# VictoriaMetrics/VictoriaLogs

Measured on NVIDIA H100. Metric: log rows scanned/sec (LogsQL phrase+regex), higher is better.
Workload: dtype u8

## Files before the change

### include/vlscan.h

```cpp
#ifndef VLSCAN_H
#define VLSCAN_H

#include <stddef.h>
#include <stdint.h>

#ifdef __cplusplus
extern "C" {
#endif

typedef struct vlscan_ctx vlscan_ctx;
typedef struct vlscan_program vlscan_program;
typedef struct vlscan_batch vlscan_batch;

enum {
    VLSCAN_VT_STRING = 1, VLSCAN_VT_DICT = 2, VLSCAN_VT_UINT8 = 3, VLSCAN_VT_UINT16 = 4, VLSCAN_VT_UINT32 = 5,
    VLSCAN_VT_UINT64 = 6, VLSCAN_VT_FLOAT64 = 7, VLSCAN_VT_IPV4 = 8, VLSCAN_VT_ISO8601 = 9, VLSCAN_VT_INT64 = 10
};

enum { VLSCAN_COL_CONST = 1, VLSCAN_COL_VALUES = 2 };

enum {
    VLSCAN_STAGE_ONDISK = 0,
    VLSCAN_STAGE_DECODED = 1
};

typedef struct vlscan_column {
    uint32_t field;
    uint8_t kind;
    uint8_t value_type;
    uint8_t stage;
    uint8_t dict_len;
    uint64_t min_value;
    uint64_t max_value;
    const uint8_t* const_value; uint64_t const_len;
    const uint8_t* dict_blob;   const uint32_t* dict_offsets;
    const uint8_t* values;      uint64_t values_len;
    const uint8_t* lens_items;  uint64_t lens_items_len;
    const uint8_t* data;        uint64_t data_len;
    const uint8_t* bloom;       uint64_t bloom_len;
} vlscan_column;

typedef struct vlscan_block {
    uint64_t rows;
    uint32_t ncols;
    uint32_t ts_marshal_type;
    const vlscan_column* cols;
    const uint8_t* timestamps; uint64_t timestamps_len;
    int64_t min_timestamp, max_timestamp;
} vlscan_block;

typedef struct vlscan_stats {
    uint64_t blocks;
    uint64_t rows;
    uint64_t rows_matched;
    uint64_t blocks_matched;
    uint64_t values_bytes;
    uint64_t bloom_probe_bytes;
    uint64_t bitmap_bytes;
    uint64_t columns_read;
    uint64_t gpu_launches;
    uint64_t h2d_bytes;
    uint64_t d2h_bytes;
    double gpu_ms;
    double scan_kernel_ms;
    uint64_t scan_kernel_bytes;
    uint64_t staged_columns;
    uint64_t pruned_columns;
} vlscan_stats;

typedef struct vlscan_gen_config {
    uint64_t seed;
    uint64_t total_rows;
    uint32_t rows_per_block;
    uint32_t hot_block_permille;
    uint32_t hit_row_permille;
    uint32_t columns_mask;
} vlscan_gen_config;
#define VLSCAN_GEN_T0 1700000000000000000ll
#define VLSCAN_GEN_STEP 1000000ll

int vlscan_device_count(void);
vlscan_ctx* vlscan_ctx_create(int device);
void vlscan_ctx_free(vlscan_ctx* ctx);
const char* vlscan_last_error(const vlscan_ctx* ctx);
void* vlscan_ctx_stream(const vlscan_ctx* ctx);
int vlscan_ctx_sync(vlscan_ctx* ctx);

enum { VLSCAN_F_NOOP = 0, VLSCAN_F_PHRASE, VLSCAN_F_PREFIX, VLSCAN_F_EXACT, VLSCAN_F_IN, VLSCAN_F_REGEXP, VLSCAN_F_AND, VLSCAN_F_OR, VLSCAN_F_NOT,
       VLSCAN_F_EXACT_PREFIX = 9, VLSCAN_F_LEN_RANGE = 10, VLSCAN_F_STRING_RANGE = 11, VLSCAN_F_IPV4_RANGE = 12, VLSCAN_F_VALUE_TYPE = 13,
       VLSCAN_F_ANY_CASE_PHRASE = 14, VLSCAN_F_ANY_CASE_PREFIX = 15, VLSCAN_F_SEQUENCE = 16, VLSCAN_F_CONTAINS_ALL = 17, VLSCAN_F_CONTAINS_ANY = 18, VLSCAN_F_EQ_FIELD = 19, VLSCAN_F_LE_FIELD = 20, VLSCAN_F_RANGE = 21, VLSCAN_F_TIME = 22 };
int vlscan_program_create(const void* tree, size_t tree_len, vlscan_program** out);
void vlscan_program_free(vlscan_program* prog);
uint32_t vlscan_program_nfields(const vlscan_program* prog);
const char* vlscan_program_field(const vlscan_program* prog, uint32_t i, size_t* len);
int64_t vlscan_program_leaf_tokens(const vlscan_program* prog, uint32_t leaf, char* buf, size_t cap);
int64_t vlscan_program_prepass_tokens(const vlscan_program* prog, char* buf, size_t cap);
int64_t vlscan_program_in_hashes(const vlscan_program* prog, uint32_t leaf, uint64_t* out, size_t cap);
int64_t vlscan_program_in_typed(const vlscan_program* prog, uint32_t leaf, int value_type, uint64_t* out, size_t cap);
int vlscan_format_float64(uint64_t ieee_bits, char* buf, size_t cap);
double vlscan_parse_math_number(const void* s, size_t len);
int vlscan_parse_typed(int value_type, const void* s, size_t len, uint64_t* out);
int vlscan_eval_predicate(int kind, const void* value, size_t value_len, const void* arg1, size_t arg1_len, const void* arg2,
                          size_t arg2_len, uint64_t aux0, uint64_t aux1);

int vlscan_batch_upload(vlscan_ctx* ctx, const char* const* field_names, const size_t* field_name_lens, uint32_t nfields,
                        const vlscan_block* blocks, uint64_t nblocks, vlscan_batch** out, vlscan_stats* stats );
void vlscan_batch_free(vlscan_batch* batch);
uint64_t vlscan_batch_nblocks(const vlscan_batch* batch);
uint64_t vlscan_batch_rows(const vlscan_batch* batch);
uint64_t vlscan_batch_words(const vlscan_batch* batch);
uint64_t vlscan_batch_device_bytes(const vlscan_batch* batch);

int vlscan_batch_generate(vlscan_ctx* ctx, const vlscan_gen_config* cfg, uint64_t block_lo, uint64_t block_hi, vlscan_batch** out);

typedef struct vlscan_host_blocks vlscan_host_blocks;
int vlscan_batch_download(vlscan_ctx* ctx, const vlscan_batch* batch, vlscan_host_blocks** out);
const vlscan_block* vlscan_host_blocks_get(const vlscan_host_blocks* hb, uint64_t* nblocks, uint32_t* nfields);
const char* vlscan_host_blocks_field(const vlscan_host_blocks* hb, uint32_t i, size_t* len);
uint64_t vlscan_host_blocks_bytes(const vlscan_host_blocks* hb);
void vlscan_host_blocks_free(vlscan_host_blocks* hb);
int vlscan_host_blocks_compress(const vlscan_host_blocks* in, int threads, vlscan_host_blocks** out);

int vlscan_zstd_decompress(vlscan_ctx* ctx, uint32_t nframes, const void* const* frames, const size_t* frame_lens, void* dst,
                           const uint64_t* dst_offsets);
int vlscan_zstd_inspect(const void* bytes_block, size_t len, uint64_t out[5]);
int vlscan_zstd_walk_digest(const vlscan_block* blocks, uint64_t nblocks, int threads, uint64_t out[12]);

typedef struct vlscan_part vlscan_part;
typedef int (*vlscan_inflate_fn)(void* user, const void* frame, size_t frame_len, void* dst, size_t dst_len);
int vlscan_part_open(vlscan_ctx* ctx , const char* path, vlscan_inflate_fn inflate , void* user, vlscan_part** out);
void vlscan_part_free(vlscan_part* part);
void vlscan_part_header(const vlscan_part* part, uint64_t out[8]);
uint64_t vlscan_part_nblocks(const vlscan_part* part);
int vlscan_part_block_header(const vlscan_part* part, uint64_t i, uint64_t out[15]);
int vlscan_part_timestamps(const vlscan_part* part, uint64_t i, const uint8_t** data, uint64_t* len);
uint32_t vlscan_part_ncolumn_names(const vlscan_part* part);
const char* vlscan_part_column_name(const vlscan_part* part, uint32_t i, size_t* len);
int vlscan_part_blocks(const vlscan_part* part, const char* const* field_names, const size_t* field_name_lens, uint32_t nfields, uint64_t block_lo,
                       uint64_t block_hi, int64_t min_timestamp, int64_t max_timestamp, vlscan_host_blocks** out);
const uint64_t* vlscan_host_blocks_source(const vlscan_host_blocks* hb, uint64_t* n);

int vlscan_scan_resident(vlscan_ctx* ctx, const vlscan_program* prog, const vlscan_batch* batch, vlscan_stats* stats);

int vlscan_last_scan_stats(vlscan_ctx* ctx, vlscan_stats* stats);

int vlscan_fetch_results(vlscan_ctx* ctx, uint64_t* out_bitmap_words, uint32_t* out_match_counts, vlscan_stats* stats );
int vlscan_fetch_hits(vlscan_ctx* ctx, uint32_t* out_hit_rows, uint64_t cap, uint64_t* out_hit_offsets);
int vlscan_gather_timestamps(vlscan_ctx* ctx, int64_t* out_timestamps, uint64_t cap, uint64_t* out_hit_offsets);
int vlscan_gather_values(vlscan_ctx* ctx, const char* field, size_t field_len, uint8_t* out_bytes, uint64_t cap_bytes, uint64_t* out_value_offsets, uint64_t cap_values,
                         uint64_t* out_total_bytes, uint64_t* out_hit_offsets);
enum { VLSCAN_BUCKET_PLAIN = 0, VLSCAN_BUCKET_WEEK = 1, VLSCAN_BUCKET_MONTH = 2, VLSCAN_BUCKET_YEAR = 3 };
#define VLSCAN_HITS_MAX_BY 4
typedef struct vlscan_hits_query {
    int64_t step, offset;
    uint32_t calendar;
    uint32_t nby;
    const char* const* by_names;
    const size_t* by_name_lens;
} vlscan_hits_query;
int vlscan_hits_stats(vlscan_ctx* ctx, const vlscan_hits_query* q, int64_t* out_buckets, uint64_t* out_counts, uint64_t cap_groups, uint8_t* out_key_bytes,
                      uint64_t cap_key_bytes, uint64_t* out_key_offsets, uint64_t out_info[4]);
#define VLSCAN_STATS_MAX_VALUES 4
int vlscan_hits_sums(vlscan_ctx* ctx, const vlscan_hits_query* q, const char* const* value_names, const size_t* value_name_lens, uint32_t nvalues, int64_t* out_buckets,
                     uint64_t* out_counts, double* out_sums, uint64_t* out_value_counts, uint64_t cap_groups, uint8_t* out_key_bytes, uint64_t cap_key_bytes,
                     uint64_t* out_key_offsets, uint64_t out_info[4]);
int64_t vlscan_truncate_timestamp(int64_t ts, int64_t step, int64_t offset, uint32_t calendar);
typedef struct vlscan_last_query {
    uint64_t limit;
    int64_t min_timestamp;
    uint32_t nfields;
    const char* const* field_names;
    const size_t* field_name_lens;
} vlscan_last_query;
int vlscan_last_rows(vlscan_ctx* ctx, const vlscan_last_query* q, int64_t* out_timestamps, uint32_t* out_blocks, uint32_t* out_rows, uint64_t cap_rows,
                     uint8_t* out_bytes, uint64_t cap_bytes, uint64_t* out_offsets, uint64_t out_info[4]);
enum { VLSCAN_FACET_UINT64 = 0, VLSCAN_FACET_NEGATIVE = 1, VLSCAN_FACET_STRING = 2 };
#define VLSCAN_FACETS_DEFAULT_MAX_VALUES 1000
#define VLSCAN_FACETS_DEFAULT_MAX_VALUE_LEN 128
typedef struct vlscan_facets_query {
    uint64_t max_values_per_field;
    uint64_t max_value_len;
    uint32_t nfields;
    const char* const* field_names;
    const size_t* field_name_lens;
} vlscan_facets_query;
int vlscan_facets(vlscan_ctx* ctx, const vlscan_facets_query* q, uint8_t* out_dropped, uint64_t* out_field_offsets, uint64_t* out_hits, uint8_t* out_classes,
                  uint64_t cap_entries, uint8_t* out_bytes, uint64_t cap_bytes, uint64_t* out_value_offsets, uint64_t out_info[4]);
int vlscan_result_digest(vlscan_ctx* ctx, uint64_t block_lo, uint64_t block_hi, uint64_t key_base, uint64_t* out_digest);
int vlscan_totals_sum(vlscan_ctx* const* ctxs, int nctx, uint64_t out4[4]);
int vlscan_result_device_ptrs(vlscan_ctx* ctx, void** bitmap_words, void** match_counts, void** totals4);

int vlscan_scan_batch(vlscan_ctx* ctx, const vlscan_program* prog, const char* const* field_names, const size_t* field_name_lens,
                      uint32_t nfields, const vlscan_block* blocks, uint64_t nblocks, uint64_t* out_bitmap_words,
                      uint32_t* out_match_counts, vlscan_stats* stats);
int vlscan_scan_batch_keep(vlscan_ctx* ctx, const vlscan_program* prog, const char* const* field_names, const size_t* field_name_lens,
                           uint32_t nfields, const vlscan_block* blocks, uint64_t nblocks, uint64_t* out_bitmap_words,
                           uint32_t* out_match_counts, vlscan_stats* stats);
int vlscan_stage_selected(vlscan_ctx* ctx, const vlscan_block* blocks, uint64_t nblocks, const char* const* field_names, const size_t* field_name_lens,
                          uint32_t nfields, const uint32_t* block_list , uint64_t nlist, uint64_t out_info[4]);

#ifdef __cplusplus
}
#endif
#endif
```

### victorialogs_b200/csrc/vl_engine.cu

```cuda
#include <dlfcn.h>
#include <algorithm>
#include <atomic>
#include <chrono>
#include <cmath>
#include <limits>
#include <thread>
#include <cstdio>
#include <cstdlib>
#include <cstring>
#include <functional>
#include <map>
#include <memory>
#include <mutex>
#include "vl_copier.h"
#include "vl_engine.h"
#include "vl_kernels.cuh"
#include "vl_program.h"
#include "vl_part.h"
#include "vl_mathnum.cuh"

using namespace vl;

namespace vl {
static thread_local std::string g_thread_err;
void set_thread_error(const std::string& s) { g_thread_err = s; }
}

struct vlscan_program {
    Program p;
    struct Image { DevBuf leaves, prepass, regexes, blob, u64s, u32s; DevProgram view; };
    std::map<int, std::unique_ptr<Image>> images;
    std::mutex mu;
    const DevProgram& image(int device, cudaStream_t st) {
        std::lock_guard<std::mutex> g(mu);
        auto it = images.find(device);
        if (it != images.end()) return it->second->view;
        auto im = std::make_unique<Image>();
        auto up = [&](DevBuf& b, const void* src, size_t n) { b.ensure(std::max<size_t>(n, 16)); if (n) VL_CUDA(cudaMemcpyAsync(b.p, src, n, cudaMemcpyHostToDevice, st)); };
        up(im->leaves, p.leaves.data(), p.leaves.size() * sizeof(DevLeaf));
        up(im->prepass, p.prepass.data(), p.prepass.size() * sizeof(DevPrepass));
        up(im->regexes, p.regexes.data(), p.regexes.size() * sizeof(DevRegex));
        up(im->blob, p.blob.data(), p.blob.size());
        up(im->u64s, p.u64s.data(), p.u64s.size() * 8);
        up(im->u32s, p.u32s.data(), p.u32s.size() * 4);
        VL_CUDA(cudaStreamSynchronize(st));
        im->view = DevProgram{im->leaves.as<DevLeaf>(), im->prepass.as<DevPrepass>(), im->regexes.as<DevRegex>(), im->blob.as<uint8_t>(), im->u64s.as<uint64_t>(), im->u32s.as<uint32_t>()};
        auto& ref = *im;
        images[device] = std::move(im);
        return ref.view;
    }
    ~vlscan_program() { for (auto& kv : images) { cudaSetDevice(kv.first); kv.second->leaves.release(); kv.second->prepass.release(); kv.second->regexes.release(); kv.second->blob.release(); kv.second->u64s.release(); kv.second->u32s.release(); } }
};

struct vlscan_host_blocks {
    void* pinned = nullptr; size_t bytes = 0;
    std::vector<vlscan_block> blocks;
    std::vector<vlscan_column> cols;
    std::vector<std::string> fields;
    std::vector<std::vector<uint32_t>> dict_offsets;
    std::vector<std::unique_ptr<std::vector<uint8_t>>> owned;
    std::vector<uint64_t> source;
};
struct vlscan_part { vl::part::PartReader r; };

void* vlscan_ctx::ensure_pinned(size_t n) {
    if (n <= pinned_cap) return pinned;
    if (pinned) cudaFreeHost(pinned);
    pinned = nullptr; pinned_cap = 0;
    VL_CUDA(cudaMallocHost(&pinned, n));
    pinned_cap = n;
    return pinned;
}

namespace {

struct ZstdWriter {
    size_t (*compress)(void*, size_t, const void*, size_t, int) = nullptr;
    size_t (*bound)(size_t) = nullptr;
    unsigned (*is_error)(size_t) = nullptr;
    bool ok = false;
    ZstdWriter() {
        void* h = dlopen("libzstd.so.1", RTLD_NOW | RTLD_GLOBAL);
        if (!h) return;
        compress = (decltype(compress))dlsym(h, "ZSTD_compress");
        bound = (decltype(bound))dlsym(h, "ZSTD_compressBound");
        is_error = (decltype(is_error))dlsym(h, "ZSTD_isError");
        ok = compress && bound && is_error;
    }
};
ZstdWriter& zstd_writer() { static ZstdWriter z; return z; }

}

namespace vl {
void finish_batch_layout(vlscan_ctx* ctx, vlscan_batch* b, const std::vector<uint32_t>& rows) {
    b->nblocks = rows.size();
    b->h_rows = rows;
    b->h_word_off.assign(rows.size() + 1, 0);
    b->rows = 0;
    for (size_t i = 0; i < rows.size(); i++) { b->h_word_off[i + 1] = b->h_word_off[i] + (rows[i] + 63) / 64; b->rows += rows[i]; }
    b->nwords = b->h_word_off.back();
    std::vector<uint32_t> wb(b->nwords);
    std::vector<uint64_t> init(b->nwords);
    for (size_t i = 0; i < rows.size(); i++) {
        for (uint64_t w = b->h_word_off[i]; w < b->h_word_off[i + 1]; w++) { wb[w] = (uint32_t)i; init[w] = ~0ull; }
        uint32_t tail = rows[i] & 63;
        if (tail) init[b->h_word_off[i + 1] - 1] = (~0ull) >> (64 - tail);
    }
    b->blk_rows.ensure(std::max<size_t>(rows.size() * 4, 16));
    b->blk_word_off.ensure((rows.size() + 1) * 8);
    b->word_block.ensure(std::max<size_t>(b->nwords * 4, 16));
    b->init_bitmap.ensure(std::max<size_t>(b->nwords * 8, 16));
    if (!rows.empty()) VL_CUDA(cudaMemcpyAsync(b->blk_rows.p, rows.data(), rows.size() * 4, cudaMemcpyHostToDevice, ctx->stream));
    VL_CUDA(cudaMemcpyAsync(b->blk_word_off.p, b->h_word_off.data(), (rows.size() + 1) * 8, cudaMemcpyHostToDevice, ctx->stream));
    if (b->nwords) {
        VL_CUDA(cudaMemcpyAsync(b->word_block.p, wb.data(), b->nwords * 4, cudaMemcpyHostToDevice, ctx->stream));
        VL_CUDA(cudaMemcpyAsync(b->init_bitmap.p, init.data(), b->nwords * 8, cudaMemcpyHostToDevice, ctx->stream));
    }
    VL_CUDA(cudaStreamSynchronize(ctx->stream));
}
}

static uint64_t collect_values_blocks(const vlscan_block* blocks, uint64_t nblocks, std::vector<ZValuesBlock>& zv, const uint8_t* need = nullptr, uint32_t nfields = 0, std::vector<size_t>* at = nullptr) {
    uint64_t zc = 512;
    if (at) at->assign((size_t)nblocks * nfields, SIZE_MAX);
    for (uint64_t b = 0; b < nblocks; b++)
        for (uint32_t k = 0; k < blocks[b].ncols; k++) {
            const vlscan_column& c = blocks[b].cols[k];
            if (c.kind != VLSCAN_COL_VALUES || c.stage != VLSCAN_STAGE_ONDISK) continue;
            if (need && (c.field >= nfields || !need[b * nfields + c.field])) continue;
            if (at && c.field < nfields && (*at)[b * nfields + c.field] == SIZE_MAX) (*at)[b * nfields + c.field] = zv.size();
            zv.push_back({c.values, (size_t)c.values_len, zc});
            zc += c.values_len;
        }
    return zc;
}
static double now_s() { return std::chrono::duration<double>(std::chrono::steady_clock::now().time_since_epoch()).count(); }

namespace {
struct Upload {
    vlscan_ctx* ctx; vlscan_batch* out; const vlscan_block* blocks; uint64_t nblocks; uint32_t nfields; vlscan_stats* stats;
    const std::vector<char>* need_bloom;
    std::vector<DevColumn>& cols = out->h_cols;
    const bool dbg = getenv("VLSCAN_DEBUG_TIMING") != nullptr; const double t_start = now_s();
    Copier io{ctx};
    std::vector<uint32_t> rows = std::vector<uint32_t>(nblocks);
    std::vector<Piece> pieces;
    std::vector<std::unique_ptr<std::vector<uint8_t>>> owned;
    uint64_t cursor = 16;
    ZstdJob zjob;
    uint64_t regen_cursor = 0;
    struct Ondisk { uint64_t col; uint32_t lens_frame, data_frame; uint64_t lens_rel, data_rel; };
    std::vector<Ondisk> ondisk;
    std::vector<OndiskCol> ocols;
    struct TsFrame { uint64_t block; uint32_t frame; uint64_t rel; };
    std::vector<TsFrame> ts_frames;
    std::vector<DevTimestamps> tsv;
    std::vector<ZValuesBlock> zv; std::vector<ZValuesInfo> zinfo; std::vector<size_t> zv_of; std::vector<uint64_t> ts_zoff; size_t zbad = SIZE_MAX; std::string zmsg;
    uint64_t add_piece(const uint8_t* src, uint64_t len) { uint64_t off = arena_reserve(cursor, len); if (len) pieces.push_back({src, len, off}); return off; }
    template <class F> void walk(bool ts, F&& f) {
        for (uint64_t b = 0; b < nblocks; b++) {
            const vlscan_block& blk = blocks[b];
            if (blk.rows > (8u << 20)) throw BadInput("block rows exceed maxRowsPerBlock (8Mi)");
            rows[b] = (uint32_t)blk.rows;
            if (ts) timestamps(blk, b);
            for (uint32_t k = 0; k < blk.ncols; k++) {
                if (blk.cols[k].field >= nfields) throw BadInput("column refers to a field outside the batch field table");
                f(blk, blk.cols[k], (size_t)b * nfields + blk.cols[k].field);
            }
        }
    }
    void sources(const uint8_t* need, bool ts) {
        uint64_t zc = collect_values_blocks(blocks, nblocks, zv, need, nfields, &zv_of);
        for (const ZValuesBlock& v : zv) if (v.n) io.src.push_back({v.p, v.n, v.zoff});
        ts_zoff.resize(ts ? nblocks : 0);
        for (uint64_t b = 0; b < nblocks && ts; b++) {
            const vlscan_block& blk = blocks[b];
            if (blk.ts_marshal_type != MT_ZSTD_NEAREST_DELTA2 && blk.ts_marshal_type != MT_ZSTD_NEAREST_DELTA) continue;
            if (blk.timestamps_len > vl::part::kMaxTimestampsBlockSize) throw BadInput("timestamps block size cannot exceed 8 MiB");
            ts_zoff[b] = zc;
            if (blk.timestamps_len) io.src.push_back({blk.timestamps, blk.timestamps_len, zc});
            zc += blk.timestamps_len;
        }
        if (!io.src.empty()) { ctx->zsrc.ensure(zc + 512); io.send_sources(ctx->zsrc.as<uint8_t>()); }
        zinfo.resize(zv.size());
        const double t_w = now_s();
        if (!zv.empty()) zjob.add_values_blocks(zv.data(), zv.size(), host_threads(), zinfo.data(), &zbad, &zmsg);
        if (dbg) fprintf(stderr, "[vlscan upload] header walk of %zu values blocks on %d host threads: %.1f ms (after %.1f ms of collecting and enqueueing the copies)\n",
                         zv.size(), host_threads(), 1e3 * (now_s() - t_w), 1e3 * (t_w - t_start));
    }
    template <class F> void header(const vlscan_column& c, size_t i, F&& payload) {
        DevColumn& d = cols[i];
        if (d.kind != COL_MISSING) throw BadInput("duplicate column for one field in a block");
        if (c.kind == VLSCAN_COL_CONST) {
            d.kind = COL_CONST; d.meta_len = (uint32_t)c.const_len; d.meta_off = add_piece(c.const_value, c.const_len);
            return;
        }
        if (c.kind != VLSCAN_COL_VALUES) throw BadInput("unknown column kind");
        if (c.value_type < VT_STRING || c.value_type >= VT_MAX) throw BadInput("unknown valueType");
        d.kind = COL_VALUES; d.vt = c.value_type; d.min_value = c.min_value; d.max_value = c.max_value;
        payload();
        if (c.bloom_len % 8) throw BadInput("cannot unmarshal bloomFilter from src with size not multiple by 8");
        if (need_bloom && !(*need_bloom)[c.field]) { d.bloom_words = 0; d.bloom_off = add_piece(c.bloom, 0); }
        else { d.bloom_words = (uint32_t)(c.bloom_len / 8); d.bloom_off = add_piece(c.bloom, c.bloom_len); }
        if (c.value_type == VT_DICT) {
            if (c.dict_len > 8) throw BadInput("valuesDict may contain max 8 items");
            d.dict_len = c.dict_len;
            uint32_t total = c.dict_len ? c.dict_offsets[c.dict_len] : 0;
            d.meta_len = total;
            if (c.dict_len && c.dict_blob == (const uint8_t*)c.dict_offsets + 4 * (c.dict_len + 1)) {
                d.meta_off = add_piece((const uint8_t*)c.dict_offsets, 4 * (c.dict_len + 1) + total);
            } else {
                auto meta = std::make_unique<std::vector<uint8_t>>();
                meta->resize(4 * (c.dict_len + 1) + total);
                if (c.dict_len) memcpy(meta->data(), c.dict_offsets, 4 * (c.dict_len + 1)); else memset(meta->data(), 0, 4);
                if (total) memcpy(meta->data() + 4 * (c.dict_len + 1), c.dict_blob, total);
                d.meta_off = add_piece(meta->data(), meta->size());
                owned.push_back(std::move(meta));
            }
        }
    }
    void values(const vlscan_block& blk, const vlscan_column& c, size_t ci) {
        DevColumn& d = cols[ci];
        if (c.stage == VLSCAN_STAGE_ONDISK) {
            const size_t z = zv_of[ci];
            if (z >= zbad) throw BadInput(zmsg);
            const uint64_t lens_len = zinfo[z].lens_len, data_len = zinfo[z].data_len;
            if (data_len > 0xFFFFFFFFull) throw BadInput("values block too large");
            const uint64_t lr = arena_reserve(regen_cursor, lens_len + 15), dr = arena_reserve(regen_cursor, data_len);
            d.lens_off = lr + 16; d.data_off = dr; d.data_len = data_len;
            ondisk.push_back({ci, (uint32_t)(2 * z), (uint32_t)(2 * z + 1), lr + 15, dr});
            ocols.push_back({ci, lens_len, blk.rows});
        } else if (c.stage == VLSCAN_STAGE_DECODED) {
            const uint8_t* lens_items = c.lens_items; const uint64_t lens_len = c.lens_items_len, data_len = c.data_len;
            if (lens_len < 1) throw BadInput("cannot unmarshal uint64 block type from empty src");
            uint8_t lt = lens_items[0];
            if (lt > 7) throw BadInput("unexpected uint64 block type");
            uint64_t want = lt < 4 ? (blk.rows << lt) : (1ull << (lt - 4));
            if (lens_len - 1 != want) throw BadInput("unexpected block length for uint items");
            d.lens_type = lt;
            if (lt >= 4) { uint64_t v = 0; for (uint64_t i = 0; i < want; i++) v = (v << 8) | lens_items[1 + i]; if (v > 0xFFFFFFFFull) throw BadInput("row length does not fit 32 bits"); d.lens_const = (uint32_t)v; }
            if (data_len > 0xFFFFFFFFull) throw BadInput("values block too large");
            d.lens_off = add_piece(lens_items + 1, lens_len - 1);
            d.data_off = add_piece(c.data, data_len); d.data_len = data_len;
            d.data_const = (blk.rows >= 2 && lt >= 4 && data_len == d.lens_const) ? 1 : 0;
        } else throw BadInput("unknown values stage");
    }
    void timestamps(const vlscan_block& blk, uint64_t b) {
        if (!blk.ts_marshal_type) return;
        if (blk.ts_marshal_type > MT_NEAREST_DELTA) throw BadInput("unknown MarshalType of a timestamps block");
        if (blk.timestamps_len > vl::part::kMaxTimestampsBlockSize) throw BadInput("timestamps block size cannot exceed 8 MiB");
        if (tsv.empty()) { tsv.resize(nblocks); memset(tsv.data(), 0, nblocks * sizeof(DevTimestamps)); }
        DevTimestamps& t = tsv[b];
        t.first = blk.min_timestamp; t.max = blk.max_timestamp;
        if (blk.ts_marshal_type == MT_ZSTD_NEAREST_DELTA2 || blk.ts_marshal_type == MT_ZSTD_NEAREST_DELTA) {
            uint64_t regen = 0; uint32_t id = 0;
            zjob.add_frame(blk.timestamps, blk.timestamps_len, ts_zoff[b], &regen, &id);
            if (regen > 10ull * blk.rows + 16) throw BadInput("cannot unmarshal timestamps: the decompressed block is larger than its varints can be");
            t.mt = blk.ts_marshal_type == MT_ZSTD_NEAREST_DELTA2 ? MT_NEAREST_DELTA2 : MT_NEAREST_DELTA;
            t.len = (uint32_t)regen;
            ts_frames.push_back({b, id, arena_reserve(regen_cursor, regen)});
        } else {
            t.mt = (uint8_t)blk.ts_marshal_type; t.len = (uint32_t)blk.timestamps_len;
            t.off = add_piece(blk.timestamps, blk.timestamps_len);
        }
    }

    uint64_t commit(DevBuf& region, const std::vector<uint64_t>* patch, bool layout) {
        const uint64_t regen_base = (cursor + kArenaAlign - 1) / kArenaAlign * kArenaAlign;
        for (const Ondisk& o : ondisk) {
            DevColumn& d = cols[o.col];
            d.lens_off += regen_base; d.data_off += regen_base;
            zjob.set_dst(o.lens_frame, regen_base + o.lens_rel); zjob.set_dst(o.data_frame, regen_base + o.data_rel);
        }
        for (const TsFrame& tf : ts_frames) { tsv[tf.block].off = regen_base + tf.rel; zjob.set_dst(tf.frame, regen_base + tf.rel); }
        const bool have_z = !ondisk.empty() || !ts_frames.empty();
        if (have_z) cursor = regen_base + regen_cursor;
        const uint64_t bytes = cursor + kArenaPad;
        const double t_desc = now_s();
        region.ensure(bytes);
        const double t_alloc = now_s();
        uint8_t* cols_base = region.as<uint8_t>();
        std::vector<ColPatch> patches;
        if (patch) {
            const uint64_t delta = (uint64_t)(uintptr_t)region.p - (uint64_t)(uintptr_t)out->arena.p;
            cols_base = out->arena.as<uint8_t>();
            patches.resize(patch->size());
            for (size_t i = 0; i < patch->size(); i++) {
                DevColumn& d = cols[(*patch)[i]];
                d.lens_off += delta; d.data_off += delta;
                patches[i].col = (*patch)[i]; patches[i].c = d;
            }
        }
        cudaStream_t cs = ctx->copy_stream;
        cudaEvent_t ev_cleared = io.events.make(), ev_copied = io.events.make();
        VL_CUDA(cudaMemsetAsync(region.p, 0, bytes, ctx->stream));
        VL_CUDA(cudaEventRecord(ev_cleared, ctx->stream));
        VL_CUDA(cudaStreamWaitEvent(cs, ev_cleared, 0));
        const double t_h2d = dbg ? now_s() : 0;
        double t_zrun = 0;
        if (have_z) {
            zjob.set_group_hook([&](uint64_t src_end) { io.wait_sources(ctx->stream, src_end); });
            zjob.run(ctx, ctx->zsrc.as<uint8_t>(), region.as<uint8_t>());
            io.ship_sources(UINT64_MAX);
            if (dbg) t_zrun = now_s();
        }
        io.copy(pieces, region.as<uint8_t>());
        DevBuf& table = patch ? ctx->patch : out->cols;
        const void* entries = patch ? (const void*)patches.data() : (const void*)cols.data();
        const size_t table_bytes = patch ? patches.size() * sizeof(ColPatch) : cols.size() * sizeof(DevColumn);
        table.ensure(std::max<size_t>(table_bytes, 16));
        if (table_bytes) VL_CUDA(cudaMemcpyAsync(table.p, entries, table_bytes, cudaMemcpyHostToDevice, cs));
        io.h2d += table_bytes;
        if (!patch) out->has_ts = !tsv.empty();
        if (!tsv.empty()) {
            out->ts.ensure(nblocks * sizeof(DevTimestamps));
            VL_CUDA(cudaMemcpyAsync(out->ts.p, tsv.data(), nblocks * sizeof(DevTimestamps), cudaMemcpyHostToDevice, cs));
            io.h2d += nblocks * sizeof(DevTimestamps);
        }
        VL_CUDA(cudaEventRecord(ev_copied, cs));
        if (!patches.empty()) {
            VL_CUDA(cudaStreamWaitEvent(ctx->stream, ev_copied, 0));
            k_patch_cols<<<cdiv(patches.size(), 128), 128, 0, ctx->stream>>>(out->cols.as<DevColumn>(), ctx->patch.as<ColPatch>(), (uint32_t)patches.size());
            launch_check(ctx);
        }
        const double t_enq = dbg ? now_s() : 0;
        if (have_z) {
            VL_CUDA(cudaStreamWaitEvent(ctx->stream, ev_copied, 0));
            ctx->zcols.ensure(16 + ocols.size() * sizeof(OndiskCol));
            VL_CUDA(cudaMemsetAsync(ctx->zcols.p, 0, 16, ctx->stream));
            VL_CUDA(cudaMemcpyAsync(ctx->zcols.as<uint8_t>() + 16, ocols.data(), ocols.size() * sizeof(OndiskCol), cudaMemcpyHostToDevice, ctx->stream));
            if (!ocols.empty()) {
                k_finish_ondisk_cols<<<cdiv(ocols.size(), 128), 128, 0, ctx->stream>>>(cols_base, out->cols.as<DevColumn>(), (const OndiskCol*)(ctx->zcols.as<uint8_t>() + 16),
                                                                                         (uint32_t)ocols.size(), ctx->zcols.as<unsigned long long>());
                launch_check(ctx);
            }
            io.h2d += ocols.size() * sizeof(OndiskCol);
            zjob.check(ctx);
            unsigned long long cst[2] = {0, 0};
            VL_CUDA(cudaMemcpy(cst, ctx->zcols.p, 16, cudaMemcpyDeviceToHost));
            static const char* what[] = {"", "cannot unmarshal uint64 block type from empty src", "unexpected uint64 block type", "unexpected block length for uint items", "row length does not fit 32 bits"};
            if (cst[0]) throw BadInput(what[std::min<unsigned long long>(cst[0], 4)]);
        }
        VL_CUDA(cudaStreamWaitEvent(ctx->stream, ev_copied, 0));
        double t_copy = 0;
        if (dbg) { VL_CUDA(cudaStreamSynchronize(ctx->stream)); t_copy = now_s(); }
        if (nfields) out->note_columns(cols);
        if (layout) finish_batch_layout(ctx, out, rows);
        else VL_CUDA(cudaStreamSynchronize(ctx->stream));
        if (dbg) fprintf(stderr, "[vlscan upload] blocks=%llu arena=%.1f MB h2d=%.1f MB pieces=%zu+%zu pinned=%d: describe %.1f ms, alloc %.1f ms, copy %.1f ms (%.1f GB/s), "
                                 "zstd %llu frames / %llu blocks / %llu sequences: enqueue %.1f ms, decode %.1f ms; layout %.1f ms\n", (unsigned long long)nblocks,
                         bytes / 1e6, io.h2d / 1e6, pieces.size(), io.src.size(), (int)io.all_pinned, 1e3 * (t_desc - t_start), 1e3 * (t_alloc - t_desc), 1e3 * (t_enq - (t_zrun > 0 ? t_zrun : t_h2d)), io.h2d / 1e9 / std::max(t_copy - t_start, 1e-9),
                         (unsigned long long)zjob.frames(), (unsigned long long)zjob.compressed_blocks(), (unsigned long long)zjob.sequences(), 1e3 * (t_zrun > 0 ? t_zrun - t_h2d : 0), 1e3 * (t_copy - t_enq), 1e3 * (now_s() - t_copy));
        if (layout) io.h2d += out->nwords * 12 + nblocks * 12;
        if (stats) stats->h2d_bytes += io.h2d;
        return bytes;
    }
};
}

enum UploadMode { UP_FULL = 0, UP_HEADERS = 1, UP_VALUES = 2, UP_LATE = 3 };
static void do_upload(vlscan_ctx* ctx, const char* const* field_names, const size_t* field_name_lens, uint32_t nfields, const vlscan_block* blocks,
                      uint64_t nblocks, vlscan_batch* out, vlscan_stats* stats, const std::vector<char>* need_bloom = nullptr, UploadMode mode = UP_FULL,
                      const uint8_t* need = nullptr, uint64_t* zframes = nullptr) {
    VL_CUDA(cudaSetDevice(ctx->device));
    if (nblocks > 0xFFFFFFF0ull) throw BadInput("too many blocks in one batch");
    out->device = ctx->device; out->nfields = nfields;
    Upload u{ctx, out, blocks, nblocks, nfields, stats, need_bloom};
    if (mode == UP_FULL || mode == UP_HEADERS) {
        for (uint32_t f = 0; f < nfields; f++) out->field_names.emplace_back(field_names[f], field_name_lens[f]);
        u.cols.assign((size_t)nblocks * std::max<uint32_t>(nfields, 1), DevColumn{});
        memset(u.cols.data(), 0, u.cols.size() * sizeof(DevColumn));
        out->late_used = 0; out->split_hdr = mode == UP_HEADERS;
    } else if (u.cols.size() != (size_t)nblocks * std::max<uint32_t>(nfields, 1) || !need) throw BadInput("internal: values phase of a bloom-first upload without its header phase");
    try {
        switch (mode) {
        case UP_FULL:
            u.sources(nullptr, true);
            u.walk(true, [&](const vlscan_block& blk, const vlscan_column& c, size_t i) { u.header(c, i, [&] { u.values(blk, c, i); }); });
            out->arena_bytes = u.commit(out->arena, nullptr, true);
            out->harena_bytes = 0;
            std::vector<DevColumn>().swap(out->h_cols);
            break;
        case UP_HEADERS:
            u.walk(false, [&](const vlscan_block&, const vlscan_column& c, size_t i) {
                u.header(c, i, [&] {
                    if (c.stage != VLSCAN_STAGE_ONDISK && c.stage != VLSCAN_STAGE_DECODED) throw BadInput("unknown values stage");
                    u.cols[i].values_state = VALUES_DEFERRED;
                });
            });
            out->harena_bytes = u.commit(out->harena, nullptr, true);
            break;
        case UP_VALUES:
            u.sources(need, true);
            u.walk(true, [&](const vlscan_block& blk, const vlscan_column& c, size_t i) {
                if (c.kind != VLSCAN_COL_VALUES) return;
                u.cols[i].values_state = need[i] ? VALUES_STAGED : VALUES_ABSENT;
                if (need[i]) u.values(blk, c, i);
            });
            out->arena_bytes = u.commit(out->arena, nullptr, false);
            break;
        case UP_LATE: {
            std::vector<uint64_t> staged;
            u.sources(need, false);
            u.walk(false, [&](const vlscan_block& blk, const vlscan_column& c, size_t i) {
                if (c.kind != VLSCAN_COL_VALUES || !need[i]) return;
                if (u.cols[i].values_state == VALUES_STAGED) throw BadInput("duplicate column for one field in a block");
                u.cols[i].values_state = VALUES_STAGED;
                u.values(blk, c, i);
                staged.push_back(i);
            });
            if (out->late_used == out->late.size()) out->late.emplace_back();
            u.commit(out->late[out->late_used], &staged, false);
            out->late_used++;
            *zframes += u.zjob.frames();
            break;
        }
        }
    } catch (...) {
        cudaStreamSynchronize(ctx->copy_stream); cudaStreamSynchronize(ctx->stream);
        throw;
    }
}

const uint32_t* vl::row_offsets(vlscan_ctx* ctx, const BatchView& B, int slot, const uint32_t* list, const uint32_t* wc, unsigned long long* stats, int wc_slot) {
    uint8_t* ready = ctx->ready[slot].as<uint8_t>();
    if (!ctx->ready_cleared[slot]) { VL_CUDA(cudaMemsetAsync(ready, 0, B.nblocks, ctx->stream)); ctx->ready_cleared[slot] = 1; }
    k_lens_offsets<<<ctx->sm_count * 8, 256, 0, ctx->stream>>>(B, slot, list, wc, ctx->row_off8[slot].as<uint32_t>(), ready, stats, wc_slot); launch_check(ctx);
    return ctx->row_off8[slot].as<uint32_t>();
}

namespace {
struct ScanRun {
    vlscan_ctx* ctx; const vlscan_program* prog; const vlscan_batch* batch;
    DevProgram P; BatchView B; std::vector<int> field_slot;
    unsigned long long* stats;
    size_t regs_used = 0;

    uint64_t* new_reg() {
        if (regs_used == ctx->regs.size()) ctx->regs.emplace_back();
        DevBuf& r = ctx->regs[regs_used++];
        r.ensure(std::max<size_t>(B.nwords * 8, 16));
        return r.as<uint64_t>();
    }
    void free_reg() { regs_used--; }
    void copy_reg(uint64_t* dst, const uint64_t* src) { if (B.nwords) VL_CUDA(cudaMemcpyAsync(dst, src, B.nwords * 8, cudaMemcpyDeviceToDevice, ctx->stream)); }
    void andnot(uint64_t* a, const uint64_t* b) { if (!B.nwords) return; k_andnot<<<cdiv(B.nwords, 256), 256, 0, ctx->stream>>>(a, b, B.nwords); launch_check(ctx); }
    void prepass(const PNode& nd, uint64_t* reg) {
        if (nd.prepass_count == 0) return;
        std::vector<int> slots(nd.prepass_count);
        for (int e = 0; e < nd.prepass_count; e++) slots[e] = field_slot[prog->p.prepass[nd.prepass_begin + e].field];
        size_t off = slots_cursor; slots_cursor += slots.size();
        ctx->slots.ensure(std::max<size_t>(slots_total * 4, 16));
        VL_CUDA(cudaMemcpyAsync(ctx->slots.as<int>() + off, slots.data(), slots.size() * 4, cudaMemcpyHostToDevice, ctx->stream));
        k_prepass<<<cdiv((uint64_t)B.nblocks * 32, 128), 128, 0, ctx->stream>>>(P, B, (uint32_t)nd.prepass_begin, (uint32_t)nd.prepass_count, ctx->slots.as<int>() + off,
                                                                             nd.kind == F_OR, reg, stats);
        launch_check(ctx);
    }
    size_t slots_cursor = 0, slots_total = 0;

    void leaf(int leaf_idx, uint64_t* reg) {
        const DevLeaf& L = prog->p.leaves[leaf_idx];
        if (L.kind == F_NOOP) return;
        int slot = L.field >= 0 ? field_slot[L.field] : -1;
        uint8_t* action = ctx->action.as<uint8_t>(); uint64_t* payload = ctx->payload.as<uint64_t>(); uint64_t* leaf_bm = ctx->leaf_bm.as<uint64_t>();
        uint32_t* lens_blocks = ctx->lens_blocks.as<uint32_t>(); uint32_t* row_blocks = ctx->row_blocks.as<uint32_t>(); uint32_t* wc = ctx->work_count.as<uint32_t>();
        ScanTile* tiles = ctx->tiles.as<ScanTile>();
        VL_CUDA(cudaMemsetAsync(wc, 0, WC_COUNT * 4, ctx->stream));
        if (L.kind == F_EQ_FIELD || L.kind == F_LE_FIELD) {
            const int slot_b = field_slot[L.field2];
            uint32_t* lens_b = ctx->lens_blocks2.as<uint32_t>();
            k_plan_pair<<<cdiv((uint64_t)B.nblocks * 32, 256), 256, 0, ctx->stream>>>(P, B, (uint32_t)leaf_idx, slot, slot_b, reg, action, payload, lens_blocks, lens_b, row_blocks, wc, stats);
            launch_check(ctx);
            if (B.nwords) {
                const int persistent = ctx->sm_count * 8;
                const uint32_t *ro_a = nullptr, *ro_b = nullptr;
                for (int side = 0; side < 2; side++) {
                    const int sl = side ? slot_b : slot;
                    if (sl >= 0) (side ? ro_b : ro_a) = row_offsets(ctx, B, sl, side ? lens_b : lens_blocks, wc, stats, side ? WC_LENS2 : WC_LENS);
                }
                k_row_pair<<<persistent, 256, 0, ctx->stream>>>(P, B, (uint32_t)leaf_idx, slot, slot_b, row_blocks, wc, payload, reg, ro_a, ro_b, leaf_bm, stats); launch_check(ctx);
                k_apply_leaf<<<cdiv(B.nwords, 256), 256, 0, ctx->stream>>>(B, action, leaf_bm, reg); launch_check(ctx);
            }
            return;
        }
        k_plan_leaf<<<cdiv(B.nblocks, VL_PLAN_WARPS), VL_PLAN_WARPS * 32, 0, ctx->stream>>>(P, B, (uint32_t)leaf_idx, slot, reg, action, payload, lens_blocks, row_blocks, tiles, wc, stats);
        launch_check(ctx);
        if (slot >= 0 && B.nwords) {
            const uint32_t vts = batch->slot_vt_mask.empty() ? ~0u : batch->slot_vt_mask[slot];
            const bool has_string = vts >> VT_STRING & 1, has_dict = vts >> VT_DICT & 1;
            const bool has_numeric = (vts & ~((1u << VT_STRING) | (1u << VT_DICT))) != 0;
            const bool may_scan = L.str_strategy == STR_SCAN && has_string;
            const bool may_row = (has_string && L.str_strategy != STR_ALL) || has_numeric;
            const uint32_t* ro = may_scan || may_row ? row_offsets(ctx, B, slot, lens_blocks, wc, stats, WC_LENS) : nullptr;
            if (may_scan) {
                VL_CUDA(cudaMemsetAsync(leaf_bm, 0, B.nwords * 8, ctx->stream));
                ScanParams sp; memset(&sp, 0, sizeof sp);
                sp.mode = L.scan_mode; sp.needle_off = L.scan_needle_off; sp.needle_len = L.scan_needle_len; sp.starts_tok = L.starts_tok; sp.ends_tok = L.ends_tok; sp.regex = L.regex;
                const bool masked = fill_scan_patterns(prog->p.blob.data() + L.scan_needle_off, L.scan_needle_len, sp.pat, sp.msk, sp.delta, sp.nd16);
                if (L.scan_mode == SCAN_CONTAINS || L.scan_mode >= SCAN_RX_DOTPLUS) { sp.starts_tok = sp.ends_tok = 0; }
                auto& evp = next_scan_events();
                VL_CUDA(cudaEventRecord(evp.first, ctx->stream));
                if (masked) k_substr_scan<true><<<ctx->sm_count * ctx->scan_occ[1], VL_SCAN_THREADS, 0, ctx->stream>>>(P, B, slot, sp, tiles, wc, ro, leaf_bm);
                else k_substr_scan<false><<<ctx->sm_count * ctx->scan_occ[0], VL_SCAN_THREADS, 0, ctx->stream>>>(P, B, slot, sp, tiles, wc, ro, leaf_bm);
                launch_check(ctx);
                VL_CUDA(cudaEventRecord(evp.second, ctx->stream));
            }
            if (may_row) { k_row_match<<<ctx->sm_count * ctx->row_occ, 256, 0, ctx->stream>>>(P, B, (uint32_t)leaf_idx, slot, row_blocks, wc, action, payload, reg, ro, leaf_bm); launch_check(ctx); }
            if (has_dict || has_numeric) { k_word_match<<<cdiv(B.nwords, 128), 128, 0, ctx->stream>>>(P, B, (uint32_t)leaf_idx, slot, action, payload, reg, leaf_bm, stats); launch_check(ctx); }
        }
        if (L.kind == F_TIME && B.nwords) {
            ctx->ts_vals.ensure(B.nwords * 64 * 8);
            k_time_match<<<ctx->sm_count * 4, 256, 0, ctx->stream>>>(B, (long long)L.aux0, (long long)L.aux1, row_blocks, wc, ctx->ts_vals.as<unsigned long long>(), leaf_bm, stats);
            launch_check(ctx);
        }
        if (B.nwords) { k_apply_leaf<<<cdiv(B.nwords, 256), 256, 0, ctx->stream>>>(B, action, leaf_bm, reg); launch_check(ctx); }
    }
    std::pair<cudaEvent_t, cudaEvent_t>& next_scan_events() {
        if (ctx->scan_events_used == ctx->scan_events.size()) { cudaEvent_t a, b; VL_CUDA(cudaEventCreate(&a)); VL_CUDA(cudaEventCreate(&b)); ctx->scan_events.emplace_back(a, b); }
        return ctx->scan_events[ctx->scan_events_used++];
    }
    void probe_leaf(int leaf_idx, const uint64_t* reg, uint8_t* need) {
        const DevLeaf& L = prog->p.leaves[leaf_idx];
        if (L.kind == F_NOOP || L.kind == F_TIME) return;
        const int slot = L.field >= 0 ? field_slot[L.field] : -1;
        if (L.kind == F_EQ_FIELD || L.kind == F_LE_FIELD) {
            k_plan_pair<<<cdiv((uint64_t)B.nblocks * 32, 256), 256, 0, ctx->stream>>>(P, B, (uint32_t)leaf_idx, slot, field_slot[L.field2], reg, nullptr, nullptr, nullptr, nullptr, nullptr, nullptr, stats, need);
        } else {
            if (slot < 0) return;
            k_plan_leaf<<<cdiv(B.nblocks, VL_PLAN_WARPS), VL_PLAN_WARPS * 32, 0, ctx->stream>>>(P, B, (uint32_t)leaf_idx, slot, reg, nullptr, nullptr, nullptr, nullptr, nullptr, nullptr, stats, need);
        }
        launch_check(ctx);
    }
    void probe_node(int id, uint64_t* reg, uint8_t* need) {
        const PNode& nd = prog->p.nodes[id];
        switch (nd.kind) {
        case F_NOOP: break;
        case F_AND: case F_OR: {
            uint64_t* r = reg;
            if (nd.prepass_count) { r = new_reg(); copy_reg(r, reg); prepass(nd, r); }
            for (int k : nd.kids) probe_node(k, r, need);
            if (nd.prepass_count) free_reg();
            break;
        }
        case F_NOT: probe_node(nd.kids[0], reg, need); break;
        default: probe_leaf(nd.leaf, reg, need);
        }
    }
    void node(int id, uint64_t* reg) {
        const PNode& nd = prog->p.nodes[id];
        switch (nd.kind) {
        case F_NOOP: break;
        case F_AND: prepass(nd, reg); for (int k : nd.kids) node(k, reg); break;
        case F_OR: {
            prepass(nd, reg);
            uint64_t* res = new_reg(); uint64_t* tmp = new_reg();
            copy_reg(res, reg);
            for (int k : nd.kids) { copy_reg(tmp, res); node(k, tmp); andnot(res, tmp); }
            andnot(reg, res);
            free_reg(); free_reg();
            break;
        }
        case F_NOT: { uint64_t* tmp = new_reg(); copy_reg(tmp, reg); node(nd.kids[0], tmp); andnot(reg, tmp); free_reg(); break; }
        default: leaf(nd.leaf, reg);
        }
    }
};
}

static void read_stats(vlscan_ctx* ctx, vlscan_stats* st, bool check_error) {
    unsigned long long h[ST_COUNT];
    VL_CUDA(cudaMemcpyAsync(h, ctx->stats.p, sizeof h, cudaMemcpyDeviceToHost, ctx->stream));
    VL_CUDA(cudaStreamSynchronize(ctx->stream));
    if (check_error && h[ST_ERROR]) {
        static const char* const msg[] = {"", "cannot unmarshal strings: row lengths do not add up to the data length", "too big index for dict value",
                                          "unexpected length for binary representation of a number", "", "", "the filter needs the timestamps of a block that was handed over without them", "cannot unmarshal timestamps",
                                          "internal: a filter reached the values of a column that the bloom-first probe pass had left on the host"};
        throw BadInput(msg[std::min<unsigned long long>(h[ST_ERROR], 8)]);
    }
    if (!st) return;
    st->values_bytes += h[ST_VALUES_BYTES]; st->bloom_probe_bytes += h[ST_BLOOM_BYTES]; st->columns_read += h[ST_COLUMNS_READ];
    st->bitmap_bytes += h[ST_BITMAP_BYTES]; st->rows_matched += h[ST_ROWS_MATCHED]; st->blocks_matched += h[ST_BLOCKS_MATCHED];
    st->scan_kernel_bytes += h[ST_SCAN_BYTES];
    float ms = 0;
    VL_CUDA(cudaEventElapsedTime(&ms, ctx->ev_begin, ctx->ev_end)); st->gpu_ms += ms;
    for (size_t i = 0; i < ctx->scan_events_used; i++) { VL_CUDA(cudaEventElapsedTime(&ms, ctx->scan_events[i].first, ctx->scan_events[i].second)); st->scan_kernel_ms += ms; }
}

static void do_scan(vlscan_ctx* ctx, const vlscan_program* prog, const vlscan_batch* batch, vlscan_stats* stats) {
    VL_CUDA(cudaSetDevice(ctx->device));
    if (batch->device != ctx->device) throw BadInput("batch lives on another device than the ctx");
    ScanRun run{ctx, prog, batch};
    run.P = const_cast<vlscan_program*>(prog)->image(ctx->device, ctx->stream);
    run.B = batch->view();
    const Program& pr = prog->p;
    run.field_slot.assign(pr.fields.size(), -1);
    for (size_t f = 0; f < pr.fields.size(); f++) for (uint32_t s = 0; s < batch->nfields; s++) if (batch->field_names[s] == pr.fields[f]) run.field_slot[f] = (int)s;
    for (auto& nd : pr.nodes) run.slots_total += nd.prepass_count;
    uint64_t nb = std::max<uint64_t>(batch->nblocks, 1), nw = std::max<uint64_t>(batch->nwords, 1);
    ctx->action.ensure(nb); ctx->payload.ensure(nb * 8); ctx->leaf_bm.ensure(nw * 8);
    ctx->lens_blocks.ensure(nb * 4); ctx->lens_blocks2.ensure(nb * 4); ctx->row_blocks.ensure(nb * 4); ctx->work_count.ensure(WC_COUNT * 4);
    {
        uint64_t max_tiles = batch->arena_bytes / VL_TILE_BYTES + nb + 16;
        ctx->tiles.ensure(max_tiles * sizeof(ScanTile));
    }
    ctx->stats.ensure(ST_COUNT * 8); ctx->totals.ensure(32); ctx->counts.ensure(nb * 4);
    if (ctx->row_off8.size() < batch->nfields) { ctx->row_off8.resize(batch->nfields); ctx->ready.resize(batch->nfields); }
    ctx->ready_cleared.assign(batch->nfields, 0);
    for (uint32_t s = 0; s < batch->nfields; s++) { ctx->row_off8[s].ensure(nw * 32); ctx->ready[s].ensure(nb); }
    uint64_t launches0 = ctx->launches;
    ctx->scan_events_used = 0;
    run.stats = ctx->stats.as<unsigned long long>();
    VL_CUDA(cudaEventRecord(ctx->ev_begin, ctx->stream));
    VL_CUDA(cudaMemsetAsync(ctx->stats.p, 0, ST_COUNT * 8, ctx->stream));
    VL_CUDA(cudaMemsetAsync(ctx->totals.p, 0, 32, ctx->stream));
    uint64_t* reg = run.new_reg();
    run.copy_reg(reg, batch->init_bitmap.as<uint64_t>());
    if (batch->nblocks) {
        run.node(pr.root, reg);
        k_finalize<<<cdiv(batch->nblocks, 8), 256, 0, ctx->stream>>>(run.B, reg, ctx->counts.as<uint32_t>(), run.stats, ctx->totals.as<unsigned long long>());
        launch_check(ctx);
    }
    VL_CUDA(cudaEventRecord(ctx->ev_end, ctx->stream));
    ctx->last_batch = batch; ctx->has_result = true; ctx->kept = false; ctx->last_launches = ctx->launches - launches0;
    ctx->last_nblocks = batch->nblocks; ctx->last_nwords = batch->nwords; ctx->last_rows = batch->rows;
    if (stats) {
        read_stats(ctx, stats, true);
        stats->blocks += batch->nblocks; stats->rows += batch->rows; stats->gpu_launches += ctx->launches - launches0;
    }
}

static void do_probe(vlscan_ctx* ctx, const vlscan_program* prog, const vlscan_batch* batch, std::vector<uint8_t>& need) {
    VL_CUDA(cudaSetDevice(ctx->device));
    ScanRun run{ctx, prog, batch};
    run.P = const_cast<vlscan_program*>(prog)->image(ctx->device, ctx->stream);
    run.B = batch->view();
    const Program& pr = prog->p;
    run.field_slot.assign(pr.fields.size(), -1);
    for (size_t f = 0; f < pr.fields.size(); f++) for (uint32_t s = 0; s < batch->nfields; s++) if (batch->field_names[s] == pr.fields[f]) run.field_slot[f] = (int)s;
    for (auto& nd : pr.nodes) run.slots_total += nd.prepass_count;
    const size_t cells = (size_t)batch->nblocks * batch->nfields;
    need.assign(cells, 0);
    if (!cells || !batch->nwords) return;
    ctx->need.ensure(std::max<size_t>(cells, 16)); ctx->stats.ensure(ST_COUNT * 8);
    VL_CUDA(cudaMemsetAsync(ctx->need.p, 0, cells, ctx->stream));
    VL_CUDA(cudaMemsetAsync(ctx->stats.p, 0, ST_COUNT * 8, ctx->stream));
    run.stats = ctx->stats.as<unsigned long long>();
    uint64_t* reg = run.new_reg();
    run.copy_reg(reg, batch->init_bitmap.as<uint64_t>());
    run.probe_node(pr.root, reg, ctx->need.as<uint8_t>());
    VL_CUDA(cudaMemcpyAsync(need.data(), ctx->need.p, cells, cudaMemcpyDeviceToHost, ctx->stream));
    VL_CUDA(cudaStreamSynchronize(ctx->stream));
}

extern "C" {

int vlscan_device_count(void) {
    int n = 0;
    if (cudaGetDeviceCount(&n) != cudaSuccess) { cudaGetLastError(); return 0; }
    return n;
}

vlscan_ctx* vlscan_ctx_create(int device) {
    vlscan_ctx* ctx = new vlscan_ctx();
    int rc = guarded(nullptr, [&] {
        int n = vlscan_device_count();
        if (n <= 0) throw CudaFail("no CUDA device is available: libvlscan has no CPU fallback", 100);
        ctx->device = ((device % n) + n) % n;
        VL_CUDA(cudaSetDevice(ctx->device));
        VL_CUDA(cudaStreamCreateWithFlags(&ctx->stream, cudaStreamNonBlocking));
        VL_CUDA(cudaStreamCreateWithFlags(&ctx->copy_stream, cudaStreamNonBlocking));
        VL_CUDA(cudaEventCreate(&ctx->ev_begin)); VL_CUDA(cudaEventCreate(&ctx->ev_end));
        cudaDeviceProp prop; VL_CUDA(cudaGetDeviceProperties(&prop, ctx->device)); ctx->sm_count = prop.multiProcessorCount;
        VL_CUDA(cudaOccupancyMaxActiveBlocksPerMultiprocessor(&ctx->scan_occ[0], k_substr_scan<false>, VL_SCAN_THREADS, 0));
        VL_CUDA(cudaOccupancyMaxActiveBlocksPerMultiprocessor(&ctx->scan_occ[1], k_substr_scan<true>, VL_SCAN_THREADS, 0));
        for (int& o : ctx->scan_occ) o = std::max(o, 1);
        VL_CUDA(cudaOccupancyMaxActiveBlocksPerMultiprocessor(&ctx->row_occ, k_row_match, 256, 0));
        ctx->row_occ = std::max(ctx->row_occ, 1);
    });
    if (rc) { delete ctx; return nullptr; }
    return ctx;
}
void vlscan_ctx_free(vlscan_ctx* ctx) {
    if (!ctx) return;
    cudaSetDevice(ctx->device);
    if (ctx->copy_stream) cudaStreamSynchronize(ctx->copy_stream);
    if (ctx->stream) cudaStreamSynchronize(ctx->stream);
    for (DevBuf* b : {&ctx->action, &ctx->payload, &ctx->leaf_bm, &ctx->lens_blocks, &ctx->row_blocks, &ctx->work_count, &ctx->stats, &ctx->totals, &ctx->counts, &ctx->slots, &ctx->hit_offs, &ctx->hits, &ctx->tiles, &ctx->lens_blocks2}) b->release();
    for (auto& r : ctx->regs) r.release();
    for (auto& r : ctx->row_off8) r.release();
    for (auto& r : ctx->ready) r.release();
    ctx->zsrc.release(); ctx->zcols.release(); ctx->ztest.release(); ctx->ts_vals.release();
    for (DevBuf* b : {&ctx->hit_block, &ctx->glens, &ctx->goffs, &ctx->gtiles, &ctx->gout, &ctx->gstat, &ctx->hslot, &ctx->hblk, &ctx->htab, &ctx->hgrp, &ctx->lcand, &ctx->ftab, &ctx->patch, &ctx->unstaged}) b->release();
    for (DevBuf& b : ctx->ftxt) b.release();
    zstd_dev_free(ctx->zdev);
    delete ctx->pool;
    if (ctx->pinned) cudaFreeHost(ctx->pinned);
    delete ctx->recycle;
    for (auto& e : ctx->scan_events) { cudaEventDestroy(e.first); cudaEventDestroy(e.second); }
    if (ctx->ev_begin) cudaEventDestroy(ctx->ev_begin);
    if (ctx->ev_end) cudaEventDestroy(ctx->ev_end);
    if (ctx->copy_stream) cudaStreamDestroy(ctx->copy_stream);
    if (ctx->stream) cudaStreamDestroy(ctx->stream);
    delete ctx;
}
const char* vlscan_last_error(const vlscan_ctx* ctx) { return ctx ? ctx->err.c_str() : g_thread_err.c_str(); }
void* vlscan_ctx_stream(const vlscan_ctx* ctx) { return (void*)ctx->stream; }
int vlscan_ctx_sync(vlscan_ctx* ctx) { return guarded(ctx, [&] { VL_CUDA(cudaSetDevice(ctx->device)); VL_CUDA(cudaStreamSynchronize(ctx->stream)); }); }

int vlscan_program_create(const void* tree, size_t tree_len, vlscan_program** out) {
    *out = nullptr;
    auto* pg = new vlscan_program();
    int rc = guarded(nullptr, [&] { ProgramBuilder(tree, tree_len, pg->p).build(); });
    if (rc) { delete pg; return rc; }
    *out = pg;
    return 0;
}
void vlscan_program_free(vlscan_program* prog) { delete prog; }
uint32_t vlscan_program_nfields(const vlscan_program* prog) { return (uint32_t)prog->p.fields.size(); }
const char* vlscan_program_field(const vlscan_program* prog, uint32_t i, size_t* len) { if (i >= prog->p.fields.size()) { *len = 0; return nullptr; } *len = prog->p.fields[i].size(); return prog->p.fields[i].data(); }
int64_t vlscan_program_leaf_tokens(const vlscan_program* prog, uint32_t leaf, char* buf, size_t cap) {
    if (leaf >= prog->p.leaf_tokens.size()) return -1;
    std::string s; for (size_t i = 0; i < prog->p.leaf_tokens[leaf].size(); i++) { if (i) s.push_back('\n'); s += prog->p.leaf_tokens[leaf][i]; }
    if (s.size() > cap) return -1;
    memcpy(buf, s.data(), s.size());
    return (int64_t)s.size();
}

int vlscan_eval_predicate(int kind, const void* value, size_t value_len, const void* arg1, size_t arg1_len, const void* arg2, size_t arg2_len, uint64_t aux0, uint64_t aux1) {
    if (value_len > 0xFFFFFFFFull || arg1_len > 0xFFFFFFFFull || arg2_len > 0xFFFFFFFFull) return -1;
    const uint8_t* v = (const uint8_t*)value; const uint32_t vn = (uint32_t)value_len;
    const uint8_t* a = (const uint8_t*)arg1; const uint32_t an = (uint32_t)arg1_len;
    switch (kind) {
    case F_REGEXP: {
        try { return vl::compile_regex(std::string((const char*)a, an)).match(v, vn) ? 1 : 0; } catch (const vl::RxError& e) { vl::set_thread_error(e.what()); return -2; }
    }
    case 14: return vl::any_case_match(v, vn, a, an, false) ? 1 : 0;
    case 15: return vl::any_case_match(v, vn, a, an, true) ? 1 : 0;
    case 16: return vl::match_sequence(v, vn, vl::PhraseList{a, an}) ? 1 : 0;
    case 17: return vl::match_all_phrases(v, vn, vl::PhraseList{a, an}) ? 1 : 0;
    case 18: return vl::match_any_phrase(v, vn, vl::PhraseList{a, an}) ? 1 : 0;
    }
    if (kind < F_EXACT_PREFIX || kind > F_IPV4_RANGE) return -1;
    return vl::range_predicate(kind, (const uint8_t*)value, (uint32_t)value_len, (const uint8_t*)arg1, (uint32_t)arg1_len, (const uint8_t*)arg2, (uint32_t)arg2_len, aux0, aux1) ? 1 : 0;
}

int64_t vlscan_program_prepass_tokens(const vlscan_program* prog, char* buf, size_t cap) {
    const Program& P = prog->p;
    std::string s;
    for (const PNode& nd : P.nodes) {
        if (nd.kind != F_AND && nd.kind != F_OR) continue;
        s += nd.kind == F_AND ? "A" : "O";
        for (int k = 0; k < nd.prepass_count; k++) {
            const DevPrepass& pp = P.prepass[(size_t)nd.prepass_begin + k];
            s += "\t" + P.fields[pp.field];
            const uint32_t* offs = (const uint32_t*)(P.blob.data() + pp.tok_offs_off);
            for (uint32_t t = 0; t < pp.ntokens; t++) { s += "\x1f"; s.append((const char*)P.blob.data() + pp.tok_blob_off + offs[t], offs[t + 1] - offs[t]); }
        }
        s += "\n";
    }
    if (s.size() > cap) return -1;
    memcpy(buf, s.data(), s.size());
    return (int64_t)s.size();
}

int64_t vlscan_program_in_hashes(const vlscan_program* prog, uint32_t leaf, uint64_t* out, size_t cap) {
    const Program& P = prog->p;
    if (leaf >= P.leaves.size() || P.leaves[leaf].kind != F_IN) return -1;
    const DevLeaf& L = P.leaves[leaf];
    std::vector<uint64_t> v;
    v.push_back(L.nhashes); v.insert(v.end(), P.u64s.begin() + L.hashes_off, P.u64s.begin() + L.hashes_off + L.nhashes);
    if (L.in_skip_sets) v.push_back(UINT64_MAX);
    else {
        v.push_back(L.in_nsets);
        for (uint32_t k = 0; k < L.in_nsets; k++) {
            const uint32_t off = P.u32s[L.in_sets_off + 2 * k], n = P.u32s[L.in_sets_off + 2 * k + 1];
            v.push_back(n); v.insert(v.end(), P.u64s.begin() + off, P.u64s.begin() + off + n);
        }
    }
    if (v.size() > cap) return -1;
    memcpy(out, v.data(), v.size() * 8);
    return (int64_t)v.size();
}

int64_t vlscan_program_in_typed(const vlscan_program* prog, uint32_t leaf, int value_type, uint64_t* out, size_t cap) {
    const Program& P = prog->p;
    if (leaf >= P.leaves.size() || P.leaves[leaf].kind != F_IN || value_type < VT_UINT8 || value_type >= VT_MAX) return -1;
    const DevLeaf& L = P.leaves[leaf];
    const uint32_t n = L.in_typed_cnt[value_type];
    if (n > cap) return -1;
    if (n) memcpy(out, P.u64s.data() + L.in_typed_off[value_type], (size_t)n * 8);
    return (int64_t)n;
}

int vlscan_parse_typed(int value_type, const void* s, size_t len, uint64_t* out) {
    const std::string v((const char*)s, len);
    uint64_t u = 0; int64_t i = 0; double f = 0; uint32_t ip = 0;
    switch (value_type) {
    case VT_UINT8: case VT_UINT16: case VT_UINT32: case VT_UINT64: if (!vl::parse_u64(v, &u)) return 0; *out = u; return 1;
    case VT_INT64: if (!vl::parse_i64(v, &i)) return 0; *out = (uint64_t)i; return 1;
    case VT_FLOAT64: if (!vl::parse_f64_exact(v, &f)) return 0; memcpy(out, &f, 8); return 1;
    case VT_IPV4: if (!vl::parse_ipv4(v, &ip)) return 0; *out = ip; return 1;
    case VT_ISO8601: if (!vl::parse_iso8601(v, &i)) return 0; *out = (uint64_t)i; return 1;
    }
    return -1;
}

double vlscan_parse_math_number(const void* s, size_t len) {
    if (len > 0xFFFFFFFFull) return NAN;
    return vl::mn::parse_math_number((const uint8_t*)s, (uint32_t)len);
}

int vlscan_format_float64(uint64_t ieee_bits, char* buf, size_t cap) {
    uint8_t tmp[VL_FMT_F64_MAX];
    int n = vl::fmt_f64(tmp, ieee_bits);
    if ((size_t)n > cap) return -1;
    memcpy(buf, tmp, (size_t)n);
    return n;
}

int vlscan_batch_upload(vlscan_ctx* ctx, const char* const* field_names, const size_t* field_name_lens, uint32_t nfields, const vlscan_block* blocks,
                        uint64_t nblocks, vlscan_batch** out, vlscan_stats* stats) {
    *out = nullptr;
    auto* b = new vlscan_batch();
    int rc = guarded(ctx, [&] { do_upload(ctx, field_names, field_name_lens, nfields, blocks, nblocks, b, stats); });
    if (rc) { delete b; return rc; }
    *out = b;
    return 0;
}
void vlscan_batch_free(vlscan_batch* batch) { delete batch; }
uint64_t vlscan_batch_nblocks(const vlscan_batch* b) { return b->nblocks; }
uint64_t vlscan_batch_rows(const vlscan_batch* b) { return b->rows; }
uint64_t vlscan_batch_words(const vlscan_batch* b) { return b->nwords; }
uint64_t vlscan_batch_device_bytes(const vlscan_batch* b) { return b->device_bytes(); }

int vlscan_batch_download(vlscan_ctx* ctx, const vlscan_batch* batch, vlscan_host_blocks** out) {
    *out = nullptr;
    auto* hb = new vlscan_host_blocks();
    int rc = guarded(ctx, [&] {
        VL_CUDA(cudaSetDevice(ctx->device));
        if (batch->split_hdr) throw BadInput("a batch staged bloom-first cannot be downloaded");
        hb->bytes = batch->arena_bytes;
        VL_CUDA(cudaMallocHost(&hb->pinned, std::max<size_t>(hb->bytes, 16)));
        std::vector<DevColumn> cols((size_t)batch->nblocks * batch->nfields);
        VL_CUDA(cudaMemcpyAsync(hb->pinned, batch->arena.p, hb->bytes, cudaMemcpyDeviceToHost, ctx->stream));
        if (!cols.empty()) VL_CUDA(cudaMemcpyAsync(cols.data(), batch->cols.p, cols.size() * sizeof(DevColumn), cudaMemcpyDeviceToHost, ctx->stream));
        VL_CUDA(cudaStreamSynchronize(ctx->stream));
        hb->fields = batch->field_names;
        const uint8_t* base = (const uint8_t*)hb->pinned;
        hb->blocks.resize(batch->nblocks);
        hb->cols.reserve(cols.size());
        std::vector<size_t> first(batch->nblocks + 1, 0);
        for (uint64_t b = 0; b < batch->nblocks; b++) {
            first[b] = hb->cols.size();
            for (uint32_t f = 0; f < batch->nfields; f++) {
                const DevColumn& d = cols[(size_t)b * batch->nfields + f];
                if (d.kind == COL_MISSING) continue;
                vlscan_column c; memset(&c, 0, sizeof c);
                c.field = f;
                if (d.kind == COL_CONST) { c.kind = VLSCAN_COL_CONST; c.const_value = base + d.meta_off; c.const_len = d.meta_len; hb->cols.push_back(c); continue; }
                c.kind = VLSCAN_COL_VALUES; c.value_type = d.vt; c.stage = VLSCAN_STAGE_DECODED; c.dict_len = d.dict_len; c.min_value = d.min_value; c.max_value = d.max_value;
// ... 90 lines not shown
                if (c.dict_len) memcpy(m, c.dict_offsets, 4 * (c.dict_len + 1)); else memset(m, 0, 4);
                if (total) memcpy(m + 4 * (c.dict_len + 1), c.dict_blob, total);
                c.dict_offsets = (const uint32_t*)m; c.dict_blob = m + 4 * (c.dict_len + 1);
            }
            memcpy(base + vbase + off_v[i], packed[i].data(), packed[i].size());
            c.stage = VLSCAN_STAGE_ONDISK; c.values = base + vbase + off_v[i]; c.values_len = packed[i].size();
            c.lens_items = nullptr; c.lens_items_len = 0; c.data = nullptr; c.data_len = 0;
            std::vector<uint8_t>().swap(packed[i]);
        }
        size_t k = 0;
        for (size_t b = 0; b < hb->blocks.size(); b++) { hb->blocks[b].cols = hb->cols.data() + k; k += hb->blocks[b].ncols; }
    });
    if (rc) { if (hb->pinned) cudaFreeHost(hb->pinned); delete hb; return rc; }
    *out = hb;
    return 0;
}

int vlscan_zstd_inspect(const void* bytes_block, size_t len, uint64_t out[5]) {
    return guarded(nullptr, [&] {
        ZstdJob job;
        uint64_t regen = 0; uint32_t id = 0;
        size_t used = job.add_bytes_block((const uint8_t*)bytes_block, len, 512, &regen, &id);
        out[0] = used; out[1] = regen; out[2] = job.blocks(); out[3] = job.compressed_blocks(); out[4] = job.sequences();
    });
}

int vlscan_zstd_walk_digest(const vlscan_block* blocks, uint64_t nblocks, int threads, uint64_t out[12]) {
    return guarded(nullptr, [&] {
        std::vector<ZValuesBlock> zv;
        collect_values_blocks(blocks, nblocks, zv);
        std::vector<ZValuesInfo> info(zv.size());
        ZstdJob job; size_t bad = SIZE_MAX; std::string msg;
        const double t0 = now_s();
        if (!zv.empty()) job.add_values_blocks(zv.data(), zv.size(), threads, info.data(), &bad, &msg);
        const double t1 = now_s();
        if (bad != SIZE_MAX) throw BadInput("values block " + std::to_string(bad) + ": " + msg);
        job.prepare();
        const double t2 = now_s();
        job.digest(out);
        uint64_t h = 5; for (const ZValuesInfo& x : info) { h = (h ^ x.lens_len) * 0x9E3779B97F4A7C15ull; h = (h ^ x.data_len) * 0x9E3779B97F4A7C15ull; h ^= h >> 29; }
        out[0] ^= h;
        out[4] = job.frames(); out[5] = job.blocks(); out[6] = job.groups(); out[7] = job.compressed_blocks(); out[8] = job.sequences();
        out[9] = (uint64_t)((t1 - t0) * 1e9); out[10] = (uint64_t)((t2 - t1) * 1e9); out[11] = 0;
    });
}

static void zstd_decompress_frames(vlscan_ctx* ctx, uint32_t nframes, const void* const* frames, const size_t* frame_lens, void* dst, const uint64_t* dst_offsets) {
    {
        VL_CUDA(cudaSetDevice(ctx->device));
        ZstdJob job;
        std::vector<uint8_t> packed(512, 0);
        for (uint32_t i = 0; i < nframes; i++) {
            uint64_t regen = 0; uint32_t id = 0;
            job.add_frame((const uint8_t*)frames[i], frame_lens[i], packed.size(), &regen, &id);
            if (regen != dst_offsets[i + 1] - dst_offsets[i]) throw BadInput("cannot decompress block: frame content size differs from the destination size");
            job.set_dst(id, 16 + dst_offsets[i]);
            packed.insert(packed.end(), (const uint8_t*)frames[i], (const uint8_t*)frames[i] + frame_lens[i]);
        }
        const uint64_t total = nframes ? dst_offsets[nframes] : 0;
        ctx->zsrc.ensure(packed.size() + 512); ctx->ztest.ensure(16 + total + 64);
        VL_CUDA(cudaMemcpyAsync(ctx->zsrc.p, packed.data(), packed.size(), cudaMemcpyHostToDevice, ctx->stream));
        VL_CUDA(cudaMemsetAsync(ctx->ztest.p, 0xA5, 16 + total + 64, ctx->stream));
        job.run(ctx, ctx->zsrc.as<uint8_t>(), ctx->ztest.as<uint8_t>());
        job.check(ctx);
        if (total) VL_CUDA(cudaMemcpy(dst, ctx->ztest.as<uint8_t>() + 16, total, cudaMemcpyDeviceToHost));
    }
}

int vlscan_zstd_decompress(vlscan_ctx* ctx, uint32_t nframes, const void* const* frames, const size_t* frame_lens, void* dst, const uint64_t* dst_offsets) {
    return guarded(ctx, [&] { zstd_decompress_frames(ctx, nframes, frames, frame_lens, dst, dst_offsets); });
}

int vlscan_part_open(vlscan_ctx* ctx, const char* path, vlscan_inflate_fn inflate, void* user, vlscan_part** out) {
    *out = nullptr;
    auto* p = new vlscan_part();
    int rc = guarded(ctx, [&] {
        if (!inflate && !ctx) throw BadInput("vlscan_part_open needs a ctx (device ZSTD decoder) or an inflate callback");
        vl::part::Inflate inf;
        if (inflate) inf = [&](const uint8_t* f, size_t n, uint8_t* dst, size_t dn) { if (inflate(user, f, n, dst, dn) != 0) throw BadInput("the inflate callback failed on a metadata frame of the part"); };
        else inf = [&](const uint8_t* f, size_t n, uint8_t* dst, size_t dn) { const void* fr[1] = {f}; const size_t ln[1] = {n}; const uint64_t offs[2] = {0, dn}; zstd_decompress_frames(ctx, 1, fr, ln, dst, offs); };
        p->r.open(path, inf);
    });
    if (rc) { delete p; return rc; }
    *out = p;
    return 0;
}
void vlscan_part_free(vlscan_part* part) { delete part; }
void vlscan_part_header(const vlscan_part* part, uint64_t out[8]) {
    const vl::part::PartHeader& h = part->r.ph;
    out[0] = h.FormatVersion; out[1] = h.CompressedSizeBytes; out[2] = h.UncompressedSizeBytes; out[3] = h.RowsCount; out[4] = h.BlocksCount;
    out[5] = (uint64_t)h.MinTimestamp; out[6] = (uint64_t)h.MaxTimestamp; out[7] = h.BloomValuesShardsCount;
}
uint64_t vlscan_part_nblocks(const vlscan_part* part) { return part->r.blockHeaders.size(); }
int vlscan_part_block_header(const vlscan_part* part, uint64_t i, uint64_t out[15]) {
    return guarded(nullptr, [&] {
        if (i >= part->r.blockHeaders.size()) throw BadInput("block index outside the part");
        const vl::part::BlockHeader& b = part->r.blockHeaders[i];
        out[0] = b.sid.accountID; out[1] = b.sid.projectID; out[2] = b.sid.hi; out[3] = b.sid.lo; out[4] = b.uncompressedSizeBytes; out[5] = b.rowsCount;
        out[6] = b.tsOffset; out[7] = b.tsSize; out[8] = (uint64_t)b.minTimestamp; out[9] = (uint64_t)b.maxTimestamp; out[10] = b.tsMarshalType;
        out[11] = b.chIndexOffset; out[12] = b.chIndexSize; out[13] = b.chOffset; out[14] = b.chSize;
    });
}
int vlscan_part_timestamps(const vlscan_part* part, uint64_t i, const uint8_t** data, uint64_t* len) {
    return guarded(nullptr, [&] {
        if (i >= part->r.blockHeaders.size()) throw BadInput("block index outside the part");
        const vl::part::BlockHeader& b = part->r.blockHeaders[i];
        if (b.tsSize > vl::part::kMaxTimestampsBlockSize) throw BadInput("timestamps block size is too big");
        *data = part->r.timestamps_file().at(b.tsOffset, b.tsSize, "a timestamps block"); *len = b.tsSize;
    });
}
uint32_t vlscan_part_ncolumn_names(const vlscan_part* part) { return (uint32_t)part->r.columnNames.size(); }
const char* vlscan_part_column_name(const vlscan_part* part, uint32_t i, size_t* len) { if (i >= part->r.columnNames.size()) { *len = 0; return nullptr; } const std::string& s = part->r.columnNames[i]; *len = s.size(); return s.data(); }
int vlscan_part_blocks(const vlscan_part* part, const char* const* field_names, const size_t* field_name_lens, uint32_t nfields, uint64_t block_lo, uint64_t block_hi,
                       int64_t min_timestamp, int64_t max_timestamp, vlscan_host_blocks** out) {
    *out = nullptr;
    auto* hb = new vlscan_host_blocks();
    int rc = guarded(nullptr, [&] {
        std::vector<std::string> fields;
        for (uint32_t f = 0; f < nfields; f++) { std::string n(field_names[f], field_name_lens[f]); fields.push_back(n.empty() ? "_msg" : n); }
        for (size_t a = 0; a < fields.size(); a++) for (size_t b = a + 1; b < fields.size(); b++) if (fields[a] == fields[b]) throw BadInput("duplicate field name");
        vl::part::Described d;
        part->r.describe(fields, block_lo, block_hi, min_timestamp, max_timestamp, d);
        hb->fields = std::move(d.fields); hb->cols = std::move(d.cols); hb->blocks = std::move(d.blocks); hb->owned = std::move(d.owned); hb->source = std::move(d.source);
        for (const vlscan_column& c : hb->cols) hb->bytes += c.const_len + c.values_len + c.bloom_len;
    });
    if (rc) { delete hb; return rc; }
    *out = hb;
    return 0;
}
const uint64_t* vlscan_host_blocks_source(const vlscan_host_blocks* hb, uint64_t* n) { *n = hb->source.size(); return hb->source.data(); }

const vlscan_block* vlscan_host_blocks_get(const vlscan_host_blocks* hb, uint64_t* nblocks, uint32_t* nfields) { *nblocks = hb->blocks.size(); *nfields = (uint32_t)hb->fields.size(); return hb->blocks.data(); }
const char* vlscan_host_blocks_field(const vlscan_host_blocks* hb, uint32_t i, size_t* len) { if (i >= hb->fields.size()) { *len = 0; return nullptr; } *len = hb->fields[i].size(); return hb->fields[i].data(); }
uint64_t vlscan_host_blocks_bytes(const vlscan_host_blocks* hb) { return hb->bytes; }
void vlscan_host_blocks_free(vlscan_host_blocks* hb) { if (!hb) return; if (hb->pinned) cudaFreeHost(hb->pinned); delete hb; }

int vlscan_scan_resident(vlscan_ctx* ctx, const vlscan_program* prog, const vlscan_batch* batch, vlscan_stats* stats) {
    return guarded(ctx, [&] { do_scan(ctx, prog, batch, stats); });
}

int vlscan_last_scan_stats(vlscan_ctx* ctx, vlscan_stats* stats) {
    return guarded(ctx, [&] {
        if (!ctx->has_result) throw BadInput("no scan on this ctx yet");
        VL_CUDA(cudaSetDevice(ctx->device));
        read_stats(ctx, stats, true);
        stats->blocks += ctx->last_nblocks; stats->rows += ctx->last_rows; stats->gpu_launches += ctx->last_launches;
    });
}

int vlscan_fetch_results(vlscan_ctx* ctx, uint64_t* out_bitmap_words, uint32_t* out_match_counts, vlscan_stats* stats) {
    return guarded(ctx, [&] {
        if (!ctx->has_result) throw BadInput("no scan result to fetch on this ctx");
        VL_CUDA(cudaSetDevice(ctx->device));
        uint64_t d2h = 0;
        if (out_bitmap_words && ctx->last_nwords) { VL_CUDA(cudaMemcpyAsync(out_bitmap_words, ctx->regs[0].p, ctx->last_nwords * 8, cudaMemcpyDeviceToHost, ctx->stream)); d2h += ctx->last_nwords * 8; }
        if (out_match_counts && ctx->last_nblocks) { VL_CUDA(cudaMemcpyAsync(out_match_counts, ctx->counts.p, ctx->last_nblocks * 4, cudaMemcpyDeviceToHost, ctx->stream)); d2h += ctx->last_nblocks * 4; }
        read_stats(ctx, nullptr, true);
        if (stats) stats->d2h_bytes += d2h;
    });
}

int vlscan_result_digest(vlscan_ctx* ctx, uint64_t block_lo, uint64_t block_hi, uint64_t key_base, uint64_t* out_digest) {
    return guarded(ctx, [&] {
        if (!ctx->has_result) throw BadInput("no scan result on this ctx");
        if (block_lo > block_hi || block_hi > ctx->last_nblocks) throw BadInput("block range outside the batch of the last scan");
        VL_CUDA(cudaSetDevice(ctx->device));
        ctx->hit_offs.ensure(16);
        VL_CUDA(cudaMemsetAsync(ctx->hit_offs.p, 0, 8, ctx->stream));
        if (block_hi > block_lo) {
            k_bitmap_digest<<<cdiv(block_hi - block_lo, 128), 128, 0, ctx->stream>>>(ctx->last_batch->view(), ctx->regs[0].as<uint64_t>(), (uint32_t)block_lo, (uint32_t)block_hi, key_base, ctx->hit_offs.as<unsigned long long>());
            launch_check(ctx);
        }
        VL_CUDA(cudaMemcpyAsync(out_digest, ctx->hit_offs.p, 8, cudaMemcpyDeviceToHost, ctx->stream));
        VL_CUDA(cudaStreamSynchronize(ctx->stream));
    });
}

int vlscan_totals_sum(vlscan_ctx* const* ctxs, int nctx, uint64_t out4[4]) {
    out4[0] = out4[1] = out4[2] = out4[3] = 0;
    for (int i = 0; i < nctx; i++) {
        vlscan_ctx* ctx = ctxs[i];
        int rc = guarded(ctx, [&] {
            if (!ctx->has_result) throw BadInput("no scan result on this ctx");
            VL_CUDA(cudaSetDevice(ctx->device));
            unsigned long long t[4];
            VL_CUDA(cudaMemcpyAsync(t, ctx->totals.p, 32, cudaMemcpyDeviceToHost, ctx->stream));
            VL_CUDA(cudaStreamSynchronize(ctx->stream));
            for (int k = 0; k < 4; k++) out4[k] += t[k];
        });
        if (rc) return rc;
    }
    return 0;
}

int vlscan_result_device_ptrs(vlscan_ctx* ctx, void** bitmap_words, void** match_counts, void** totals4) {
    if (!ctx->has_result) { ctx->err = "no scan result on this ctx"; return -1; }
    if (bitmap_words) *bitmap_words = ctx->regs[0].p;
    if (match_counts) *match_counts = ctx->counts.p;
    if (totals4) *totals4 = ctx->totals.p;
    return 0;
}

static vlscan_batch::CellSig cell_sig(const vlscan_column& c) {
    vlscan_batch::CellSig g;
    g.stage = c.stage;
    if (c.stage == VLSCAN_STAGE_ONDISK) g.len0 = c.values_len; else { g.len0 = c.lens_items_len; g.len1 = c.data_len; }
    return g;
}

static int scan_batch_impl(vlscan_ctx* ctx, const vlscan_program* prog, const char* const* field_names, const size_t* field_name_lens, uint32_t nfields,
                           const vlscan_block* blocks, uint64_t nblocks, uint64_t* out_bitmap_words, uint32_t* out_match_counts, vlscan_stats* stats, bool keep) {
    vlscan_batch* b = ctx->recycle ? ctx->recycle : new vlscan_batch();
    ctx->recycle = nullptr;
    b->field_names.clear(); b->slot_vt_mask.clear();
    uint64_t launches0 = ctx->launches;
    std::vector<char> need_bloom(nfields, 0), in_prog(nfields, 0);
    {
        const Program& P = prog->p;
        auto mark = [&](std::vector<char>& m, int field) { for (uint32_t s = 0; s < nfields; s++) if (std::string(field_names[s], field_name_lens[s]) == P.fields[field]) m[s] = 1; };
        for (const DevLeaf& L : P.leaves) if (L.nhashes || L.nhashes2 || L.in_nsets) mark(need_bloom, L.field);
        for (const DevPrepass& pp : P.prepass) if (pp.nhashes) mark(need_bloom, pp.field);
        if (keep) for (size_t f = 0; f < P.fields.size(); f++) mark(in_prog, (int)f);
    }
    int bf = 1;
    if (const char* e = getenv("VLSCAN_BLOOM_FIRST")) bf = atoi(e);
    bool probes = false;
    for (char c : need_bloom) probes |= c != 0;
    if (ctx->bf_prog != (const void*)prog) { ctx->bf_prog = prog; ctx->bf_skip = 0; }
    const bool probe = bf != 0 && probes && nblocks > 0 && (bf == 2 || ctx->bf_skip == 0);
    if (!probe && ctx->bf_skip > 0) ctx->bf_skip--;
    int rc;
    if (probe || keep) {
        rc = guarded(ctx, [&] {
            do_upload(ctx, field_names, field_name_lens, nfields, blocks, nblocks, b, stats, &need_bloom, UP_HEADERS);
            std::vector<uint8_t> need;
            if (probe) do_probe(ctx, prog, b, need);
            else {
                need.assign(std::max<size_t>((size_t)nblocks * nfields, 1), 0);
                for (uint64_t i = 0; i < nblocks; i++)
                    for (uint32_t k = 0; k < blocks[i].ncols; k++) if (blocks[i].cols[k].field < nfields && in_prog[blocks[i].cols[k].field]) need[i * nfields + blocks[i].cols[k].field] = 1;
            }
            uint64_t vals_all = 0, vals_need = 0, cols_all = 0, cols_need = 0;
            for (uint64_t i = 0; i < nblocks; i++)
                for (uint32_t k = 0; k < blocks[i].ncols; k++) {
                    const vlscan_column& c = blocks[i].cols[k];
                    if (c.kind != VLSCAN_COL_VALUES || c.field >= nfields) continue;
                    const bool needed = need[i * nfields + c.field] != 0;
                    cols_all++; cols_need += needed;
                    if (keep && !in_prog[c.field]) continue;
                    const uint64_t n = c.stage == VLSCAN_STAGE_ONDISK ? c.values_len : c.lens_items_len + c.data_len;
                    vals_all += n;
                    if (needed) vals_need += n;
                }
            if (stats && probe) { stats->staged_columns += cols_need; stats->pruned_columns += cols_all - cols_need; }
            if (probe && vals_need * 8 > vals_all * 7) ctx->bf_skip = 7;
            do_upload(ctx, field_names, field_name_lens, nfields, blocks, nblocks, b, stats, &need_bloom, UP_VALUES, need.data());
            if (keep) {
                b->h_sig.assign((size_t)nblocks * nfields, vlscan_batch::CellSig{});
                b->h_ncols.resize(nblocks);
                for (uint64_t i = 0; i < nblocks; i++) {
                    b->h_ncols[i] = blocks[i].ncols;
                    for (uint32_t k = 0; k < blocks[i].ncols; k++) {
                        const vlscan_column& c = blocks[i].cols[k];
                        if (c.kind == VLSCAN_COL_VALUES) b->h_sig[i * nfields + c.field] = cell_sig(c);
                    }
                }
            }
        });
    } else rc = guarded(ctx, [&] { do_upload(ctx, field_names, field_name_lens, nfields, blocks, nblocks, b, stats, &need_bloom); });
    if (!rc) rc = vlscan_scan_resident(ctx, prog, b, nullptr);
    if (!rc) rc = vlscan_fetch_results(ctx, out_bitmap_words, out_match_counts, stats);
    if (!rc && stats) {
        rc = guarded(ctx, [&] { read_stats(ctx, stats, true); stats->blocks += b->nblocks; stats->rows += b->rows; stats->gpu_launches += ctx->launches - launches0; });
    }
    if (keep && !rc) ctx->kept = true;
    else { ctx->has_result = false; ctx->last_batch = nullptr; ctx->kept = false; }
    ctx->recycle = b;
    return rc;
}

int vlscan_scan_batch(vlscan_ctx* ctx, const vlscan_program* prog, const char* const* field_names, const size_t* field_name_lens, uint32_t nfields,
                      const vlscan_block* blocks, uint64_t nblocks, uint64_t* out_bitmap_words, uint32_t* out_match_counts, vlscan_stats* stats) {
    return scan_batch_impl(ctx, prog, field_names, field_name_lens, nfields, blocks, nblocks, out_bitmap_words, out_match_counts, stats, false);
}

int vlscan_scan_batch_keep(vlscan_ctx* ctx, const vlscan_program* prog, const char* const* field_names, const size_t* field_name_lens, uint32_t nfields,
                           const vlscan_block* blocks, uint64_t nblocks, uint64_t* out_bitmap_words, uint32_t* out_match_counts, vlscan_stats* stats) {
    if (!ctx || !prog) return guarded(nullptr, [&] { throw BadInput(!ctx ? "vlscan_scan_batch_keep needs a vlscan_ctx on a CUDA device (there is no CPU fallback)" : "vlscan_scan_batch_keep: no program"); });
    return scan_batch_impl(ctx, prog, field_names, field_name_lens, nfields, blocks, nblocks, out_bitmap_words, out_match_counts, stats, true);
}

int vlscan_stage_selected(vlscan_ctx* ctx, const vlscan_block* blocks, uint64_t nblocks, const char* const* field_names, const size_t* field_name_lens, uint32_t nfields,
                          const uint32_t* block_list, uint64_t nlist, uint64_t out_info[4]) {
    uint64_t info[4] = {0, 0, 0, 0};
    bool staging = false;
    const int rc = guarded(ctx, [&] {
        if (nfields == 0) throw BadInput("vlscan_stage_selected needs at least one field");
        const std::vector<std::string> names = canonical_names(field_names, field_name_lens, nfields, "vlscan_stage_selected");
        if (nlist && !block_list) throw BadInput("vlscan_stage_selected: block list missing");
        if (!ctx) throw BadInput("vlscan_stage_selected needs a vlscan_ctx on a CUDA device (there is no CPU fallback)");
        if (!ctx->has_result || !ctx->kept || !ctx->recycle || ctx->last_batch != ctx->recycle) throw BadInput("no kept scan on this ctx (vlscan_scan_batch_keep keeps one until the next scan)");
        vlscan_batch* b = ctx->recycle;
        VL_CUDA(cudaSetDevice(ctx->device));
        const uint32_t nf = b->nfields;
        std::vector<char> want(nf, 0);
        for (const std::string& n : names) {
            const int slot = b->field_slot(n);
            if (slot < 0) throw BadInput("field `" + n + "` is not a field of the kept batch");
            want[slot] = 1;
        }
        if (!blocks || nblocks != b->nblocks) throw BadInput("the block descriptors differ from those of the kept scan: " + std::to_string(nblocks) + " blocks instead of " + std::to_string(b->nblocks));
        std::vector<uint8_t> sel(nblocks, 0);
        if (block_list) {
            for (uint64_t i = 0; i < nlist; i++) {
                if (block_list[i] >= nblocks) throw BadInput("block_list[" + std::to_string(i) + "] = " + std::to_string(block_list[i]) + " is outside the kept batch of " + std::to_string(nblocks) + " blocks");
                sel[block_list[i]] = 1;
            }
        } else if (nblocks) {
            std::vector<uint32_t> cnt(nblocks);
            VL_CUDA(cudaMemcpyAsync(cnt.data(), ctx->counts.p, nblocks * 4, cudaMemcpyDeviceToHost, ctx->stream));
            VL_CUDA(cudaStreamSynchronize(ctx->stream));
            for (uint64_t i = 0; i < nblocks; i++) sel[i] = cnt[i] != 0;
        }
        auto mismatch = [&](uint64_t i, const char* what) { return BadInput("the block descriptors differ from those of the kept scan: block " + std::to_string(i) + ", " + what); };
        for (uint64_t i = 0; i < nblocks; i++) {
            if (!sel[i]) continue;
            const vlscan_block& blk = blocks[i];
            if (blk.rows != b->h_rows[i]) throw mismatch(i, "row count");
            if (blk.ncols != b->h_ncols[i] || (blk.ncols && !blk.cols)) throw mismatch(i, "column count");
            for (uint32_t k = 0; k < blk.ncols; k++) {
                const vlscan_column& c = blk.cols[k];
                if (c.field >= nf) throw mismatch(i, "field of a column");
                const DevColumn& d = b->h_cols[i * nf + c.field];
                if (c.kind == VLSCAN_COL_CONST) { if (d.kind != COL_CONST || d.meta_len != c.const_len) throw mismatch(i, "const column"); }
                else if (c.kind == VLSCAN_COL_VALUES) {
                    if (d.kind != COL_VALUES || d.vt != c.value_type) throw mismatch(i, "column kind or value type");
                    const vlscan_batch::CellSig want = cell_sig(c), &had = b->h_sig[i * nf + c.field];
                    if (had.stage != want.stage || had.len0 != want.len0 || had.len1 != want.len1) throw mismatch(i, "values stage or payload lengths");
                } else throw mismatch(i, "column kind");
            }
        }
        std::vector<uint8_t> need((size_t)nblocks * nf, 0);
        for (uint64_t i = 0; i < nblocks; i++) {
            if (!sel[i]) continue;
            for (uint32_t s = 0; s < nf; s++) {
                const DevColumn& d = b->h_cols[i * nf + s];
                if (!want[s] || d.kind != COL_VALUES) continue;
                if (d.values_state == VALUES_STAGED) info[1]++;
                else { need[i * nf + s] = 1; info[0]++; }
            }
        }
        if (!info[0]) return;
        vlscan_stats st;
        memset(&st, 0, sizeof st);
        staging = true;
        do_upload(ctx, nullptr, nullptr, nf, blocks, nblocks, b, &st, nullptr, UP_LATE, need.data(), &info[3]);
        info[2] = st.h2d_bytes;
    });
    if (rc && staging) {
        ctx->has_result = false; ctx->last_batch = nullptr; ctx->kept = false;
        info[0] = info[1] = info[2] = info[3] = 0;
    }
    if (out_info && !rc) memcpy(out_info, info, sizeof info);
    return rc;
}

}
```

### victorialogs_b200/csrc/vl_engine.h

```cpp
#pragma once
#include <cuda_runtime.h>
#include <stdint.h>
#include <algorithm>
#include <string>
#include <vector>
#include "../../include/vlscan.h"
#include "vl_types.h"
#include "vl_zstd.h"
#include "vl_zstd_walk.h"
#include "vl_hostpool.h"

namespace vl {

void set_thread_error(const std::string& s);
#define VL_CUDA(call)                                                                                                   \
    do {                                                                                                                \
        cudaError_t e__ = (call);                                                                                       \
        if (e__ != cudaSuccess) throw CudaFail(std::string(#call) + ": " + cudaGetErrorString(e__), (int)e__);        \
    } while (0)
struct CudaFail { std::string msg; int code; CudaFail(std::string m, int c) : msg(std::move(m)), code(c) {} };

struct DevBuf {
    void* p = nullptr; size_t cap = 0;
    void ensure(size_t n) {
        if (n <= cap) return;
        if (p) VL_CUDA(cudaFree(p));
        p = nullptr; cap = 0;
        size_t want = n + std::min<size_t>(n / 8, (size_t)256 << 20) + 256;
        VL_CUDA(cudaMalloc(&p, want)); cap = want;
    }
    void release() { if (p) cudaFree(p); p = nullptr; cap = 0; }
    template <class T> T* as() const { return (T*)p; }
};



static const size_t kArenaAlign = 16;
static const size_t kArenaPad = 32;
inline uint64_t arena_reserve(uint64_t& cursor, uint64_t len) {
    uint64_t off = (cursor + kArenaAlign - 1) / kArenaAlign * kArenaAlign;
    cursor = off + len + kArenaPad;
    return off;
}

}

struct vlscan_batch {
    int device = 0;
    uint32_t nfields = 0;
    std::vector<std::string> field_names;
    uint64_t nblocks = 0, nwords = 0, rows = 0;
    uint64_t arena_bytes = 0, harena_bytes = 0;
    vl::DevBuf arena, cols, blk_rows, blk_word_off, word_block, init_bitmap, ts;
    vl::DevBuf harena;
    bool split_hdr = false;
    std::vector<vl::DevColumn> h_cols;
    bool has_ts = false;
    std::vector<uint32_t> h_rows;
    std::vector<uint64_t> h_word_off;
    std::vector<uint32_t> slot_vt_mask;
    std::vector<vl::DevBuf> late;
    size_t late_used = 0;
    struct CellSig { uint64_t len0 = 0, len1 = 0; uint32_t stage = 0; };
    std::vector<CellSig> h_sig;
    std::vector<uint32_t> h_ncols;
    void note_columns(const std::vector<vl::DevColumn>& cols) {
        slot_vt_mask.assign(nfields, 0);
        for (size_t i = 0; i < cols.size(); i++) if (cols[i].kind == vl::COL_VALUES) slot_vt_mask[i % nfields] |= 1u << cols[i].vt;
    }
    int field_slot(const std::string& name) const {
        for (uint32_t s = 0; s < nfields; s++) if (field_names[s] == name) return (int)s;
        return -1;
    }
    vl::BatchView view() const {
        vl::BatchView v;
        v.arena = arena.as<uint8_t>(); v.hdr = split_hdr ? harena.as<uint8_t>() : arena.as<uint8_t>(); v.cols = cols.as<vl::DevColumn>(); v.blk_rows = blk_rows.as<uint32_t>();
        v.blk_word_off = blk_word_off.as<uint64_t>(); v.word_block = word_block.as<uint32_t>();
        v.ts = has_ts ? ts.as<vl::DevTimestamps>() : nullptr;
        v.nblocks = (uint32_t)nblocks; v.nfields = nfields; v.nwords = nwords;
        return v;
    }
    uint64_t device_bytes() const {
        uint64_t n = arena.cap + harena.cap + cols.cap + blk_rows.cap + blk_word_off.cap + word_block.cap + init_bitmap.cap + ts.cap;
        for (const vl::DevBuf& r : late) n += r.cap;
        return n;
    }
    ~vlscan_batch() {
        cudaSetDevice(device); arena.release(); harena.release(); cols.release(); blk_rows.release(); blk_word_off.release(); word_block.release(); init_bitmap.release(); ts.release();
        for (vl::DevBuf& r : late) r.release();
    }
};

struct vlscan_ctx {
    int device = 0;
    cudaStream_t stream = nullptr;
    cudaStream_t copy_stream = nullptr;
    std::string err;
    uint64_t launches = 0;
    vl::DevBuf action, payload, leaf_bm, lens_blocks, work_count, stats, totals, counts, slots, tiles;
    vl::DevBuf lens_blocks2;
    vl::DevBuf row_blocks;
    vl::DevBuf hit_offs, hits;
    std::vector<vl::DevBuf> regs;
    std::vector<vl::DevBuf> row_off8;
    std::vector<vl::DevBuf> ready;
    std::vector<char> ready_cleared;
    vl::DevBuf hit_block, glens, goffs, gtiles, gout, gstat;
    vl::DevBuf ts_vals;
    vl::DevBuf hslot;
    vl::DevBuf hblk, htab, hgrp;
    vl::DevBuf lcand;
    vl::DevBuf ftab;
    std::vector<vl::DevBuf> ftxt;
    vl::DevBuf need;
    const void* bf_prog = nullptr; int bf_skip = 0;
    vl::DevBuf zsrc, zcols, ztest;
    vl::ZstdDev* zdev = nullptr;
    void* pinned = nullptr; size_t pinned_cap = 0;
    vl::HostPool* pool = nullptr;
    cudaEvent_t ev_begin = nullptr, ev_end = nullptr;
    std::vector<std::pair<cudaEvent_t, cudaEvent_t>> scan_events; size_t scan_events_used = 0;
    const vlscan_batch* last_batch = nullptr;
    uint64_t last_nblocks = 0, last_nwords = 0, last_rows = 0;
    vlscan_batch* recycle = nullptr;
    bool kept = false;
    vl::DevBuf patch, unstaged;
    bool has_result = false;
    uint64_t last_launches = 0;
    int sm_count = 132;
    int scan_occ[2] = {1, 1};
    int row_occ = 1;
    void* ensure_pinned(size_t n);
};

namespace vl {
void finish_batch_layout(vlscan_ctx* ctx, vlscan_batch* b, const std::vector<uint32_t>& rows);

const uint32_t* row_offsets(vlscan_ctx* ctx, const BatchView& B, int slot, const uint32_t* list, const uint32_t* wc, unsigned long long* stats, int wc_slot);

template <class F> int guarded(vlscan_ctx* ctx, F&& f) {
    try { f(); return 0; }
    catch (const CudaFail& e) { set_thread_error(e.msg); if (ctx) ctx->err = e.msg; return e.code > 0 ? e.code : 1; }
    catch (const BadInput& e) { set_thread_error(e.msg); if (ctx) ctx->err = e.msg; return -1; }
    catch (const ProgError& e) { set_thread_error(e.what()); if (ctx) ctx->err = e.what(); return -2; }
    catch (const std::exception& e) { set_thread_error(e.what()); if (ctx) ctx->err = e.what(); return -3; }
}

inline void launch_check(vlscan_ctx* ctx) { ctx->launches++; VL_CUDA(cudaGetLastError()); }
inline unsigned cdiv(uint64_t a, uint64_t b) { return (unsigned)((a + b - 1) / b); }

inline std::vector<std::string> canonical_names(const char* const* names, const size_t* lens, uint32_t n, const char* what) {
    if (n && (!names || !lens)) throw BadInput(std::string(what) + ": field names missing");
    std::vector<std::string> out;
    for (uint32_t f = 0; f < n; f++) out.push_back(lens[f] ? std::string(names[f], lens[f]) : "_msg");
    return out;
}
}
```

### victorialogs_b200/csrc/vl_kernels.cuh

```cuda
#pragma once
#include <cuda_runtime.h>
#include <stdint.h>
#include "vl_anycase.cuh"
#include "vl_mathnum.cuh"
#include "vl_cell.cuh"

namespace vl {

#define VL_SHORT_ROW_BYTES 48u

static __device__ __forceinline__ uint32_t rx_class(const DevRegex& R, const uint8_t* blob, int32_t r) {
    if (r < 128) return blob[R.ascii_off + r];
    const int32_t* b = (const int32_t*)(blob + R.bounds_off);
    int lo = 0, hi = (int)R.nclasses - 1;
    while (lo < hi) { int mid = (lo + hi + 1) >> 1; if (b[mid] <= r) lo = mid; else hi = mid - 1; }
    return (uint32_t)lo;
}
static __device__ bool dfa_run(const DevRegex& R, const uint8_t* blob, const uint8_t* s, uint32_t n) {
    const uint16_t* T = (const uint16_t*)(blob + R.trans_off);
    uint32_t st = 0;
    for (uint32_t i = 0; i < n;) {
        int w; int32_t r = s[i];
        if (r < 0x80) w = 1; else r = decode_rune(s + i, n - i, &w);
        i += w;
// ... 314 lines not shown
            case F_CONTAINS_ALL:
                if (is_uintN) {
                    const uint32_t n_values = (uint32_t)L.aux0;
                    if (n_values == 0) act = ACT_ALL;
                    else if (n_values != 1 || L.in_typed_cnt[vt] != 1) act = ACT_NONE;
                    else if (!probe(H, nH)) act = ACT_NONE;
                    else { act = fixed_ok ? ACT_FIXED_EQ : ACT_ROW_EQ; pay = P.u64s[L.in_typed_off[vt]]; }
                } else tostring_path(true);
                break;
            case F_CONTAINS_ANY:
                if (is_uintN) {
                    if (L.in_typed_cnt[vt] == 0) act = ACT_NONE;
                    else {
                        bool ok = probe(H, nH);
                        if (ok && !(L.in_skip_sets || (uint64_t)L.in_nsets > 10ull * rows)) {
                            bool any = false;
                            const uint32_t* sets = P.u32s + L.in_sets_off;
                            for (uint32_t s = 0; s < L.in_nsets && !any; s++) { bloom_bytes += 8ull * sets[2 * s + 1]; any = bloom_contains_all_warp(bloom, c->bloom_words, P.u64s + sets[2 * s], sets[2 * s + 1]); }
                            ok = any;
                        }
                        act = !ok ? ACT_NONE : fixed_ok ? ACT_FIXED_IN : ACT_ROW_IN;
                    }
                } else {
                    bool ok = probe(H, nH);
                    if (ok) {
                        bool any = false;
                        const uint32_t* sets = P.u32s + L.in_sets_off;
                        for (uint32_t s = 0; s < L.in_nsets; s++) { bloom_bytes += 8ull * sets[2 * s + 1]; any |= bloom_contains_all_warp(bloom, c->bloom_words, P.u64s + sets[2 * s], sets[2 * s + 1]); }
                        ok = any;
                    }
                    act = ok ? ACT_ROW : ACT_NONE;
                }
                break;
            case F_RANGE: {
                const double fmn = __longlong_as_double((long long)L.rng_fmin), fmx = __longlong_as_double((long long)L.rng_fmax);
                if (is_uintN) act = (fmx < 0 || L.rng_ulo > c->max_value || L.rng_uhi < c->min_value) ? ACT_NONE : ACT_ROW;
                else if (vt == VT_INT64) act = (L.rng_ilo > (int64_t)c->max_value || L.rng_ihi < (int64_t)c->min_value) ? ACT_NONE : ACT_ROW;
                else if (vt == VT_FLOAT64) act = (fmn > __longlong_as_double((long long)c->max_value) || fmx < __longlong_as_double((long long)c->min_value)) ? ACT_NONE : ACT_ROW;
                else if (vt == VT_IPV4) act = (c->min_value > (uint64_t)L.rng_iphi || c->max_value < (uint64_t)L.rng_iplo) ? ACT_NONE : ACT_ROW;
                else act = (fmx < 0 || L.rng_ilo > (int64_t)c->max_value || L.rng_ihi < (int64_t)c->min_value) ? ACT_NONE : ACT_ROW;
                break;
            }
            case F_EXACT_PREFIX: {
                const bool is_uint = vt == VT_UINT8 || vt == VT_UINT16 || vt == VT_UINT32 || vt == VT_UINT64;
                if (nl == 0) act = ACT_ALL;
                else if (is_uint) act = (L.nhashes > 0 || !tn.ok || tn.val > c->max_value) ? ACT_NONE : ACT_ROW;
                else if (vt == VT_INT64) {
                    bool dash = nl == 1 && nd[0] == '-';
                    if (L.nhashes > 0) act = ACT_NONE;
                    else if (!dash && (!tn.ok || tn.sval > (int64_t)c->max_value || tn.sval < (int64_t)c->min_value)) act = ACT_NONE;
                    else act = ACT_ROW;
                }
                else if (vt == VT_FLOAT64) act = (L.nhashes > 2 * 6 || !probe(H, L.nhashes)) ? ACT_NONE : ACT_ROW;
                else if (vt == VT_IPV4) act = (!(L.gates & GATE_DIGIT_PREFIX) || L.nhashes > 3 * 6 || !probe(H, L.nhashes)) ? ACT_NONE : ACT_ROW;
                else act = (!(L.gates & GATE_DIGIT_PREFIX) || !probe(H, L.nhashes)) ? ACT_NONE : ACT_ROW;
                break;
            }
            case F_LEN_RANGE: {
                const uint64_t mn = L.aux0, mx = L.aux1;
                uint8_t tmp[24];
                if (vt == VT_UINT8 || vt == VT_UINT16 || vt == VT_UINT32 || vt == VT_UINT64) {
                    const uint64_t maxd = vt == VT_UINT8 ? 3 : vt == VT_UINT16 ? 5 : vt == VT_UINT32 ? 10 : 20;
                    if (mn > maxd || mx == 0) act = ACT_NONE;
                    else if (mx < (uint64_t)fmt_u64(tmp, c->min_value) || mn > (uint64_t)fmt_u64(tmp, c->max_value)) act = ACT_NONE;
                    else act = ACT_ROW;
                } else if (vt == VT_INT64) {
                    if (mn > 21 || mx == 0) act = ACT_NONE;
                    else { int a = fmt_i64(tmp, (int64_t)c->min_value), b2 = fmt_i64(tmp, (int64_t)c->max_value); act = (uint64_t)(a > b2 ? a : b2) < mn ? ACT_NONE : ACT_ROW; }
                } else if (vt == VT_FLOAT64) act = (mn > 24 || mx == 0) ? ACT_NONE : ACT_ROW;
                else if (vt == VT_IPV4) act = (mn > 15 || mx < 7) ? ACT_NONE : ACT_ROW;
                else act = (mn > 24 || mx < 24) ? ACT_NONE : ACT_ALL;
                break;
            }
            case F_STRING_RANGE:
                if (vt == VT_INT64) act = (L.gates & GATE_SR_INT) ? ACT_ROW : ACT_NONE;
                else if (vt == VT_FLOAT64) act = (L.gates & GATE_SR_FLOAT) ? ACT_ROW : ACT_NONE;
                else act = (L.gates & GATE_SR_UINT) ? ACT_ROW : ACT_NONE;
                break;
            case F_IPV4_RANGE:
                if (vt != VT_IPV4) act = ACT_NONE;
                else act = (c->min_value > L.aux1 || c->max_value < L.aux0) ? ACT_NONE : ACT_ROW;
                break;
            }
        }
        if (act >= ACT_DICT || values_bytes) values_bytes = lens_stored_bytes(*c, rows) + c->data_len;
    }
    if (c && c->kind == COL_VALUES && c->vt == VT_DICT && act == ACT_DICT) values_bytes = lens_stored_bytes(*c, rows) + c->data_len;
    if (need) {
        if (c && c->kind == COL_VALUES && (values_bytes || act >= ACT_DICT) && lane_id() == 0) need[(uint64_t)b * B.nfields + slot] = 1;
        act = ACT_NONE; values_bytes = 0; bloom_bytes = 0; err = 0;
    } else if (c && c->kind == COL_VALUES && c->values_state != VALUES_STAGED && (values_bytes || act >= ACT_DICT)) {
        act = ACT_NONE; values_bytes = 0; err = ERR_VALUES_ABSENT;
    }
    if (c && c->kind == COL_VALUES && (act == ACT_SCAN || act >= ACT_ROW)) {
        need_lens = 1;
        if (act == ACT_SCAN) { ntiles = (uint32_t)((c->data_len + VL_TILE_BYTES - 1) / VL_TILE_BYTES); scan_bytes = c->data_len; scan_off = c->data_off; }
        else need_row = 1;
    }
    }
    if (need) return;
    if (lane_id() == 0) {
        if (valid) { action[b] = act; payload[b] = pay; }
        if (err) atomicMax(&stats[ST_ERROR], (unsigned long long)err);
        s_cnt[warp][0] = need_lens; s_cnt[warp][1] = ntiles; s_cnt[warp][2] = need_row;
        s_stat[warp][0] = bloom_bytes; s_stat[warp][1] = values_bytes; s_stat[warp][2] = values_bytes ? 1 : 0; s_stat[warp][3] = scan_bytes;
    }
    __syncthreads();
    if (threadIdx.x < 3) {
        uint32_t tot = 0;
        for (int w = 0; w < VL_PLAN_WARPS; w++) { s_off[w][threadIdx.x] = tot; tot += s_cnt[w][threadIdx.x]; }
        const uint32_t base = tot ? atomicAdd(&work_count[threadIdx.x], tot) : 0;
        for (int w = 0; w < VL_PLAN_WARPS; w++) s_off[w][threadIdx.x] += base;
    } else if (threadIdx.x >= 32 && threadIdx.x < 36) {
        const int k = threadIdx.x - 32;
        unsigned long long tot = 0;
        for (int w = 0; w < VL_PLAN_WARPS; w++) tot += s_stat[w][k];
        if (tot) atomicAdd(&stats[k == 0 ? ST_BLOOM_BYTES : k == 1 ? ST_VALUES_BYTES : k == 2 ? ST_COLUMNS_READ : ST_SCAN_BYTES], tot);
    }
    __syncthreads();
    if (need_lens && lane_id() == 0) lens_blocks[s_off[warp][0]] = b;
    if (need_row && lane_id() == 0) row_blocks[s_off[warp][2]] = b;
    for (uint32_t k = lane_id(); k < ntiles; k += 32) {
        const uint32_t t0 = k * VL_TILE_BYTES;
        tiles[s_off[warp][1] + k] = ScanTile{scan_off + t0, (uint32_t)min(scan_bytes - t0, (unsigned long long)VL_TILE_BYTES), b};
    }
}

struct OndiskCol { uint64_t col; uint64_t lens_total; uint64_t rows; };
static __global__ void k_finish_ondisk_cols(const uint8_t* __restrict__ arena, DevColumn* __restrict__ cols, const OndiskCol* __restrict__ oc, uint32_t n,
                                            unsigned long long* __restrict__ status) {
    uint32_t i = blockIdx.x * blockDim.x + threadIdx.x;
    if (i >= n) return;
    DevColumn& c = cols[oc[i].col];
    const uint64_t total = oc[i].lens_total, rows = oc[i].rows;
    unsigned err = 0;
    if (total < 1) err = 1;
    else {
        const uint8_t* p = arena + c.lens_off - 1;
        uint32_t lt = p[0];
        if (lt > 7) err = 2;
        else {
            uint64_t want = lt < 4 ? (rows << lt) : (1ull << (lt - 4));
            if (total - 1 != want) err = 3;
            else {
                c.lens_type = (uint8_t)lt;
                if (lt >= 4) {
                    uint64_t v = 0; for (uint64_t k = 0; k < want; k++) v = (v << 8) | p[1 + k];
                    if (v > 0xFFFFFFFFull) err = 4;
                    else { c.lens_const = (uint32_t)v; c.data_const = (rows >= 2 && c.data_len == v) ? 1 : 0; }
                }
            }
        }
    }
    if (err) atomicMax(&status[0], (unsigned long long)err);
}
struct ColPatch { uint64_t col; DevColumn c; };
static __global__ void k_patch_cols(DevColumn* __restrict__ cols, const ColPatch* __restrict__ p, uint32_t n) {
    const uint32_t i = blockIdx.x * blockDim.x + threadIdx.x;
    if (i < n) cols[p[i].col] = p[i].c;
}

static __global__ void k_lens_offsets(BatchView B, int slot, const uint32_t* __restrict__ lens_blocks, const uint32_t* __restrict__ work_count,
                               uint32_t* __restrict__ row_off8, uint8_t* __restrict__ ready, unsigned long long* __restrict__ stats, int wc_idx = WC_LENS) {
    const uint32_t nwork = work_count[wc_idx];
    const uint32_t warps = (gridDim.x * blockDim.x) >> 5, lane = lane_id();
    for (uint32_t j = (blockIdx.x * blockDim.x + threadIdx.x) >> 5; j < nwork; j += warps) {
        const uint32_t b = lens_blocks[j];
        if (ready[b]) continue;
        const DevColumn& c = B.cols[(uint64_t)b * B.nfields + slot];
        if (c.values_state != VALUES_STAGED) {
            if (lane == 0) atomicMax(&stats[ST_ERROR], (unsigned long long)ERR_VALUES_ABSENT);
            continue;
        }
        const uint32_t rows = B.blk_rows[b];
        const uint64_t w0 = B.blk_word_off[b]; const uint32_t nw = (uint32_t)(B.blk_word_off[b + 1] - w0);
        const uint8_t* lens = B.arena + c.lens_off;
        if (c.lens_type >= 4) {
            if (lane == 0) {
                if ((unsigned long long)rows * c.lens_const != c.data_len) atomicMax(&stats[ST_ERROR], (unsigned long long)ERR_LENS_MISMATCH);
                ready[b] = 1;
            }
            continue;
        }
        unsigned long long carry = 0;
        for (uint32_t base = 0; base < nw; base += 32) {
            const uint32_t w = base + lane;
            uint32_t g[8] = {0, 0, 0, 0, 0, 0, 0, 0};
            unsigned long long sum = 0;
            if (w < nw) {
                const uint32_t r0 = w * 64, r1 = min(rows, r0 + 64);
                if (c.lens_type == 0) {
                    if (r1 - r0 == 64) {
                        const uint4* v = (const uint4*)(lens + r0);
#pragma unroll
                        for (int q = 0; q < 4; q++) { uint4 x = v[q]; g[2 * q] = __vsadu4(x.x, 0) + __vsadu4(x.y, 0); g[2 * q + 1] = __vsadu4(x.z, 0) + __vsadu4(x.w, 0); }
                    } else for (uint32_t r = r0; r < r1; r++) g[(r - r0) >> 3] += lens[r];
#pragma unroll
                    for (int q = 0; q < 8; q++) sum += g[q];
                } else {
                    unsigned long long g64[8] = {0, 0, 0, 0, 0, 0, 0, 0};
                    for (uint32_t r = r0; r < r1; r++) g64[(r - r0) >> 3] += c.lens_type == 3 ? ld_be64(lens + 8 * (uint64_t)r) : (unsigned long long)row_len(c, lens, r);
#pragma unroll
                    for (int q = 0; q < 8; q++) { sum += g64[q]; g[q] = (uint32_t)min(g64[q], 0xFFFFFFFFull); }
                    if (sum > 0xFFFFFFFFull) sum = 0x100000000ull;
                }
            }
            unsigned long long incl = sum;
#pragma unroll
            for (int d = 1; d < 32; d <<= 1) { unsigned long long t = __shfl_up_sync(0xffffffffu, incl, d); if (lane >= d) incl += t; }
            const unsigned long long excl = carry + incl - sum;
            if (w < nw) {
                uint32_t o = (uint32_t)min(excl, 0xFFFFFFFFull);
                uint4 a, bq;
                a.x = o; o += g[0]; a.y = o; o += g[1]; a.z = o; o += g[2]; a.w = o; o += g[3];
                bq.x = o; o += g[4]; bq.y = o; o += g[5]; bq.z = o; o += g[6]; bq.w = o;
                uint4* dst = (uint4*)(row_off8 + ((w0 + w) << 3));
                dst[0] = a; dst[1] = bq;
            }
            carry += __shfl_sync(0xffffffffu, incl, 31);
        }
        if (lane == 0) {
            if (carry != c.data_len) atomicMax(&stats[ST_ERROR], (unsigned long long)ERR_LENS_MISMATCH);
            ready[b] = 1;
        }
    }
}

struct ScanParams {
    uint32_t mode;
    uint32_t needle_off, needle_len;
    uint32_t pat[4], msk[4];
    int32_t delta[4];
    uint32_t nd16[4];
    uint8_t starts_tok, ends_tok;
    int32_t regex;
};

static __device__ __forceinline__ uint32_t ld_u32_unaligned(const uint8_t* p) {
    const uint32_t* a = (const uint32_t*)((uintptr_t)p & ~(uintptr_t)3);
    return __funnelshift_r(a[0], a[1], 8 * (uint32_t)((uintptr_t)p & 3));
}

static __device__ __forceinline__ void scan_verify_lane(const DevProgram& P, const BatchView& B, const DevColumn& c, const ScanParams& sp, uint32_t b,
                                                     const uint32_t* __restrict__ row_off8, uint32_t pos, uint64_t* __restrict__ leaf_bm) {
    const uint8_t* data = B.arena + c.data_off;
    const uint32_t L = sp.needle_len, n = (uint32_t)c.data_len;
    const uint32_t lens_type = c.lens_type, lens_const = c.lens_const;
    const uint8_t* lens = B.arena + c.lens_off;
    const uint32_t rows = B.blk_rows[b];
    const uint64_t w0 = B.blk_word_off[b];
    if ((uint64_t)pos + L > n) return;
    {
        const uint32_t head = L < 16 ? L : 16;
#pragma unroll
        for (uint32_t k = 0; k < 16; k += 4) {
            if (k >= head) break;
            const uint32_t m = head - k >= 4 ? 0xFFFFFFFFu : (1u << (8 * (head - k))) - 1;
            if ((ld_u32_unaligned(data + pos + k) ^ sp.nd16[k >> 2]) & m) return;
        }
        const uint8_t* nd = P.blob + sp.needle_off;
        for (uint32_t k = 16; k < L; k++) if (data[pos + k] != nd[k]) return;
    }
    uint32_t r, off, len;
    if (lens_type >= 4) {
        len = lens_const;
        if (len == 0) return;
        r = pos / len; off = r * len;
        if (r >= rows) return;
    } else {
        const uint32_t* ro = row_off8 + (w0 << 3);
        const uint32_t n8 = (rows + 7) >> 3;
        uint32_t lo, hi;
        {
            const uint32_t g = min((uint32_t)(__uint2float_rz(pos) * __fdividef(__uint2float_rz(n8), __uint2float_rz(n))), n8 - 1);
            lo = g ? g - 1 : 0; hi = min(g + 1, n8 - 1);
            if (!(ro[lo] <= pos && (hi + 1 >= n8 || ro[hi + 1] > pos))) { lo = 0; hi = n8 - 1; }
        }
        while (lo < hi) { const uint32_t mid = (lo + hi + 1) >> 1; if (ro[mid] <= pos) lo = mid; else hi = mid - 1; }
        const uint32_t r0 = lo * 8, kmax = min(8u, rows - r0);
        uint32_t o = ro[lo];
        r = r0; off = o; len = 0;
        if (lens_type == 0) {
            const uint2 lw = *(const uint2*)(lens + r0);
            const uint64_t l8 = ((uint64_t)lw.y << 32) | lw.x;
            for (uint32_t k = 0; k < kmax && o <= pos; k++) { const uint32_t l = (uint32_t)(l8 >> (8 * k)) & 0xFF; r = r0 + k; off = o; len = l; o += l; }
        } else {
            for (uint32_t k = 0; k < kmax && o <= pos; k++) { const uint32_t l = row_len(c, lens, r0 + k); r = r0 + k; off = o; len = l; o += l; }
        }
        if (pos < off || pos - off >= len) return;
    }
    if ((uint64_t)off + len > n) return;
    if (pos + L > off + len) return;
    const uint8_t* s = data + off; const uint32_t p = pos - off;
    bool hit;
    switch (sp.mode) {
    case SCAN_PHRASE: hit = phrase_boundaries_ok(s, len, p, L, sp.starts_tok, sp.ends_tok); break;
    case SCAN_PREFIX: hit = phrase_boundaries_ok(s, len, p, L, sp.starts_tok, false); break;
    case SCAN_CONTAINS: hit = true; break;
    case SCAN_RX_DOTPLUS: hit = p + L < len; break;
    case SCAN_RX_TAIL: {
        const DevRegex& R = P.regexes[sp.regex];
        hit = find_bytes(s, p, P.blob + R.prefix_off, R.prefix_len, 0) >= 0;
        break;
    }
    default: {
        const DevRegex& R = P.regexes[sp.regex];
        if (R.tail_len) hit = find_bytes(s + p + L, len - p - L, P.blob + R.tail_off, R.tail_len, 0) >= 0;
// ... 456 lines not shown
```

### victorialogs_b200/csrc/vl_zstd.cu

```cuda
#include "vl_zstd.h"

#include <algorithm>
#include <array>
#include <atomic>
#include <chrono>
#include <cstdio>
#include <cstdlib>
#include <cstring>
#include <exception>
#include <thread>

#include "vl_engine.h"
#include "vl_zstd.cuh"
#include "vl_zstd_job.h"

namespace vl {

using namespace zs;

struct ZstdDev {
    DevBuf frames, blocks, bstate, huf_tab, fse_tab, huf_state, fse_state, predef, lits, seqs, frame_err, status, lists;
    bool predef_ready = false;
    cudaStream_t xstream = nullptr;
    std::vector<cudaEvent_t> events;
    cudaEvent_t event(size_t i) {
        while (events.size() <= i) { cudaEvent_t e; VL_CUDA(cudaEventCreateWithFlags(&e, cudaEventDisableTiming)); events.push_back(e); }
        return events[i];
    }
    void* hpin = nullptr; size_t hpin_cap = 0;
    void* ensure_hpin(size_t n) {
        if (n <= hpin_cap) return hpin;
        if (hpin) cudaFreeHost(hpin);
        hpin = nullptr; hpin_cap = 0;
        VL_CUDA(cudaMallocHost(&hpin, n + n / 4 + 4096)); hpin_cap = n + n / 4 + 4096;
        return hpin;
    }
    void release() {
        DevBuf* all[] = {&frames, &blocks, &bstate, &huf_tab, &fse_tab, &huf_state, &fse_state, &predef, &lits, &seqs, &frame_err, &status, &lists};
        for (DevBuf* b : all) b->release();
        for (cudaEvent_t e : events) cudaEventDestroy(e);
        events.clear();
        if (xstream) cudaStreamDestroy(xstream);
        xstream = nullptr;
        if (hpin) cudaFreeHost(hpin);
        hpin = nullptr; hpin_cap = 0;
    }
};

static __global__ void k_pull_words(uint4* __restrict__ dst, const uint4* __restrict__ src, size_t n) {
    for (size_t i = (size_t)blockIdx.x * blockDim.x + threadIdx.x; i < n; i += (size_t)gridDim.x * blockDim.x) dst[i] = src[i];
}
void zstd_dev_free(ZstdDev* d) { if (d) { d->release(); delete d; } }

namespace {
inline unsigned cdiv_u(uint64_t a, uint64_t b) { return (unsigned)((a + b - 1) / b); }
}

struct ZstdJob::Impl : ZstdJobImpl {};

ZstdJob::ZstdJob() : m(new Impl) {}
ZstdJob::~ZstdJob() { delete m; }
bool ZstdJob::empty() const { return m->frames.empty(); }
uint64_t ZstdJob::frames() const { return m->frames.size(); }
uint64_t ZstdJob::blocks() const { return m->blocks.size(); }
uint64_t ZstdJob::compressed_blocks() const { return m->n_compressed; }
uint64_t ZstdJob::sequences() const { return m->n_seqs; }
uint64_t ZstdJob::groups() const { return m->groups.size(); }
void ZstdJob::set_dst(uint32_t id, uint64_t arena_off) { m->frames[id].dst = arena_off; }
void ZstdJob::set_group_hook(std::function<void(uint64_t)> f) { m->group_hook = std::move(f); }

void ZstdJob::add_frame(const uint8_t* f, size_t n, uint64_t zoff, uint64_t* regen, uint32_t* id) {
    ZFrame fr{};
    zwalk::parse_frame_into(m->blocks, (uint32_t)m->frames.size(), f, n, zoff, fr);
    *regen = fr.fcs; *id = (uint32_t)m->frames.size();
    m->commit_frame(fr);
}

size_t ZstdJob::add_bytes_block(const uint8_t* p, size_t n, uint64_t zoff, uint64_t* regen, uint32_t* id) {
    ZFrame fr{};
    const size_t used = zwalk::parse_bytes_block_into(m->blocks, (uint32_t)m->frames.size(), p, n, zoff, fr);
    *regen = fr.fcs; *id = (uint32_t)m->frames.size();
    m->commit_frame(fr);
    return used;
}

void ZstdJob::add_values_blocks(const ZValuesBlock* v, size_t n, int threads, ZValuesInfo* info, size_t* bad, std::string* msg) {
    *bad = SIZE_MAX;
    if (!m->frames.empty()) throw BadInput("BUG: add_values_blocks needs an empty job");
    if (threads > 0) { m->walk_values_blocks(v, n, threads, info, bad, msg); return; }
    uint64_t total_seqs = 0;
    if (!group_scale_env()) {
        ZstdJob dry;
        dry.m->limit_scale = 1u << 20;
        for (size_t i = 0; i < n; i++) {
            try {
                uint64_t r = 0; uint32_t id = 0;
                const size_t c1 = dry.add_bytes_block(v[i].p, v[i].n, v[i].zoff, &r, &id);
                dry.add_bytes_block(v[i].p + c1, v[i].n - c1, v[i].zoff + c1, &r, &id);
            } catch (const BadInput&) { break; }
        }
        total_seqs = dry.m->n_seqs;
    }
    auto taper = [&] { if (!group_scale_env()) m->limit_scale = (m->groups.empty() || m->n_seqs > total_seqs - total_seqs / 12) ? 1 : 4; };
    for (size_t i = 0; i < n; i++) {
        try {
            uint32_t f1 = 0, f2 = 0;
            taper();
            const size_t c1 = add_bytes_block(v[i].p, v[i].n, v[i].zoff, &info[i].lens_len, &f1);
            taper();
            const size_t c2 = add_bytes_block(v[i].p + c1, v[i].n - c1, v[i].zoff + c1, &info[i].data_len, &f2);
            if (c1 + c2 != v[i].n) throw BadInput("unexpected non-empty tail after reading bytes block with strings");
        } catch (const BadInput& e) { *bad = i; *msg = e.msg; return; }
    }
    if (!group_scale_env()) m->limit_scale = 1;
}

void ZstdJob::prepare() { m->prepare(); }

void ZstdJob::digest(uint64_t out[4]) const { m->digest(out); }

void ZstdJob::run(vlscan_ctx* ctx, const uint8_t* zsrc, uint8_t* arena) {
    Impl& J = *m;
    if (J.frames.empty()) return;
    auto now = [] { return std::chrono::duration<double>(std::chrono::steady_clock::now().time_since_epoch()).count(); };
    const double t_prep = now();
    J.prepare();
    const double t_lists = now();
    const std::vector<uint32_t>& lists = J.lists;
    if (!ctx->zdev) ctx->zdev = new ZstdDev;
    ZstdDev& D = *ctx->zdev;
    cudaStream_t st = ctx->stream;
    D.frames.ensure(J.frames.size() * sizeof(ZFrame) + 16); D.blocks.ensure(J.blocks.size() * sizeof(ZBlock) + 16); D.bstate.ensure(J.blocks.size() * sizeof(ZBlockState));
    D.frame_err.ensure(J.frames.size() * 4); D.status.ensure(16); D.lists.ensure(lists.size() * 4 + 16);
    D.huf_tab.ensure(std::max<size_t>((size_t)J.max_huf * Z_HUF_TABLE * 2, 16)); D.huf_state.ensure(std::max<size_t>((size_t)J.max_huf * sizeof(ZSlotState), 16));
    D.fse_tab.ensure(std::max<size_t>((size_t)J.max_fse * Z_FSE_SLOT_BYTES, 16)); D.fse_state.ensure(std::max<size_t>((size_t)J.max_fse * sizeof(ZSlotState), 16));
    const size_t lits_stride = (J.max_lits + 64 + 255) / 256 * 256, seqs_stride = std::max<size_t>(J.max_seqs, 1);
    D.lits.ensure(2 * lits_stride); D.seqs.ensure(2 * seqs_stride * 16);
    if (!D.xstream) VL_CUDA(cudaStreamCreateWithFlags(&D.xstream, cudaStreamNonBlocking));
    if (!D.predef_ready) {
        D.predef.ensure(Z_FSE_SLOT_BYTES);
        k_zstd_predef<<<1, 32, 0, st>>>(D.predef.as<uint8_t>());
        VL_CUDA(cudaFuncSetAttribute(k_seq_decode, cudaFuncAttributeMaxDynamicSharedMemorySize, (int)(Z_SEQ_CTA_LANES * (Z_FSE_SLOT_BYTES + Z_LINEBUF))));
        VL_CUDA(cudaFuncSetAttribute(k_huf_decode, cudaFuncAttributeMaxDynamicSharedMemorySize, (int)(Z_HUF_CTA_BLOCKS * Z_HUF_TABLE * 2)));
        ctx->launches++; VL_CUDA(cudaGetLastError());
        D.predef_ready = true;
    }
    {
        auto up16 = [](size_t n) { return (n + 15) / 16 * 16; };
        const size_t nf = up16(J.frames.size() * sizeof(ZFrame)), nb = up16(J.blocks.size() * sizeof(ZBlock)), nl = up16(lists.size() * 4);
        uint8_t* h = (uint8_t*)D.ensure_hpin(nf + nb + nl + 64);
        const double t_cp = now();
        J.spread_copy(h, J.frames.data(), J.frames.size() * sizeof(ZFrame));
        J.spread_copy(h + nf, J.blocks.data(), J.blocks.size() * sizeof(ZBlock));
        if (!lists.empty()) J.spread_copy(h + nf + nb, lists.data(), lists.size() * 4);
        if (getenv("VLSCAN_DEBUG_TIMING")) fprintf(stderr, "[vlscan zstd] host: work lists of %zu launch groups %.1f ms, %.1f MB of tables to pinned memory %.1f ms (%d threads)\n",
                                                   J.groups.size(), 1e3 * (t_lists - t_prep), (nf + nb + nl) / 1e6, 1e3 * (now() - t_cp), std::max(J.threads, 1));
        k_pull_words<<<296, 256, 0, st>>>(D.frames.as<uint4>(), (const uint4*)h, nf / 16); ctx->launches++;
        k_pull_words<<<296, 256, 0, st>>>(D.blocks.as<uint4>(), (const uint4*)(h + nf), nb / 16); ctx->launches++;
        if (nl) { k_pull_words<<<296, 256, 0, st>>>(D.lists.as<uint4>(), (const uint4*)(h + nf + nb), nl / 16); ctx->launches++; }
        VL_CUDA(cudaGetLastError());
    }
    VL_CUDA(cudaMemsetAsync(D.frame_err.p, 0, J.frames.size() * 4, st));
    VL_CUDA(cudaMemsetAsync(D.status.p, 0, 16, st));
    VL_CUDA(cudaMemsetAsync(D.bstate.p, 0, J.blocks.size() * sizeof(ZBlockState), st));
    ZView V{};
    V.src = zsrc; V.arena = arena; V.frames = D.frames.as<ZFrame>(); V.blocks = D.blocks.as<ZBlock>(); V.bstate = D.bstate.as<ZBlockState>();
    V.huf_tab = D.huf_tab.as<uint16_t>(); V.fse_tab = D.fse_tab.as<uint8_t>(); V.huf_state = D.huf_state.as<ZSlotState>(); V.fse_state = D.fse_state.as<ZSlotState>();
    V.predef = D.predef.as<uint8_t>(); V.lits = D.lits.as<uint8_t>(); V.seqs = D.seqs.as<uint4>(); V.frame_err = D.frame_err.as<unsigned int>();
    V.status = D.status.as<unsigned long long>();
    const uint32_t* L = D.lists.as<uint32_t>();
    const bool dbg = getenv("VLSCAN_DEBUG_TIMING") != nullptr;
    static const char* phase_name[6] = {"huf_build", "huf_decode", "fse_build", "seq_decode", "seq_resolve", "execute"};
    std::vector<std::pair<int, std::pair<cudaEvent_t, cudaEvent_t>>> marks;
    int phase = 0;
    static const bool overlap = [] { const char* e = getenv("VLSCAN_ZSTD_OVERLAP"); return !e || atoi(e) != 0; }();
    cudaStream_t xs = overlap ? D.xstream : st;
    cudaStream_t cur_stream = st;
    auto begin = [&](int p) { phase = p; if (dbg) { cudaEvent_t a, b; cudaEventCreate(&a); cudaEventCreate(&b); cudaEventRecord(a, cur_stream); marks.push_back({p, {a, b}}); } };
    auto launched = [&] { ctx->launches++; VL_CUDA(cudaGetLastError()); if (dbg) cudaEventRecord(marks.back().second.second, cur_stream); };
    VL_CUDA(cudaEventRecord(D.event(0), st)); VL_CUDA(cudaStreamWaitEvent(xs, D.event(0), 0));
    size_t gi = 0;
    for (const Group& g : J.groups) {
        uint32_t nh = g.huf_hi - g.huf_lo, nl = g.lit_hi - g.lit_lo, ns = g.seq_hi - g.seq_lo, nf = g.frame_hi - g.frame_lo;
        if (J.group_hook) {
            uint64_t need = 0;
            for (uint32_t i = J.frames[g.frame_lo].blk_lo; i < J.frames[g.frame_hi - 1].blk_hi; i++) need = std::max<uint64_t>(need, J.blocks[i].src + (J.blocks[i].type == ZB_RLE ? 1 : J.blocks[i].size));
            J.group_hook(need);
        }
        ZView W = V;
        W.lits = V.lits + (gi & 1) * lits_stride; W.seqs = V.seqs + (gi & 1) * seqs_stride;
        cudaEvent_t ev_entropy = D.event(1 + 2 * gi), ev_exec = D.event(2 + 2 * gi);
        cur_stream = st;
        if (gi >= 2) VL_CUDA(cudaStreamWaitEvent(st, D.event(2 + 2 * (gi - 2)), 0));
        if (nh) { begin(0); k_huf_build<<<cdiv_u(nh, 4), 128, 0, st>>>(W, L + g.huf_lo, nh); launched(); }
        if (nl) { begin(1); k_huf_decode<<<cdiv_u(nl, Z_HUF_CTA_BLOCKS), Z_HUF_CTA_BLOCKS * 4, Z_HUF_CTA_BLOCKS * Z_HUF_TABLE * 2, st>>>(W, L + g.lit_lo, nl); launched(); }
        if (ns) {
            begin(2); k_fse_build<<<cdiv_u(ns, 64), 64, 0, st>>>(W, L + g.seq_lo, ns); launched();
            begin(3); k_seq_decode<<<cdiv_u(ns, Z_SEQ_CTA_LANES), 64, Z_SEQ_CTA_LANES * (Z_FSE_SLOT_BYTES + Z_LINEBUF), st>>>(W, L + g.seq_lo, ns); launched();
        }
        VL_CUDA(cudaEventRecord(ev_entropy, st));
        VL_CUDA(cudaStreamWaitEvent(xs, ev_entropy, 0));
        cur_stream = xs;
        begin(4); k_seq_resolve<<<cdiv_u(nf, 64), 64, 0, xs>>>(W, g.frame_lo, nf); launched();
        begin(5); k_execute<<<cdiv_u((uint64_t)nf * 32, Z_EXEC_WARPS * 32), Z_EXEC_WARPS * 32, 0, xs>>>(W, L + g.ord_lo, nf); launched();
        VL_CUDA(cudaEventRecord(ev_exec, xs));
        gi++;
    }
    if (gi) VL_CUDA(cudaStreamWaitEvent(st, D.event(2 + 2 * (gi - 1)), 0));
    cur_stream = st;
    if (dbg) {
        VL_CUDA(cudaStreamSynchronize(xs)); VL_CUDA(cudaStreamSynchronize(st));
        float tot[6] = {0, 0, 0, 0, 0, 0};
        for (auto& mk : marks) { float ms = 0; cudaEventElapsedTime(&ms, mk.second.first, mk.second.second); tot[mk.first] += ms; cudaEventDestroy(mk.second.first); cudaEventDestroy(mk.second.second); }
        fprintf(stderr, "[vlscan zstd] %zu groups:", J.groups.size());
        for (int p = 0; p < 6; p++) fprintf(stderr, " %s %.2f ms", phase_name[p], tot[p]);
        fprintf(stderr, "\n");
    }
    (void)phase;
    J.ran = true;
}

void ZstdJob::check(vlscan_ctx* ctx) {
    if (!m->ran) return;
    unsigned long long stt[2] = {0, 0};
    VL_CUDA(cudaMemcpyAsync(stt, ctx->zdev->status.p, 16, cudaMemcpyDeviceToHost, ctx->stream));
    VL_CUDA(cudaStreamSynchronize(ctx->stream));
    if (!stt[0]) return;
    static const char* what[] = {"", "bad Huffman tree description", "bad Huffman stream", "bad FSE table description", "bad sequences bitstream", "match offset beyond the regenerated data",
                                 "regenerated size differs from the frame content size", "bad literals section"};
    throw BadInput(std::string("cannot decompress block: ") + (stt[0] < 8 ? what[stt[0]] : "corrupted frame") + " (frame " + std::to_string(stt[1] - 1) + " of the batch)");
}

}
```

### victorialogs_b200/csrc/vl_zstd.h

```cpp
#pragma once
#include <stddef.h>
#include <stdint.h>
#include <functional>
#include <string>
#include <vector>

struct vlscan_ctx;

namespace vl {

struct ZstdDev;
void zstd_dev_free(ZstdDev* d);

struct ZstdTimings { float total_ms = 0; };

struct ZValuesBlock { const uint8_t* p; size_t n; uint64_t zoff; };
struct ZValuesInfo { uint64_t lens_len, data_len; };

class ZstdJob {
public:
    ZstdJob();
    ~ZstdJob();
    ZstdJob(const ZstdJob&) = delete;
    ZstdJob& operator=(const ZstdJob&) = delete;
    size_t add_bytes_block(const uint8_t* p, size_t n, uint64_t zoff, uint64_t* regen, uint32_t* id);
    void add_frame(const uint8_t* f, size_t n, uint64_t zoff, uint64_t* regen, uint32_t* id);
    void add_values_blocks(const ZValuesBlock* v, size_t n, int threads, ZValuesInfo* info, size_t* bad, std::string* msg);
    void prepare();
    void digest(uint64_t out[4]) const;
    void set_dst(uint32_t id, uint64_t arena_off);
    bool empty() const;
    uint64_t frames() const;
    uint64_t blocks() const;
    uint64_t compressed_blocks() const;
    uint64_t sequences() const;
    uint64_t groups() const;
    void set_group_hook(std::function<void(uint64_t src_end)> f);
    void run(vlscan_ctx* ctx, const uint8_t* zsrc, uint8_t* arena);
    void check(vlscan_ctx* ctx);
private:
    struct Impl;
    Impl* m;
};

}
```

### victorialogs_b200/scan.py

```python
import ctypes as C
import math
import os

import numpy as np

_HERE = os.path.dirname(os.path.abspath(__file__))
_LIB = None

F_NOOP, F_PHRASE, F_PREFIX, F_EXACT, F_IN, F_REGEXP, F_AND, F_OR, F_NOT = range(9)
F_EXACT_PREFIX, F_LEN_RANGE, F_STRING_RANGE, F_IPV4_RANGE, F_VALUE_TYPE = 9, 10, 11, 12, 13
F_ANY_CASE_PHRASE, F_ANY_CASE_PREFIX, F_SEQUENCE, F_CONTAINS_ALL, F_CONTAINS_ANY, F_EQ_FIELD, F_LE_FIELD, F_RANGE, F_TIME = 14, 15, 16, 17, 18, 19, 20, 21, 22
VT_STRING, VT_DICT, VT_UINT8, VT_UINT16, VT_UINT32, VT_UINT64, VT_FLOAT64, VT_IPV4, VT_ISO8601, VT_INT64 = 1, 2, 3, 4, 5, 6, 7, 8, 9, 10
COL_CONST, COL_VALUES = 1, 2
STAGE_ONDISK, STAGE_DECODED = 0, 1


class VlscanError(RuntimeError):
    def __init__(self, code, msg):
        super().__init__("vlscan error %d: %s" % (code, msg))
        self.code = code


class CColumn(C.Structure):
    _fields_ = [("field", C.c_uint32), ("kind", C.c_uint8), ("value_type", C.c_uint8), ("stage", C.c_uint8), ("dict_len", C.c_uint8),
                ("min_value", C.c_uint64), ("max_value", C.c_uint64),
                ("const_value", C.c_void_p), ("const_len", C.c_uint64),
                ("dict_blob", C.c_void_p), ("dict_offsets", C.c_void_p),
                ("values", C.c_void_p), ("values_len", C.c_uint64),
                ("lens_items", C.c_void_p), ("lens_items_len", C.c_uint64),
                ("data", C.c_void_p), ("data_len", C.c_uint64),
                ("bloom", C.c_void_p), ("bloom_len", C.c_uint64)]


class CBlock(C.Structure):
    _fields_ = [("rows", C.c_uint64), ("ncols", C.c_uint32), ("ts_marshal_type", C.c_uint32), ("cols", C.POINTER(CColumn)),
                ("timestamps", C.c_void_p), ("timestamps_len", C.c_uint64), ("min_timestamp", C.c_int64), ("max_timestamp", C.c_int64)]


class CStats(C.Structure):
    _fields_ = [(n, C.c_uint64) for n in ("blocks", "rows", "rows_matched", "blocks_matched", "values_bytes", "bloom_probe_bytes", "bitmap_bytes",
                                          "columns_read", "gpu_launches", "h2d_bytes", "d2h_bytes")] + \
               [("gpu_ms", C.c_double), ("scan_kernel_ms", C.c_double), ("scan_kernel_bytes", C.c_uint64), ("staged_columns", C.c_uint64), ("pruned_columns", C.c_uint64)]

    def as_dict(self):
        return {n: getattr(self, n) for n, _ in self._fields_}


BUCKET_PLAIN, BUCKET_WEEK, BUCKET_MONTH, BUCKET_YEAR = 0, 1, 2, 3
HITS_MAX_BY = 4
GEN_TIMESTAMPS = 1 << 4
GEN_T0, GEN_STEP = 1700000000000000000, 1000000
GEN_STREAMS_SHIFT = 12
I64_MIN = -(1 << 63)


def gen_streams(k):
    return k << GEN_STREAMS_SHIFT


class HitsQuery(C.Structure):
    _fields_ = [("step", C.c_int64), ("offset", C.c_int64), ("calendar", C.c_uint32), ("nby", C.c_uint32),
                ("by_names", C.POINTER(C.c_char_p)), ("by_name_lens", C.POINTER(C.c_size_t))]


class LastQuery(C.Structure):
    _fields_ = [("limit", C.c_uint64), ("min_timestamp", C.c_int64), ("nfields", C.c_uint32),
                ("field_names", C.POINTER(C.c_char_p)), ("field_name_lens", C.POINTER(C.c_size_t))]


class FacetsQuery(C.Structure):
    _fields_ = [("max_values_per_field", C.c_uint64), ("max_value_len", C.c_uint64), ("nfields", C.c_uint32),
                ("field_names", C.POINTER(C.c_char_p)), ("field_name_lens", C.POINTER(C.c_size_t))]


FACET_UINT64, FACET_NEGATIVE, FACET_STRING = 0, 1, 2
FACETS_DEFAULT_MAX_VALUES, FACETS_DEFAULT_MAX_VALUE_LEN = 1000, 128


class GenConfig(C.Structure):
    _fields_ = [("seed", C.c_uint64), ("total_rows", C.c_uint64), ("rows_per_block", C.c_uint32), ("hot_block_permille", C.c_uint32),
                ("hit_row_permille", C.c_uint32), ("columns_mask", C.c_uint32)]


EXPORTS = ["vlscan_device_count", "vlscan_ctx_create", "vlscan_ctx_free", "vlscan_last_error", "vlscan_ctx_stream", "vlscan_ctx_sync",
           "vlscan_program_create", "vlscan_program_free", "vlscan_program_nfields", "vlscan_program_field", "vlscan_program_leaf_tokens", "vlscan_program_prepass_tokens", "vlscan_program_in_hashes", "vlscan_program_in_typed", "vlscan_format_float64", "vlscan_parse_math_number", "vlscan_parse_typed", "vlscan_eval_predicate",
           "vlscan_batch_upload", "vlscan_batch_free", "vlscan_batch_nblocks", "vlscan_batch_rows", "vlscan_batch_words", "vlscan_batch_device_bytes",
           "vlscan_batch_generate", "vlscan_batch_download", "vlscan_host_blocks_get", "vlscan_host_blocks_field", "vlscan_host_blocks_bytes",
           "vlscan_host_blocks_free", "vlscan_host_blocks_compress", "vlscan_zstd_decompress", "vlscan_zstd_inspect", "vlscan_zstd_walk_digest", "vlscan_part_open", "vlscan_part_free", "vlscan_part_header", "vlscan_part_nblocks", "vlscan_part_block_header", "vlscan_part_timestamps",
           "vlscan_part_ncolumn_names", "vlscan_part_column_name", "vlscan_part_blocks", "vlscan_host_blocks_source", "vlscan_scan_resident", "vlscan_last_scan_stats", "vlscan_fetch_results", "vlscan_fetch_hits", "vlscan_gather_timestamps", "vlscan_gather_values", "vlscan_hits_stats", "vlscan_hits_sums", "vlscan_truncate_timestamp", "vlscan_last_rows", "vlscan_facets", "vlscan_result_digest", "vlscan_totals_sum", "vlscan_result_device_ptrs", "vlscan_scan_batch",
           "vlscan_scan_batch_keep", "vlscan_stage_selected"]


def lib_path():
    return os.path.join(_HERE, "libvlscan.so")


def lib():
    global _LIB
    if _LIB is None:
        path = lib_path()
        if not os.path.exists(path):
            raise ImportError("libvlscan.so is missing (%s): build it with victorialogs_b200/build.sh; there is no fallback path" % path)
        L = C.CDLL(path)
        L.vlscan_ctx_create.restype = C.c_void_p
        L.vlscan_last_error.restype = C.c_char_p
        L.vlscan_last_error.argtypes = [C.c_void_p]
        L.vlscan_ctx_stream.restype = C.c_void_p
        L.vlscan_ctx_stream.argtypes = [C.c_void_p]
        L.vlscan_program_field.restype = C.c_void_p
        L.vlscan_host_blocks_field.restype = C.c_void_p
        L.vlscan_host_blocks_get.restype = C.POINTER(CBlock)
        L.vlscan_program_leaf_tokens.restype = C.c_int64
        for n in ("vlscan_batch_nblocks", "vlscan_batch_rows", "vlscan_batch_words", "vlscan_batch_device_bytes", "vlscan_host_blocks_bytes"):
            getattr(L, n).restype = C.c_uint64
            getattr(L, n).argtypes = [C.c_void_p]
        for n in ("vlscan_ctx_free", "vlscan_program_free", "vlscan_batch_free", "vlscan_host_blocks_free"):
            getattr(L, n).argtypes = [C.c_void_p]
            getattr(L, n).restype = None
        L.vlscan_truncate_timestamp.argtypes = [C.c_int64, C.c_int64, C.c_int64, C.c_uint32]
        L.vlscan_truncate_timestamp.restype = C.c_int64
        L.vlscan_format_float64.argtypes = [C.c_uint64, C.c_char_p, C.c_size_t]
        L.vlscan_format_float64.restype = C.c_int
        _LIB = L
    return _LIB


def eval_predicate(kind, value, arg1=b"", arg2=b"", aux0=0, aux1=0):
    value, arg1, arg2 = _b(value), _b(arg1), _b(arg2)
    L = lib()
    L.vlscan_eval_predicate.argtypes = [C.c_int, C.c_char_p, C.c_size_t, C.c_char_p, C.c_size_t, C.c_char_p, C.c_size_t, C.c_uint64, C.c_uint64]
    r = L.vlscan_eval_predicate(kind, value, len(value), arg1, len(arg1), arg2, len(arg2), aux0, aux1)
    if r < 0:
        raise ValueError(kind)
    return bool(r)


def zstd_inspect(bytes_block):
    out = (C.c_uint64 * 5)()
    rc = lib().vlscan_zstd_inspect(bytes_block, C.c_size_t(len(bytes_block)), out)
    if rc:
        raise VlscanError(rc, lib().vlscan_last_error(None).decode("utf-8", "replace"))
    return dict(consumed=out[0], regenerated=out[1], blocks=out[2], compressed_blocks=out[3], sequences=out[4])


def zstd_walk_digest(host_blocks, threads):
    out = (C.c_uint64 * 12)()
    rc = lib().vlscan_zstd_walk_digest(host_blocks.blocks, C.c_uint64(host_blocks.nblocks), C.c_int(threads), out)
    if rc:
        raise VlscanError(rc, lib().vlscan_last_error(None).decode("utf-8", "replace"))
    return dict(digest=tuple(out[:4]), frames=out[4], blocks=out[5], groups=out[6], compressed_blocks=out[7], sequences=out[8],
                walk_seconds=out[9] * 1e-9, lists_seconds=out[10] * 1e-9)


def parse_typed(value_type, text):
    text = _b(text)
    out = C.c_uint64()
    r = lib().vlscan_parse_typed(C.c_int(value_type), text, C.c_size_t(len(text)), C.byref(out))
    if r < 0:
        raise ValueError(value_type)
    return out.value if r else None


def format_float64(bits):
    buf = C.create_string_buffer(352)
    n = lib().vlscan_format_float64(C.c_uint64(bits), buf, C.c_size_t(352))
    if n < 0:
        raise ValueError(bits)
    return buf.raw[:n]


def truncate_timestamp(ts, step, offset=0, calendar=BUCKET_PLAIN):
    return lib().vlscan_truncate_timestamp(ts, step, offset, calendar)


def hits_query(step, offset=0, calendar=BUCKET_PLAIN, by=()):
    names = [_b(f) for f in by]
    arr = (C.c_char_p * max(len(names), 1))(*names)
    lens = (C.c_size_t * max(len(names), 1))(*[len(x) for x in names])
    return HitsQuery(step, offset, calendar, len(names), arr, lens), (arr, lens)


def last_query(limit, fields=(), min_timestamp=None):
    names = [_b(f) for f in fields]
    arr = (C.c_char_p * max(len(names), 1))(*names)
    lens = (C.c_size_t * max(len(names), 1))(*[len(x) for x in names])
    floor = I64_MIN if min_timestamp is None else min_timestamp
    return LastQuery(limit, floor, len(names), arr, lens), (arr, lens)


def facets_query(fields, max_values_per_field=0, max_value_len=0):
    names = [_b(f) for f in fields]
    arr = (C.c_char_p * max(len(names), 1))(*names)
    lens = (C.c_size_t * max(len(names), 1))(*[len(x) for x in names])
    return FacetsQuery(max_values_per_field, max_value_len, len(names), arr, lens), (arr, lens)


def facets_merge(states, limit=10, keep_const_fields=False, max_values_per_field=0):
    rows = sum(n for _, n in states)
    max_values = max_values_per_field or FACETS_DEFAULT_MAX_VALUES
    merged, dropped = {}, set()
    for st, _ in states:
        for field, entries in st.items():
            if entries is None:
                dropped.add(field)
                continue
            m = merged.setdefault(field, {})
            for cls, text, hits in entries:
                m[(cls, text)] = m.get((cls, text), 0) + hits
    out = []
    for field in sorted(merged.keys() - dropped):
        m = merged[field]
        if len(m) > max_values:
            continue
        if len(m) == 1 and next(iter(m.values())) == rows and not keep_const_fields:
            continue
        ents = sorted(m.items(), key=lambda kv: (-kv[1], kv[0][1], kv[0][0]))[:limit]
        out.extend((field, text, hits) for (cls, text), hits in ents)
    return out


def stats_merge(states):
    out = {}
    for st in states:
        for bucket, keys, rows, vals in st:
            k = (bucket, keys)
            if k not in out:
                out[k] = (rows, list(vals))
                continue
            r0, v0 = out[k]
            out[k] = (r0 + rows, [(b if math.isnan(a) else a if math.isnan(b) else a + b, ca + cb) for (a, ca), (b, cb) in zip(v0, vals)])
    return out


def parse_math_number(s):
    L = lib()
    L.vlscan_parse_math_number.restype = C.c_double
    s = _b(s)
# ... 316 lines not shown
        L.vlscan_part_ncolumn_names.argtypes = [C.c_void_p]
        L.vlscan_part_column_name.restype = C.c_void_p
        L.vlscan_part_free.argtypes = [C.c_void_p]
        L.vlscan_part_free.restype = None
        L.vlscan_host_blocks_source.restype = C.POINTER(C.c_uint64)
        self._cb = None
        if inflate is not None:
            def cb(user, frame, n, dst, dn):
                try:
                    out = inflate(C.string_at(frame, n), dn)
                    if len(out) != dn:
                        return 1
                    C.memmove(dst, out, dn)
                    return 0
                except Exception:
                    return 2
            self._cb = INFLATE_FN(cb)
        self.h = C.c_void_p()
        rc = L.vlscan_part_open(ctx.h if ctx is not None else None, _b(path), self._cb if self._cb is not None else C.cast(None, INFLATE_FN), None, C.byref(self.h))
        if rc:
            raise VlscanError(rc, L.vlscan_last_error(ctx.h if ctx is not None else None).decode("utf-8", "replace"))
        out = (C.c_uint64 * 8)()
        L.vlscan_part_header(self.h, out)
        self.header = {k: (_signed(out[i]) if k in ("MinTimestamp", "MaxTimestamp") else out[i]) for i, k in enumerate(PART_HEADER_FIELDS)}
        self.nblocks = L.vlscan_part_nblocks(self.h)
        self.column_names = []
        for i in range(L.vlscan_part_ncolumn_names(self.h)):
            ln = C.c_size_t()
            p = L.vlscan_part_column_name(self.h, C.c_uint32(i), C.byref(ln))
            self.column_names.append(C.string_at(p, ln.value))

    def block_header(self, i):
        out = (C.c_uint64 * 15)()
        rc = lib().vlscan_part_block_header(self.h, C.c_uint64(i), out)
        if rc:
            raise VlscanError(rc, lib().vlscan_last_error(None).decode("utf-8", "replace"))
        return {k: (_signed(out[j]) if k in ("min_timestamp", "max_timestamp") else out[j]) for j, k in enumerate(BLOCK_HEADER_FIELDS)}

    def timestamps(self, i):
        p, n = C.c_void_p(), C.c_uint64()
        rc = lib().vlscan_part_timestamps(self.h, C.c_uint64(i), C.byref(p), C.byref(n))
        if rc:
            raise VlscanError(rc, lib().vlscan_last_error(None).decode("utf-8", "replace"))
        return C.string_at(p, n.value) if n.value else b""

    def blocks(self, fields, lo=0, hi=None, min_timestamp=-(1 << 63), max_timestamp=(1 << 63) - 1):
        fields = [_b(f) for f in fields]
        names = (C.c_char_p * max(len(fields), 1))(*fields)
        lens = (C.c_size_t * max(len(fields), 1))(*[len(f) for f in fields])
        h = C.c_void_p()
        rc = lib().vlscan_part_blocks(self.h, names, lens, C.c_uint32(len(fields)), C.c_uint64(lo), C.c_uint64(self.nblocks if hi is None else hi),
                                      C.c_int64(min_timestamp), C.c_int64(max_timestamp), C.byref(h))
        if rc:
            raise VlscanError(rc, lib().vlscan_last_error(None).decode("utf-8", "replace"))
        hb = DownloadedBlocks(None, None, _handle=h)
        n = C.c_uint64()
        p = lib().vlscan_host_blocks_source(h, C.byref(n))
        hb.source = [p[i] for i in range(n.value)]
        hb._part = self
        return hb

    def close(self):
        if self.h:
            lib().vlscan_part_free(self.h)
            self.h = None

    def __del__(self):
        try:
            self.close()
        except Exception:
            pass


def search_part(ctx, part, flt, min_timestamp=-(1 << 63), max_timestamp=(1 << 63) - 1, batch_blocks=8192):
    prog = Program(flt)
    fields = prog.fields()
    hits = []
    for lo in range(0, part.nblocks, batch_blocks):
        hb = part.blocks(fields, lo, min(part.nblocks, lo + batch_blocks), min_timestamp, max_timestamp)
        if hb.nblocks == 0:
            continue
        words, counts, _ = ctx.scan_batch(prog, hb)
        for src, w, c in zip(hb.source, split_bitmaps(words, hb.rows), counts):
            if c:
                bh = part.block_header(src)
                hits.append((src, w.copy(), int(c), min_timestamp <= bh["min_timestamp"] and bh["max_timestamp"] <= max_timestamp))
    return hits


def totals_sum(ctxs):
    arr = (C.c_void_p * len(ctxs))(*[c.h for c in ctxs])
    out = (C.c_uint64 * 4)()
    rc = lib().vlscan_totals_sum(arr, C.c_int(len(ctxs)), out)
    if rc:
        raise VlscanError(rc, lib().vlscan_last_error(None).decode("utf-8", "replace"))
    return [int(x) for x in out]


class Batch:
    def __init__(self, h, ctx):
        self.h = h
        self.ctx = ctx
        L = lib()
        self.nblocks = L.vlscan_batch_nblocks(h)
        self.rows = L.vlscan_batch_rows(h)
        self.words = L.vlscan_batch_words(h)
        self.device_bytes = L.vlscan_batch_device_bytes(h)

    def free(self):
        if self.h:
            lib().vlscan_batch_free(self.h)
            self.h = None

    def __del__(self):
        try:
            self.free()
        except Exception:
            pass


class KeptBatch:

    def __init__(self, nblocks, rows, words):
        self.nblocks, self.rows, self.words = nblocks, rows, words


class Ctx:

    def __init__(self, device=0):
        h = lib().vlscan_ctx_create(C.c_int(device))
        if not h:
            raise VlscanError(100, lib().vlscan_last_error(None).decode("utf-8", "replace"))
        self.h = C.c_void_p(h)

    def _check(self, rc):
        if rc:
            raise VlscanError(rc, lib().vlscan_last_error(self.h).decode("utf-8", "replace"))

    def _call_grown(self, call, caps, needed):
        rc, out = call(*caps)
        want = [int(w) for w in needed()]
        if rc and any(w > c for w, c in zip(want, caps)):
            rc, out = call(*[max(c, w) for c, w in zip(caps, want)])
        self._check(rc)
        return out

    @property
    def stream(self):
        return lib().vlscan_ctx_stream(self.h)

    def sync(self):
        self._check(lib().vlscan_ctx_sync(self.h))

    def zstd_decompress(self, frames, sizes):
        n = len(frames)
        keep = [C.create_string_buffer(f, len(f)) if f else C.create_string_buffer(1) for f in frames]
        ptrs = (C.c_void_p * max(n, 1))(*[C.cast(k, C.c_void_p) for k in keep])
        lens = (C.c_size_t * max(n, 1))(*[len(f) for f in frames])
        offs = np.zeros(n + 1, dtype=np.uint64)
        offs[1:] = np.cumsum(np.asarray(sizes, dtype=np.uint64)) if n else 0
        total = int(offs[-1])
        dst = C.create_string_buffer(max(total, 1))
        self._check(lib().vlscan_zstd_decompress(self.h, C.c_uint32(n), ptrs, lens, dst, offs.ctypes.data_as(C.c_void_p)))
        raw = dst.raw
        return [raw[int(offs[i]):int(offs[i + 1])] for i in range(n)]

    def upload(self, host_blocks, stats=None):
        names, lens = host_blocks.name_arrays()
        out = C.c_void_p()
        self._check(lib().vlscan_batch_upload(self.h, names, lens, C.c_uint32(len(host_blocks.field_names)), host_blocks.blocks,
                                              C.c_uint64(host_blocks.nblocks), C.byref(out), C.byref(stats) if stats is not None else None))
        return Batch(out, self)

    def generate(self, cfg, block_lo, block_hi):
        out = C.c_void_p()
        self._check(lib().vlscan_batch_generate(self.h, C.byref(cfg), C.c_uint64(block_lo), C.c_uint64(block_hi), C.byref(out)))
        return Batch(out, self)

    def download(self, batch):
        return DownloadedBlocks(self, batch)

    def scan_resident(self, program, batch, want_stats=True):
        st = CStats() if want_stats else None
        self._check(lib().vlscan_scan_resident(self.h, program.h, batch.h, C.byref(st) if st is not None else None))
        self._last = batch
        return st

    def last_scan_stats(self):
        st = CStats()
        self._check(lib().vlscan_last_scan_stats(self.h, C.byref(st)))
        return st

    def fetch(self, batch=None, bitmaps=True, counts=True, stats=None):
        batch = batch or self._last
        words = np.zeros(max(batch.words, 1), dtype=np.uint64) if bitmaps else None
        cnt = np.zeros(max(batch.nblocks, 1), dtype=np.uint32) if counts else None
        self._check(lib().vlscan_fetch_results(self.h, words.ctypes.data_as(C.c_void_p) if bitmaps else None,
                                               cnt.ctypes.data_as(C.c_void_p) if counts else None, C.byref(stats) if stats is not None else None))
        return (words[:batch.words] if bitmaps else None), (cnt[:batch.nblocks] if counts else None)

    def fetch_hits(self, batch=None, cap=None):
        batch = batch or self._last
        cap = cap if cap is not None else max(int(batch.rows), 1)
        hits = np.zeros(cap, dtype=np.uint32)
        offs = np.zeros(batch.nblocks + 1, dtype=np.uint64)
        self._check(lib().vlscan_fetch_hits(self.h, hits.ctypes.data_as(C.c_void_p), C.c_uint64(cap), offs.ctypes.data_as(C.c_void_p)))
        return hits[:int(offs[-1])], offs

    def gather_timestamps(self, batch=None):
        batch = batch or self._last
        cap = max(int(batch.rows), 1)
        ts = np.zeros(cap, dtype=np.int64)
        offs = np.zeros(batch.nblocks + 1, dtype=np.uint64)
        self._check(lib().vlscan_gather_timestamps(self.h, ts.ctypes.data_as(C.c_void_p), C.c_uint64(cap), offs.ctypes.data_as(C.c_void_p)))
        return ts[:int(offs[-1])], offs

    def gather_values(self, field, batch=None):
        batch = batch or self._last
        field = _b(field)
        hoffs = np.zeros(batch.nblocks + 1, dtype=np.uint64)
        nrows = max(int(batch.rows), 1)
        voffs = np.zeros(nrows + 1, dtype=np.uint64)
        total = C.c_uint64()

        def call(cap):
            out = np.zeros(cap, dtype=np.uint8)
            return lib().vlscan_gather_values(self.h, field, C.c_size_t(len(field)), out.ctypes.data_as(C.c_void_p), C.c_uint64(cap), voffs.ctypes.data_as(C.c_void_p),
                                              C.c_uint64(nrows), C.byref(total), hoffs.ctypes.data_as(C.c_void_p)), out
        out = self._call_grown(call, (1 << 16,), lambda: (total.value,))
        n = int(hoffs[-1])
        raw = out.tobytes()
        return [raw[int(voffs[i]):int(voffs[i + 1])] for i in range(n)], hoffs

    def hits_stats(self, step, offset=0, calendar=BUCKET_PLAIN, by=(), batch=None, info=None):
        batch = batch or getattr(self, "_last", None)
        q, keep = hits_query(step, offset, calendar, by)
        nby = len(by)
        out_info = (C.c_uint64 * 4)()

        def call(cap_groups, cap_bytes):
            buckets = np.zeros(cap_groups, dtype=np.int64)
            counts = np.zeros(cap_groups, dtype=np.uint64)
            offs = np.zeros(cap_groups * nby + 1, dtype=np.uint64)
            kb = np.zeros(max(cap_bytes, 1), dtype=np.uint8)
            rc = lib().vlscan_hits_stats(self.h, C.byref(q), buckets.ctypes.data_as(C.c_void_p), counts.ctypes.data_as(C.c_void_p), C.c_uint64(cap_groups),
                                         kb.ctypes.data_as(C.c_void_p), C.c_uint64(cap_bytes), offs.ctypes.data_as(C.c_void_p), out_info)
            return rc, (buckets, counts, offs, kb)
        buckets, counts, offs, kb = self._call_grown(call, (max(1, min(int(batch.rows) if batch else 0, 1 << 16)), 1 << 16), lambda: out_info[:2])
        if info is not None:
            info.update(groups=out_info[0], key_bytes=out_info[1], rows=out_info[2], blocks_decoded=out_info[3])
        keys = _row_texts(kb.tobytes(), offs, int(out_info[0]), nby)
        return [(int(buckets[g]), keys[g], int(counts[g])) for g in range(int(out_info[0]))]

    def hits_sums(self, step, offset=0, calendar=BUCKET_PLAIN, by=(), values=(), batch=None, info=None):
        batch = batch or getattr(self, "_last", None)
        q, keep = hits_query(step, offset, calendar, by)
        vn = [_b(f) for f in values]
        varr = (C.c_char_p * max(len(vn), 1))(*vn)
        vlens = (C.c_size_t * max(len(vn), 1))(*[len(x) for x in vn])
        nby, nv = len(by), len(vn)
        out_info = (C.c_uint64 * 4)()

        def call(cap_groups, cap_bytes):
            buckets = np.zeros(cap_groups, dtype=np.int64)
            counts = np.zeros(cap_groups, dtype=np.uint64)
            sums = np.zeros(max(cap_groups * nv, 1), dtype=np.float64)
            vcounts = np.zeros(max(cap_groups * nv, 1), dtype=np.uint64)
            offs = np.zeros(cap_groups * nby + 1, dtype=np.uint64)
            kb = np.zeros(max(cap_bytes, 1), dtype=np.uint8)
            rc = lib().vlscan_hits_sums(self.h, C.byref(q), varr, vlens, C.c_uint32(nv), buckets.ctypes.data_as(C.c_void_p), counts.ctypes.data_as(C.c_void_p),
                                        sums.ctypes.data_as(C.c_void_p), vcounts.ctypes.data_as(C.c_void_p), C.c_uint64(cap_groups),
                                        kb.ctypes.data_as(C.c_void_p), C.c_uint64(cap_bytes), offs.ctypes.data_as(C.c_void_p), out_info)
            return rc, (buckets, counts, sums, vcounts, offs, kb)
        buckets, counts, sums, vcounts, offs, kb = self._call_grown(call, (max(1, min(int(batch.rows) if batch else 0, 1 << 16)), 1 << 16), lambda: out_info[:2])
        if info is not None:
            info.update(groups=out_info[0], key_bytes=out_info[1], rows=out_info[2], blocks_decoded=out_info[3])
        G = int(out_info[0])
        keys = _row_texts(kb.tobytes(), offs, G, nby)
        return [(int(buckets[g]), keys[g], int(counts[g]), [(float(sums[g * nv + f]), int(vcounts[g * nv + f])) for f in range(nv)]) for g in range(G)]

    def last_rows(self, limit, fields=(), min_timestamp=None, info=None):
        q, keep = last_query(limit, fields, min_timestamp)
        nf = len(fields)
        out_info = (C.c_uint64 * 4)()

        def call(cap_rows, cap_bytes):
            ts = np.zeros(cap_rows, dtype=np.int64)
            blocks = np.zeros(cap_rows, dtype=np.uint32)
            rows = np.zeros(cap_rows, dtype=np.uint32)
            offs = np.zeros(cap_rows * nf + 1, dtype=np.uint64)
            vb = np.zeros(max(cap_bytes, 1), dtype=np.uint8)
            rc = lib().vlscan_last_rows(self.h, C.byref(q), ts.ctypes.data_as(C.c_void_p), blocks.ctypes.data_as(C.c_void_p), rows.ctypes.data_as(C.c_void_p),
                                        C.c_uint64(cap_rows), vb.ctypes.data_as(C.c_void_p), C.c_uint64(cap_bytes), offs.ctypes.data_as(C.c_void_p), out_info)
            return rc, (ts, blocks, rows, offs, vb)
        ts, blocks, rows, offs, vb = self._call_grown(call, (max(1, min(int(limit), 1 << 12)), 1 << 16), lambda: out_info[:2])
        if info is not None:
            info.update(rows=out_info[0], value_bytes=out_info[1], selected=out_info[2], blocks_decoded=out_info[3])
        texts = _row_texts(vb.tobytes(), offs, int(out_info[0]), nf)
        return [(int(ts[i]), int(blocks[i]), int(rows[i]), texts[i]) for i in range(int(out_info[0]))]

    def facets(self, fields, max_values_per_field=0, max_value_len=0, info=None):
        q, keep = facets_query(fields, max_values_per_field, max_value_len)
        nf = len(fields)
        out_info = (C.c_uint64 * 4)()

        def call(cap_entries, cap_bytes):
# ... 81 lines not shown
```

Baseline: 22.70 billion.

## Defer upload error checks, build batch layout on device, and add timeline marks

The scan-batch path no longer makes several blocking host round-trips during upload. The zstd and length status checks are folded into the single stats readback. The batch layout arrays (word_block, init bitmap) are now built by a GPU kernel from a small pinned buffer instead of host loops and large H2D copies. The full-arena memset is narrowed to skip the regenerated zstd region, with a slack-clearing kernel zeroing the alignment padding instead. Event-based timeline marks and an export for reading them are added, which cost an event record per mark during scans.

```diff
diff --git a/include/vlscan.h b/include/vlscan.h
--- a/include/vlscan.h
+++ b/include/vlscan.h
@@ -85,6 +85,7 @@
 const char* vlscan_last_error(const vlscan_ctx* ctx);
 void* vlscan_ctx_stream(const vlscan_ctx* ctx);
 int vlscan_ctx_sync(vlscan_ctx* ctx);
+int vlscan_last_timeline(vlscan_ctx* ctx, char* out, size_t cap, size_t* len);
 
 enum { VLSCAN_F_NOOP = 0, VLSCAN_F_PHRASE, VLSCAN_F_PREFIX, VLSCAN_F_EXACT, VLSCAN_F_IN, VLSCAN_F_REGEXP, VLSCAN_F_AND, VLSCAN_F_OR, VLSCAN_F_NOT,
        VLSCAN_F_EXACT_PREFIX = 9, VLSCAN_F_LEN_RANGE = 10, VLSCAN_F_STRING_RANGE = 11, VLSCAN_F_IPV4_RANGE = 12, VLSCAN_F_VALUE_TYPE = 13,
diff --git a/victorialogs_b200/csrc/vl_engine.cu b/victorialogs_b200/csrc/vl_engine.cu
--- a/victorialogs_b200/csrc/vl_engine.cu
+++ b/victorialogs_b200/csrc/vl_engine.cu
@@ -63,6 +63,18 @@
 };
 struct vlscan_part { vl::part::PartReader r; };
 
+void vlscan_ctx::mark(const char* name, cudaStream_t st) {
+    if (!marking) return;
+    if (mark_events.size() == marks.size()) {
+        cudaEvent_t e;
+        if (cudaEventCreate(&e) != cudaSuccess) { cudaGetLastError(); return; }
+        mark_events.push_back(e);
+    }
+    cudaEvent_t e = mark_events[marks.size()];
+    if (cudaEventRecord(e, st) != cudaSuccess) { cudaGetLastError(); return; }
+    marks.push_back({name, std::chrono::duration<double>(std::chrono::steady_clock::now().time_since_epoch()).count(), e});
+}
+
 void* vlscan_ctx::ensure_pinned(size_t n) {
     if (n <= pinned_cap) return pinned;
     if (pinned) cudaFreeHost(pinned);
@@ -100,24 +112,25 @@
     b->rows = 0;
     for (size_t i = 0; i < rows.size(); i++) { b->h_word_off[i + 1] = b->h_word_off[i] + (rows[i] + 63) / 64; b->rows += rows[i]; }
     b->nwords = b->h_word_off.back();
-    std::vector<uint32_t> wb(b->nwords);
-    std::vector<uint64_t> init(b->nwords);
-    for (size_t i = 0; i < rows.size(); i++) {
-        for (uint64_t w = b->h_word_off[i]; w < b->h_word_off[i + 1]; w++) { wb[w] = (uint32_t)i; init[w] = ~0ull; }
-        uint32_t tail = rows[i] & 63;
-        if (tail) init[b->h_word_off[i + 1] - 1] = (~0ull) >> (64 - tail);
-    }
     b->blk_rows.ensure(std::max<size_t>(rows.size() * 4, 16));
     b->blk_word_off.ensure((rows.size() + 1) * 8);
     b->word_block.ensure(std::max<size_t>(b->nwords * 4, 16));
     b->init_bitmap.ensure(std::max<size_t>(b->nwords * 8, 16));
-    if (!rows.empty()) VL_CUDA(cudaMemcpyAsync(b->blk_rows.p, rows.data(), rows.size() * 4, cudaMemcpyHostToDevice, ctx->stream));
-    VL_CUDA(cudaMemcpyAsync(b->blk_word_off.p, b->h_word_off.data(), (rows.size() + 1) * 8, cudaMemcpyHostToDevice, ctx->stream));
-    if (b->nwords) {
-        VL_CUDA(cudaMemcpyAsync(b->word_block.p, wb.data(), b->nwords * 4, cudaMemcpyHostToDevice, ctx->stream));
-        VL_CUDA(cudaMemcpyAsync(b->init_bitmap.p, init.data(), b->nwords * 8, cudaMemcpyHostToDevice, ctx->stream));
-    }
-    VL_CUDA(cudaStreamSynchronize(ctx->stream));
+    const size_t nr = (rows.size() + 1) / 2 * 2, need = nr * 4 + (rows.size() + 1) * 8;
+    if (!ctx->ev_layout) VL_CUDA(cudaEventCreateWithFlags(&ctx->ev_layout, cudaEventDisableTiming));
+    VL_CUDA(cudaEventSynchronize(ctx->ev_layout));
+    if (need > ctx->hlayout_cap) {
+        if (ctx->hlayout) VL_CUDA(cudaFreeHost(ctx->hlayout));
+        ctx->hlayout = nullptr; ctx->hlayout_cap = 0;
+        VL_CUDA(cudaMallocHost(&ctx->hlayout, need)); ctx->hlayout_cap = need;
+    }
+    uint32_t* h_rows = (uint32_t*)ctx->hlayout; uint64_t* h_off = (uint64_t*)(h_rows + nr);
+    if (!rows.empty()) memcpy(h_rows, rows.data(), rows.size() * 4);
+    memcpy(h_off, b->h_word_off.data(), (rows.size() + 1) * 8);
+    k_batch_layout<<<cdiv(((uint64_t)rows.size() + 1) * 32, 256), 256, 0, ctx->stream>>>(h_rows, h_off, (uint32_t)rows.size(), b->blk_rows.as<uint32_t>(), b->blk_word_off.as<uint64_t>(),
+                                                                                      b->word_block.as<uint32_t>(), b->init_bitmap.as<uint64_t>());
+    launch_check(ctx);
+    VL_CUDA(cudaEventRecord(ctx->ev_layout, ctx->stream));
 }
 }
 
@@ -137,10 +150,21 @@
 }
 static double now_s() { return std::chrono::duration<double>(std::chrono::steady_clock::now().time_since_epoch()).count(); }
 
+static const char* lens_check_message(unsigned long long e) {
+    static const char* what[] = {"", "cannot unmarshal uint64 block type from empty src", "unexpected uint64 block type", "unexpected block length for uint items", "row length does not fit 32 bits"};
+    return what[std::min<unsigned long long>(e, 4)];
+}
+static void check_lens(vlscan_ctx* ctx) {
+    unsigned long long cst[2] = {0, 0};
+    VL_CUDA(cudaMemcpy(cst, ctx->zcols.p, 16, cudaMemcpyDeviceToHost));
+    if (cst[0]) throw BadInput(lens_check_message(cst[0]));
+}
+
 namespace {
 struct Upload {
     vlscan_ctx* ctx; vlscan_batch* out; const vlscan_block* blocks; uint64_t nblocks; uint32_t nfields; vlscan_stats* stats;
     const std::vector<char>* need_bloom;
+    bool defer_checks;
     std::vector<DevColumn>& cols = out->h_cols;
     const bool dbg = getenv("VLSCAN_DEBUG_TIMING") != nullptr; const double t_start = now_s();
     Copier io{ctx};
@@ -186,6 +210,7 @@
         zinfo.resize(zv.size());
         const double t_w = now_s();
         if (!zv.empty()) zjob.add_values_blocks(zv.data(), zv.size(), host_threads(), zinfo.data(), &zbad, &zmsg);
+        ctx->mark("walked", ctx->stream);
         if (dbg) fprintf(stderr, "[vlscan upload] header walk of %zu values blocks on %d host threads: %.1f ms (after %.1f ms of collecting and enqueueing the copies)\n",
                          zv.size(), host_threads(), 1e3 * (now_s() - t_w), 1e3 * (t_w - t_start));
     }
@@ -292,10 +317,15 @@
                 patches[i].col = (*patch)[i]; patches[i].c = d;
             }
         }
+        ctx->mark("described", ctx->stream);
+        if (layout) { finish_batch_layout(ctx, out, rows); ctx->mark("layout", ctx->stream); }
         cudaStream_t cs = ctx->copy_stream;
         cudaEvent_t ev_cleared = io.events.make(), ev_copied = io.events.make();
-        VL_CUDA(cudaMemsetAsync(region.p, 0, bytes, ctx->stream));
+        const uint64_t regen_end = have_z ? cursor : 0;
+        VL_CUDA(cudaMemsetAsync(region.p, 0, have_z ? regen_base : bytes, ctx->stream));
+        if (have_z) VL_CUDA(cudaMemsetAsync(region.as<uint8_t>() + regen_end, 0, bytes - regen_end, ctx->stream));
         VL_CUDA(cudaEventRecord(ev_cleared, ctx->stream));
+        ctx->mark("cleared", ctx->stream);
         VL_CUDA(cudaStreamWaitEvent(cs, ev_cleared, 0));
         const double t_h2d = dbg ? now_s() : 0;
         double t_zrun = 0;
@@ -336,23 +366,20 @@
                 launch_check(ctx);
             }
             io.h2d += ocols.size() * sizeof(OndiskCol);
-            zjob.check(ctx);
-            unsigned long long cst[2] = {0, 0};
-            VL_CUDA(cudaMemcpy(cst, ctx->zcols.p, 16, cudaMemcpyDeviceToHost));
-            static const char* what[] = {"", "cannot unmarshal uint64 block type from empty src", "unexpected uint64 block type", "unexpected block length for uint items", "row length does not fit 32 bits"};
-            if (cst[0]) throw BadInput(what[std::min<unsigned long long>(cst[0], 4)]);
+            zjob.clear_slack(ctx, region.as<uint8_t>());
+            if (defer_checks) ctx->zcheck_pending = true;
+            else { zjob.check(ctx); check_lens(ctx); }
         }
         VL_CUDA(cudaStreamWaitEvent(ctx->stream, ev_copied, 0));
         double t_copy = 0;
         if (dbg) { VL_CUDA(cudaStreamSynchronize(ctx->stream)); t_copy = now_s(); }
         if (nfields) out->note_columns(cols);
-        if (layout) finish_batch_layout(ctx, out, rows);
-        else VL_CUDA(cudaStreamSynchronize(ctx->stream));
+        if (!defer_checks) VL_CUDA(cudaStreamSynchronize(ctx->stream));
         if (dbg) fprintf(stderr, "[vlscan upload] blocks=%llu arena=%.1f MB h2d=%.1f MB pieces=%zu+%zu pinned=%d: describe %.1f ms, alloc %.1f ms, copy %.1f ms (%.1f GB/s), "
-                                 "zstd %llu frames / %llu blocks / %llu sequences: enqueue %.1f ms, decode %.1f ms; layout %.1f ms\n", (unsigned long long)nblocks,
+                                 "zstd %llu frames / %llu blocks / %llu sequences: enqueue %.1f ms, decode %.1f ms\n", (unsigned long long)nblocks,
                          bytes / 1e6, io.h2d / 1e6, pieces.size(), io.src.size(), (int)io.all_pinned, 1e3 * (t_desc - t_start), 1e3 * (t_alloc - t_desc), 1e3 * (t_enq - (t_zrun > 0 ? t_zrun : t_h2d)), io.h2d / 1e9 / std::max(t_copy - t_start, 1e-9),
-                         (unsigned long long)zjob.frames(), (unsigned long long)zjob.compressed_blocks(), (unsigned long long)zjob.sequences(), 1e3 * (t_zrun > 0 ? t_zrun - t_h2d : 0), 1e3 * (t_copy - t_enq), 1e3 * (now_s() - t_copy));
-        if (layout) io.h2d += out->nwords * 12 + nblocks * 12;
+                         (unsigned long long)zjob.frames(), (unsigned long long)zjob.compressed_blocks(), (unsigned long long)zjob.sequences(), 1e3 * (t_zrun > 0 ? t_zrun - t_h2d : 0), 1e3 * (t_copy - t_enq));
+        if (layout) io.h2d += nblocks * 12 + 8;
         if (stats) stats->h2d_bytes += io.h2d;
         return bytes;
     }
@@ -362,11 +389,11 @@
 enum UploadMode { UP_FULL = 0, UP_HEADERS = 1, UP_VALUES = 2, UP_LATE = 3 };
 static void do_upload(vlscan_ctx* ctx, const char* const* field_names, const size_t* field_name_lens, uint32_t nfields, const vlscan_block* blocks,
                       uint64_t nblocks, vlscan_batch* out, vlscan_stats* stats, const std::vector<char>* need_bloom = nullptr, UploadMode mode = UP_FULL,
-                      const uint8_t* need = nullptr, uint64_t* zframes = nullptr) {
+                      const uint8_t* need = nullptr, uint64_t* zframes = nullptr, bool defer_checks = false) {
     VL_CUDA(cudaSetDevice(ctx->device));
     if (nblocks > 0xFFFFFFF0ull) throw BadInput("too many blocks in one batch");
     out->device = ctx->device; out->nfields = nfields;
-    Upload u{ctx, out, blocks, nblocks, nfields, stats, need_bloom};
+    Upload u{ctx, out, blocks, nblocks, nfields, stats, need_bloom, defer_checks};
     if (mode == UP_FULL || mode == UP_HEADERS) {
         for (uint32_t f = 0; f < nfields; f++) out->field_names.emplace_back(field_names[f], field_name_lens[f]);
         u.cols.assign((size_t)nblocks * std::max<uint32_t>(nfields, 1), DevColumn{});
@@ -569,9 +596,21 @@
 }
 
 static void read_stats(vlscan_ctx* ctx, vlscan_stats* st, bool check_error) {
+    if (!ctx->hstatus) VL_CUDA(cudaMallocHost(&ctx->hstatus, (4 + ST_COUNT) * 8));
+    unsigned long long* hs = ctx->hstatus;
+    const bool upload = ctx->zcheck_pending;
+    ctx->zcheck_pending = false;
+    if (upload) {
+        VL_CUDA(cudaMemcpyAsync(hs, zstd_status_words(ctx), 16, cudaMemcpyDeviceToHost, ctx->stream));
+        VL_CUDA(cudaMemcpyAsync(hs + 2, ctx->zcols.p, 16, cudaMemcpyDeviceToHost, ctx->stream));
+    }
+    VL_CUDA(cudaMemcpyAsync(hs + 4, ctx->stats.p, ST_COUNT * 8, cudaMemcpyDeviceToHost, ctx->stream));
+    VL_CUDA(cudaStreamSynchronize(ctx->stream));
+    ctx->mark("checked", ctx->stream);
+    if (upload && hs[0]) throw BadInput(zstd_status_message(hs));
+    if (upload && hs[2]) throw BadInput(lens_check_message(hs[2]));
     unsigned long long h[ST_COUNT];
-    VL_CUDA(cudaMemcpyAsync(h, ctx->stats.p, sizeof h, cudaMemcpyDeviceToHost, ctx->stream));
-    VL_CUDA(cudaStreamSynchronize(ctx->stream));
+    memcpy(h, hs + 4, sizeof h);
     if (check_error && h[ST_ERROR]) {
         static const char* const msg[] = {"", "cannot unmarshal strings: row lengths do not add up to the data length", "too big index for dict value",
                                           "unexpected length for binary representation of a number", "", "", "the filter needs the timestamps of a block that was handed over without them", "cannot unmarshal timestamps",
@@ -698,6 +737,10 @@
     if (ctx->pinned) cudaFreeHost(ctx->pinned);
     delete ctx->recycle;
     for (auto& e : ctx->scan_events) { cudaEventDestroy(e.first); cudaEventDestroy(e.second); }
+    for (cudaEvent_t e : ctx->mark_events) cudaEventDestroy(e);
+    if (ctx->hstatus) cudaFreeHost(ctx->hstatus);
+    if (ctx->hlayout) cudaFreeHost(ctx->hlayout);
+    if (ctx->ev_layout) cudaEventDestroy(ctx->ev_layout);
     if (ctx->ev_begin) cudaEventDestroy(ctx->ev_begin);
     if (ctx->ev_end) cudaEventDestroy(ctx->ev_end);
     if (ctx->copy_stream) cudaStreamDestroy(ctx->copy_stream);
@@ -707,6 +750,22 @@
 const char* vlscan_last_error(const vlscan_ctx* ctx) { return ctx ? ctx->err.c_str() : g_thread_err.c_str(); }
 void* vlscan_ctx_stream(const vlscan_ctx* ctx) { return (void*)ctx->stream; }
 int vlscan_ctx_sync(vlscan_ctx* ctx) { return guarded(ctx, [&] { VL_CUDA(cudaSetDevice(ctx->device)); VL_CUDA(cudaStreamSynchronize(ctx->stream)); }); }
+int vlscan_last_timeline(vlscan_ctx* ctx, char* out, size_t cap, size_t* len) {
+    return guarded(ctx, [&] {
+        VL_CUDA(cudaSetDevice(ctx->device));
+        VL_CUDA(cudaStreamSynchronize(ctx->stream));
+        std::string s;
+        char line[160];
+        for (const vlscan_ctx::Mark& m : ctx->marks) {
+            float ms = -1;
+            if (cudaEventElapsedTime(&ms, ctx->marks[0].ev, m.ev) != cudaSuccess) { cudaGetLastError(); ms = -1; }
+            snprintf(line, sizeof line, "%s %.3f %.3f\n", m.name, 1e3 * (m.host_s - ctx->marks[0].host_s), ms);
+            s += line;
+        }
+        *len = s.size();
+        if (out && cap) { const size_t n = std::min(cap - 1, s.size()); memcpy(out, s.data(), n); out[n] = 0; }
+    });
+}
 
 int vlscan_program_create(const void* tree, size_t tree_len, vlscan_program** out) {
     *out = nullptr;
@@ -1103,10 +1162,12 @@
     return guarded(ctx, [&] {
         if (!ctx->has_result) throw BadInput("no scan result to fetch on this ctx");
         VL_CUDA(cudaSetDevice(ctx->device));
+        read_stats(ctx, nullptr, true);
         uint64_t d2h = 0;
         if (out_bitmap_words && ctx->last_nwords) { VL_CUDA(cudaMemcpyAsync(out_bitmap_words, ctx->regs[0].p, ctx->last_nwords * 8, cudaMemcpyDeviceToHost, ctx->stream)); d2h += ctx->last_nwords * 8; }
         if (out_match_counts && ctx->last_nblocks) { VL_CUDA(cudaMemcpyAsync(out_match_counts, ctx->counts.p, ctx->last_nblocks * 4, cudaMemcpyDeviceToHost, ctx->stream)); d2h += ctx->last_nblocks * 4; }
-        read_stats(ctx, nullptr, true);
+        if (d2h) VL_CUDA(cudaStreamSynchronize(ctx->stream));
+        ctx->mark("fetched", ctx->stream);
         if (stats) stats->d2h_bytes += d2h;
     });
 }
@@ -1163,6 +1224,8 @@
                            const vlscan_block* blocks, uint64_t nblocks, uint64_t* out_bitmap_words, uint32_t* out_match_counts, vlscan_stats* stats, bool keep) {
     vlscan_batch* b = ctx->recycle ? ctx->recycle : new vlscan_batch();
     ctx->recycle = nullptr;
+    ctx->marks.clear(); ctx->marking = true;
+    ctx->mark("call", ctx->stream);
     b->field_names.clear(); b->slot_vt_mask.clear();
     uint64_t launches0 = ctx->launches;
     std::vector<char> need_bloom(nfields, 0), in_prog(nfields, 0);
@@ -1205,7 +1268,7 @@
                 }
             if (stats && probe) { stats->staged_columns += cols_need; stats->pruned_columns += cols_all - cols_need; }
             if (probe && vals_need * 8 > vals_all * 7) ctx->bf_skip = 7;
-            do_upload(ctx, field_names, field_name_lens, nfields, blocks, nblocks, b, stats, &need_bloom, UP_VALUES, need.data());
+            do_upload(ctx, field_names, field_name_lens, nfields, blocks, nblocks, b, stats, &need_bloom, UP_VALUES, need.data(), nullptr, true);
             if (keep) {
                 b->h_sig.assign((size_t)nblocks * nfields, vlscan_batch::CellSig{});
                 b->h_ncols.resize(nblocks);
@@ -1218,9 +1281,14 @@
                 }
             }
         });
-    } else rc = guarded(ctx, [&] { do_upload(ctx, field_names, field_name_lens, nfields, blocks, nblocks, b, stats, &need_bloom); });
-    if (!rc) rc = vlscan_scan_resident(ctx, prog, b, nullptr);
+    } else rc = guarded(ctx, [&] { do_upload(ctx, field_names, field_name_lens, nfields, blocks, nblocks, b, stats, &need_bloom, UP_FULL, nullptr, nullptr, true); });
+    if (!rc) { rc = vlscan_scan_resident(ctx, prog, b, nullptr); ctx->mark("scanned", ctx->stream); }
     if (!rc) rc = vlscan_fetch_results(ctx, out_bitmap_words, out_match_counts, stats);
+    if (ctx->zcheck_pending) {
+        const int rz = guarded(ctx, [&] { read_stats(ctx, nullptr, false); });
+        if (rz) rc = rz;
+    }
+    ctx->marking = false;
     if (!rc && stats) {
         rc = guarded(ctx, [&] { read_stats(ctx, stats, true); stats->blocks += b->nblocks; stats->rows += b->rows; stats->gpu_launches += ctx->launches - launches0; });
     }
diff --git a/victorialogs_b200/csrc/vl_engine.h b/victorialogs_b200/csrc/vl_engine.h
--- a/victorialogs_b200/csrc/vl_engine.h
+++ b/victorialogs_b200/csrc/vl_engine.h
@@ -130,6 +130,12 @@
     int sm_count = 132;
     int scan_occ[2] = {1, 1};
     int row_occ = 1;
+    bool zcheck_pending = false;
+    unsigned long long* hstatus = nullptr;
+    void* hlayout = nullptr; size_t hlayout_cap = 0; cudaEvent_t ev_layout = nullptr;
+    struct Mark { const char* name; double host_s; cudaEvent_t ev; };
+    std::vector<Mark> marks; std::vector<cudaEvent_t> mark_events; bool marking = false;
+    void mark(const char* name, cudaStream_t st);
     void* ensure_pinned(size_t n);
 };
 
diff --git a/victorialogs_b200/csrc/vl_kernels.cuh b/victorialogs_b200/csrc/vl_kernels.cuh
--- a/victorialogs_b200/csrc/vl_kernels.cuh
+++ b/victorialogs_b200/csrc/vl_kernels.cuh
@@ -490,7 +490,23 @@
             }
         }
     }
-    if (err) atomicMax(&status[0], (unsigned long long)err);
+    if (err) { c.kind = COL_MISSING; atomicMax(&status[0], (unsigned long long)err); }
+}
+
+static __global__ void k_batch_layout(const uint32_t* __restrict__ rows, const uint64_t* __restrict__ word_off, uint32_t nblocks, uint32_t* __restrict__ blk_rows,
+                                      uint64_t* __restrict__ blk_word_off, uint32_t* __restrict__ word_block, uint64_t* __restrict__ init) {
+    const uint64_t b = ((uint64_t)blockIdx.x * blockDim.x + threadIdx.x) / 32;
+    if (b > nblocks) return;
+    const uint64_t lo = word_off[b];
+    if ((threadIdx.x & 31) == 0) blk_word_off[b] = lo;
+    if (b == nblocks) return;
+    const uint64_t hi = word_off[b + 1];
+    const uint32_t r = rows[b], tail = r & 63;
+    if ((threadIdx.x & 31) == 0) blk_rows[b] = r;
+    for (uint64_t w = lo + (threadIdx.x & 31); w < hi; w += 32) {
+        word_block[w] = (uint32_t)b;
+        init[w] = (w + 1 == hi && tail) ? (~0ull) >> (64 - tail) : ~0ull;
+    }
 }
 struct ColPatch { uint64_t col; DevColumn c; };
 static __global__ void k_patch_cols(DevColumn* __restrict__ cols, const ColPatch* __restrict__ p, uint32_t n) {
diff --git a/victorialogs_b200/csrc/vl_zstd.cu b/victorialogs_b200/csrc/vl_zstd.cu
--- a/victorialogs_b200/csrc/vl_zstd.cu
+++ b/victorialogs_b200/csrc/vl_zstd.cu
@@ -50,7 +50,20 @@
 static __global__ void k_pull_words(uint4* __restrict__ dst, const uint4* __restrict__ src, size_t n) {
     for (size_t i = (size_t)blockIdx.x * blockDim.x + threadIdx.x; i < n; i += (size_t)gridDim.x * blockDim.x) dst[i] = src[i];
 }
+static __global__ void k_clear_slack(uint8_t* __restrict__ arena, const ZFrame* __restrict__ frames, uint32_t n) {
+    const uint32_t i = blockIdx.x * blockDim.x + threadIdx.x;
+    if (i >= n) return;
+    const uint64_t dst = frames[i].dst, end = dst + frames[i].fcs;
+    for (uint64_t a = dst / kArenaAlign * kArenaAlign; a < dst; a++) arena[a] = 0;
+    for (uint64_t a = end, e = (end + kArenaPad + kArenaAlign - 1) / kArenaAlign * kArenaAlign; a < e; a++) arena[a] = 0;
+}
 void zstd_dev_free(ZstdDev* d) { if (d) { d->release(); delete d; } }
+const void* zstd_status_words(vlscan_ctx* ctx) { return ctx->zdev->status.p; }
+std::string zstd_status_message(const unsigned long long st[2]) {
+    static const char* what[] = {"", "bad Huffman tree description", "bad Huffman stream", "bad FSE table description", "bad sequences bitstream", "match offset beyond the regenerated data",
+                                 "regenerated size differs from the frame content size", "bad literals section"};
+    return std::string("cannot decompress block: ") + (st[0] < 8 ? what[st[0]] : "corrupted frame") + " (frame " + std::to_string(st[1] - 1) + " of the batch)";
+}
 
 namespace {
 inline unsigned cdiv_u(uint64_t a, uint64_t b) { return (unsigned)((a + b - 1) / b); }
@@ -159,6 +172,7 @@
         k_pull_words<<<296, 256, 0, st>>>(D.blocks.as<uint4>(), (const uint4*)(h + nf), nb / 16); ctx->launches++;
         if (nl) { k_pull_words<<<296, 256, 0, st>>>(D.lists.as<uint4>(), (const uint4*)(h + nf + nb), nl / 16); ctx->launches++; }
         VL_CUDA(cudaGetLastError());
+        ctx->mark("tables", st);
     }
     VL_CUDA(cudaMemsetAsync(D.frame_err.p, 0, J.frames.size() * 4, st));
     VL_CUDA(cudaMemsetAsync(D.status.p, 0, 16, st));
@@ -192,6 +206,7 @@
         cudaEvent_t ev_entropy = D.event(1 + 2 * gi), ev_exec = D.event(2 + 2 * gi);
         cur_stream = st;
         if (gi >= 2) VL_CUDA(cudaStreamWaitEvent(st, D.event(2 + 2 * (gi - 2)), 0));
+        if (gi == 0) ctx->mark("group0", st);
         if (nh) { begin(0); k_huf_build<<<cdiv_u(nh, 4), 128, 0, st>>>(W, L + g.huf_lo, nh); launched(); }
         if (nl) { begin(1); k_huf_decode<<<cdiv_u(nl, Z_HUF_CTA_BLOCKS), Z_HUF_CTA_BLOCKS * 4, Z_HUF_CTA_BLOCKS * Z_HUF_TABLE * 2, st>>>(W, L + g.lit_lo, nl); launched(); }
         if (ns) {
@@ -207,6 +222,7 @@
         gi++;
     }
     if (gi) VL_CUDA(cudaStreamWaitEvent(st, D.event(2 + 2 * (gi - 1)), 0));
+    ctx->mark("decoded", st);
     cur_stream = st;
     if (dbg) {
         VL_CUDA(cudaStreamSynchronize(xs)); VL_CUDA(cudaStreamSynchronize(st));
@@ -220,15 +236,19 @@
     J.ran = true;
 }
 
+void ZstdJob::clear_slack(vlscan_ctx* ctx, uint8_t* arena) {
+    if (!m->ran) return;
+    const uint32_t n = (uint32_t)m->frames.size();
+    k_clear_slack<<<cdiv_u(n, 128), 128, 0, ctx->stream>>>(arena, ctx->zdev->frames.as<ZFrame>(), n);
+    ctx->launches++; VL_CUDA(cudaGetLastError());
+}
+
 void ZstdJob::check(vlscan_ctx* ctx) {
     if (!m->ran) return;
     unsigned long long stt[2] = {0, 0};
     VL_CUDA(cudaMemcpyAsync(stt, ctx->zdev->status.p, 16, cudaMemcpyDeviceToHost, ctx->stream));
     VL_CUDA(cudaStreamSynchronize(ctx->stream));
-    if (!stt[0]) return;
-    static const char* what[] = {"", "bad Huffman tree description", "bad Huffman stream", "bad FSE table description", "bad sequences bitstream", "match offset beyond the regenerated data",
-                                 "regenerated size differs from the frame content size", "bad literals section"};
-    throw BadInput(std::string("cannot decompress block: ") + (stt[0] < 8 ? what[stt[0]] : "corrupted frame") + " (frame " + std::to_string(stt[1] - 1) + " of the batch)");
-}
-
-}
+    if (stt[0]) throw BadInput(zstd_status_message(stt));
+}
+
+}
diff --git a/victorialogs_b200/csrc/vl_zstd.h b/victorialogs_b200/csrc/vl_zstd.h
--- a/victorialogs_b200/csrc/vl_zstd.h
+++ b/victorialogs_b200/csrc/vl_zstd.h
@@ -11,6 +11,8 @@
 
 struct ZstdDev;
 void zstd_dev_free(ZstdDev* d);
+const void* zstd_status_words(vlscan_ctx* ctx);
+std::string zstd_status_message(const unsigned long long st[2]);
 
 struct ZstdTimings { float total_ms = 0; };
 
@@ -37,6 +39,7 @@
     uint64_t groups() const;
     void set_group_hook(std::function<void(uint64_t src_end)> f);
     void run(vlscan_ctx* ctx, const uint8_t* zsrc, uint8_t* arena);
+    void clear_slack(vlscan_ctx* ctx, uint8_t* arena);
     void check(vlscan_ctx* ctx);
 private:
     struct Impl;
diff --git a/victorialogs_b200/scan.py b/victorialogs_b200/scan.py
--- a/victorialogs_b200/scan.py
+++ b/victorialogs_b200/scan.py
@@ -82,7 +82,7 @@
                 ("hit_row_permille", C.c_uint32), ("columns_mask", C.c_uint32)]
 
 
-EXPORTS = ["vlscan_device_count", "vlscan_ctx_create", "vlscan_ctx_free", "vlscan_last_error", "vlscan_ctx_stream", "vlscan_ctx_sync",
+EXPORTS = ["vlscan_device_count", "vlscan_ctx_create", "vlscan_ctx_free", "vlscan_last_error", "vlscan_ctx_stream", "vlscan_ctx_sync", "vlscan_last_timeline",
            "vlscan_program_create", "vlscan_program_free", "vlscan_program_nfields", "vlscan_program_field", "vlscan_program_leaf_tokens", "vlscan_program_prepass_tokens", "vlscan_program_in_hashes", "vlscan_program_in_typed", "vlscan_format_float64", "vlscan_parse_math_number", "vlscan_parse_typed", "vlscan_eval_predicate",
            "vlscan_batch_upload", "vlscan_batch_free", "vlscan_batch_nblocks", "vlscan_batch_rows", "vlscan_batch_words", "vlscan_batch_device_bytes",
            "vlscan_batch_generate", "vlscan_batch_download", "vlscan_host_blocks_get", "vlscan_host_blocks_field", "vlscan_host_blocks_bytes",
@@ -705,6 +705,17 @@
     def sync(self):
         self._check(lib().vlscan_ctx_sync(self.h))
 
+    def last_timeline(self):
+        n = C.c_size_t(0)
+        self._check(lib().vlscan_last_timeline(self.h, None, C.c_size_t(0), C.byref(n)))
+        buf = C.create_string_buffer(n.value + 1)
+        self._check(lib().vlscan_last_timeline(self.h, buf, C.c_size_t(n.value + 1), C.byref(n)))
+        out = []
+        for line in buf.value.decode().splitlines():
+            name, host_ms, dev_ms = line.split()
+            out.append((name, float(host_ms), float(dev_ms)))
+        return out
+
     def zstd_decompress(self, frames, sizes):
         n = len(frames)
         keep = [C.create_string_buffer(f, len(f)) if f else C.create_string_buffer(1) for f in frames]
```

Result: no change. 22.70 billion, median of 6 (-0.0%).
